# mooch443/trex

Hardware: AMD Instinct MI355X
Metric: frames/s end-to-end (segment+CNN-ID), 2048x2048 x100 individuals (higher is better)
Workload: dtype fp16x3-split

## Files before the change

### include/trexhip.h

```cpp
#ifndef TREXHIP_H
#define TREXHIP_H
#include <stddef.h>
#include <stdint.h>
#ifdef __cplusplus
extern "C" {
#endif

#define TREXHIP_ABI_VERSION 22

enum {
    TREXHIP_OK = 0,
    TREXHIP_E_INVALID = -1,
    TREXHIP_E_DEVICE = -2,
    TREXHIP_E_CAPACITY = -3,
    TREXHIP_E_UNSUPPORTED = -4,
    TREXHIP_E_NOMEM = -5
};

#define TREXHIP_FRAME_OVERFLOW_RUNS   1u
#define TREXHIP_FRAME_OVERFLOW_OUTPUT 2u
#define TREXHIP_FRAME_MALFORMED       4u

typedef struct trexhip_params {
    int32_t device;
    int32_t width, height;
    int32_t max_batch;
    int32_t max_runs;
    int32_t max_blobs;
    int32_t max_pixels;
    int32_t threshold;
    int32_t threshold_maximum;
    int32_t enable_difference;
    int32_t absolute_difference;
    int32_t image_invert;
    int32_t inclusive;
    int32_t zero_is_background;
    int32_t connectivity;
    int32_t dilation_size;
    int32_t use_closing;
    int32_t closing_size;
    int32_t n_ranges;
    double  cm_per_pixel;
    double  ranges[16];
    int32_t pixel_encoding;
    int32_t image_adjust, blur_difference, equalize_histogram, correct_luminance, use_adaptive_threshold;
    int32_t device_color_reduce;
    int32_t reserved_[1];
} trexhip_params;
enum { TREXHIP_ENC_GRAY = 0, TREXHIP_ENC_R3G3B2 = 1, TREXHIP_ENC_RGB8 = 2 };

#define TREXHIP_BLOB_IN_RANGE    0u
#define TREXHIP_BLOB_BELOW_RANGE 1u
#define TREXHIP_BLOB_BIG         2u

typedef struct trexhip_run { uint16_t x0, x1, y, pad; } trexhip_run;

typedef struct trexhip_blob {
    uint32_t run_begin, n_runs;
    uint32_t pix_begin, n_pixels;
    uint16_t x0, y0, x1, y1;
    uint32_t bid;
    uint32_t px_min_max;
    uint32_t parent;
    uint32_t flags;
    uint64_t m10, m01;
    uint64_t m20, m11, m02;
    uint64_t sp, spx, spy;
} trexhip_blob;

typedef struct trexhip_frame_info {
    uint32_t n_blobs, n_runs, n_pixels;
    uint32_t blob_begin, run_begin, pix_begin;
    uint32_t n_raw_runs, n_raw_blobs;
    uint32_t flags;
    uint32_t reserved[3];
} trexhip_frame_info;

typedef struct trexhip_batch_result {
    int32_t n_frames;
    uint32_t total_blobs, total_runs, total_pixels;
    const trexhip_frame_info* frames;
    const trexhip_blob* blobs;
    const trexhip_run* runs;
    const uint8_t* pixels;
    uint32_t pixel_channels;
    uint32_t reserved_;
} trexhip_batch_result;

typedef struct trexhip_device_view {
    const trexhip_frame_info* frames;
    const trexhip_blob* blobs;
// ... 92 lines not shown
    int32_t n_ranges;
    int32_t reserved_;
    double  size_ranges[16];
} trexhip_split_params;
typedef struct trexhip_split_info {
    int32_t threshold;
    int32_t effective_threshold;
    int32_t status;
    int32_t initial_action;
    int32_t n_result;
    int32_t n_evaluated;
    int32_t min_pixel, max_pixel;
    float   first_size;
    float   reserved_;
    double  min_size_bound;
} trexhip_split_info;
void trexhip_default_split_params(trexhip_split_params* p);
int trexhip_split_search_device(trexhip_ctx* ctx, const trexhip_split_params* sp, int32_t method, const int32_t* d_presumed_nr,
                                int32_t n_blobs, int32_t* d_thresholds, trexhip_split_info* d_info);

typedef struct trexhip_posture_params {
    float   outline_resample;
    int32_t outline_smooth_samples;
    int32_t outline_smooth_step;
    int32_t outline_approximate;
    float   outline_curvature_range_ratio;
    float   midline_walk_offset;
    int32_t max_points;
    int32_t posture_closing_steps, peak_mode, posture_direction_smoothing;
} trexhip_posture_params;
typedef struct trexhip_posture_info { int32_t status, n_outline, n_segments, tail_index, head_index, n_traced, reserved[2]; } trexhip_posture_info;
void trexhip_default_posture_params(trexhip_posture_params* p);
int trexhip_posture_device(trexhip_ctx* ctx, int32_t table, const trexhip_posture_params* pp, int32_t n_blobs,
                           float* d_outline, float* d_segments, trexhip_posture_info* d_info);

int trexhip_posture_auto_device(trexhip_ctx* ctx, const trexhip_posture_params* pp, int32_t method, int32_t track_posture_threshold,
                                int32_t n_blobs, float* d_outline, float* d_segments, trexhip_posture_info* d_info,
                                int32_t* d_threshold_used, int32_t* d_iterations);

typedef struct trexhip_midline_params {
    int32_t midline_resolution;
    float   midline_stiff_percentage;
    int32_t midline_invert;
    int32_t midline_start_with_head;
} trexhip_midline_params;
typedef struct trexhip_midline_info { int32_t status, n; float len, angle, offx, offy; int32_t reserved[2]; } trexhip_midline_info;
void trexhip_default_midline_params(trexhip_midline_params* p);
int trexhip_midline_device(trexhip_ctx* ctx, const trexhip_midline_params* mp, int32_t n_blobs, int32_t max_points,
                           const trexhip_posture_info* d_posture_info, float* d_segments, float* d_midline,
                           trexhip_midline_info* d_midline_info);
int trexhip_midline_movement_device(trexhip_ctx* ctx, const trexhip_midline_params* mp, int32_t n_blobs, int32_t max_points,
                                    const trexhip_posture_info* d_posture_info, float* d_segments, float* d_midline,
                                    trexhip_midline_info* d_midline_info, const float* d_movement_direction);

enum { TREXHIP_NORMALIZE_NONE = 0, TREXHIP_NORMALIZE_MOMENTS = 1, TREXHIP_NORMALIZE_POSTURE = 2 };
int trexhip_crops_device(trexhip_ctx* ctx, uint8_t* d_crops, int32_t n_blobs, int32_t out_w, int32_t out_h,
                         int32_t normalization, int32_t difference);

int trexhip_crops_transformed_device(trexhip_ctx* ctx, uint8_t* d_crops, int32_t n_blobs, int32_t out_w, int32_t out_h,
                                     const float* transforms, const float* midline_lengths, int32_t use_legacy,
                                     float image_scale, int32_t difference);
int trexhip_crops_posture_device(trexhip_ctx* ctx, uint8_t* d_crops, int32_t n_blobs, int32_t out_w, int32_t out_h,
                                 const trexhip_midline_info* d_midline_info, const float* midline_lengths, int32_t use_legacy,
                                 float image_scale, int32_t difference);

int trexhip_load_weights(trexhip_ctx* ctx, const void* blob, size_t bytes);
int trexhip_num_classes(trexhip_ctx* ctx);
int trexhip_network_channels(trexhip_ctx* ctx);
int trexhip_network_image_size(trexhip_ctx* ctx, int32_t* width, int32_t* height);
enum { TREXHIP_NET_V118_3 = 0, TREXHIP_NET_V100 = 1, TREXHIP_NET_V110 = 2, TREXHIP_NET_V119 = 3, TREXHIP_NET_V200 = 4 };
int trexhip_network_version(trexhip_ctx* ctx);
size_t trexhip_network_blob_bytes(int32_t version, int32_t classes, int32_t channels, int32_t width, int32_t height);
int trexhip_identify_chunk_crops(trexhip_ctx* ctx, int32_t* crops);
enum { TREXHIP_CNN_FP32 = 0, TREXHIP_CNN_BF16X6 = 1, TREXHIP_CNN_BF16X3 = 2, TREXHIP_CNN_FP16X3 = 3 };
int trexhip_set_identity_precision(trexhip_ctx* ctx, int32_t mode);
int trexhip_identify_device(trexhip_ctx* ctx, const uint8_t* d_crops, int32_t n, float* d_probs, float* d_logits);
int trexhip_identify(trexhip_ctx* ctx, const uint8_t* crops, int32_t n, float* probs);
int trexhip_identify_guard_stats(trexhip_ctx* ctx, uint32_t* rerun_crops, uint32_t* whole_batch);
int trexhip_identify_skip_stats(trexhip_ctx* ctx, uint32_t* passes, uint32_t* listed, uint64_t* bytes_filled);

int trexhip_identify_skip3_stats(trexhip_ctx* ctx, uint32_t* pairs, uint32_t* listed, uint32_t* passes, uint64_t* bytes_filled);

int trexhip_identify_skipx_stats(trexhip_ctx* ctx, uint32_t* crops_windowed, uint32_t* windowed_passes, uint32_t* full_passes);

int trexhip_identify_fc1_stats(trexhip_ctx* ctx, uint32_t* rows, uint32_t* listed);

int trexhip_export_id_table_device(trexhip_ctx* ctx, const float* d_probs, int32_t n_blobs, int32_t classes,
                                   uint32_t frame_base, void* d_table, int32_t max_rows);
int trexhip_export_id_table_ex_device(trexhip_ctx* ctx, const float* d_probs, int32_t n_blobs, int32_t classes, uint32_t frame_base,
                                      const float* d_midline, const trexhip_midline_info* d_midline_info, int32_t midline_resolution,
                                      void* d_table, int32_t max_rows);

typedef struct trexhip_comm trexhip_comm;
int trexhip_comm_unique_id(void* id128);
int trexhip_comm_create(trexhip_ctx* ctx, const void* id128, int32_t rank, int32_t world, trexhip_comm** out);
void trexhip_comm_destroy(trexhip_comm* comm);
int trexhip_comm_rank(trexhip_comm* comm);
int trexhip_comm_world(trexhip_comm* comm);
int trexhip_comm_gather_device(trexhip_comm* comm, const void* d_send, size_t bytes, void* d_recv_rank0);
int trexhip_comm_gather_device_on(trexhip_comm* comm, trexhip_ctx* stream_ctx, const void* d_send, size_t bytes, void* d_recv_rank0);
int trexhip_comm_count_ranks(trexhip_comm* comm, int32_t* ranks_seen);

enum { TREXHIP_STAGE_ROWS = 0, TREXHIP_STAGE_SEGMENT_ALL = 1, TREXHIP_STAGE_CONV2 = 2, TREXHIP_STAGE_CONV3 = 3,
       TREXHIP_STAGE_CNN_ALL = 4, TREXHIP_STAGE_CROPS = 5, TREXHIP_STAGE_POSTURE = 6,
       TREXHIP_STAGE_UPLOAD_COPY = 8, TREXHIP_STAGE_UPLOAD_DMA = 9, TREXHIP_STAGE_COUNT = 10 };
int trexhip_profile_enable(trexhip_ctx* ctx, int32_t on);
int trexhip_profile_read(trexhip_ctx* ctx, int32_t stage, double* total_ms, int64_t* launches);
int trexhip_profile_reset(trexhip_ctx* ctx);

#define TREXHIP_NET_CATEGORY 100
typedef struct trexhip_trainer trexhip_trainer;
typedef struct {
    int32_t max_batch;
    float lr;
    float beta1, beta2, eps;
    float bn_momentum;
    float dropout;
    int32_t precision;
    uint64_t seed;
} trexhip_train_params;
size_t trexhip_weight_blob_bytes(int32_t classes, int32_t channels);
int trexhip_trainer_create(trexhip_ctx* ctx, const void* blob, size_t bytes, const trexhip_train_params* params, trexhip_trainer** out);
void trexhip_trainer_destroy(trexhip_trainer* trainer);
int trexhip_trainer_set_lr(trexhip_trainer* trainer, float lr);
int64_t trexhip_trainer_steps(trexhip_trainer* trainer);
int trexhip_trainer_image_size(trexhip_trainer* trainer, int32_t* width, int32_t* height);
int trexhip_trainer_version(trexhip_trainer* trainer, int32_t* version);
size_t trexhip_trainer_keep_mask_bytes(trexhip_trainer* trainer, int32_t n);
int trexhip_train_step_device(trexhip_trainer* trainer, const float* d_inputs, const int32_t* d_targets, int32_t n, const uint8_t* d_keep_masks,
                              float* loss, int32_t* correct);
int trexhip_train_eval_device(trexhip_trainer* trainer, const float* d_inputs, const int32_t* d_targets, int32_t n, float* loss, int32_t* correct);
int trexhip_train_eval(trexhip_trainer* trainer, const float* inputs, const int32_t* targets, int32_t n, float* loss, int32_t* correct);
int trexhip_train_step(trexhip_trainer* trainer, const float* inputs, const int32_t* targets, int32_t n, const uint8_t* keep_masks, float* loss,
                       int32_t* correct);
int trexhip_train_predict_device(trexhip_trainer* trainer, const uint8_t* d_crops, int32_t n, float* d_probs);
int trexhip_trainer_read(trexhip_trainer* trainer, int32_t tensor, int32_t kind, float* out, size_t count);
int trexhip_trainer_export(trexhip_trainer* trainer, void* blob, size_t capacity, size_t* bytes);

typedef struct {
    float degrees;
    float translate_x, translate_y;
    float brightness_lo, brightness_hi;
    float contrast_lo, contrast_hi;
    float saturation_lo, saturation_hi;
    float hue_lo, hue_hi;
    uint64_t seed;
} trexhip_augment_params;
typedef struct {
    float angle; int32_t tx, ty;
    float brightness, contrast, saturation, hue;
    int32_t order;
} trexhip_augment_draw;
void trexhip_default_augment_params(trexhip_augment_params* p, int32_t width, int32_t height);
int trexhip_augment_device(trexhip_ctx* ctx, const trexhip_augment_params* ap, const uint8_t* d_pool, const int32_t* d_pool_targets,
                           int32_t pool_size, const int32_t* indices, int32_t n, int32_t width, int32_t height, int32_t channels,
                           trexhip_augment_draw* d_draws, int32_t draws_given, uint64_t counter, float* d_out, int32_t* d_targets_out);

typedef struct {
    uint32_t good_frames, bad_frames;
    float    good_ratio;
    float    mean_unique;
    float    mean_unique_raw;
} trexhip_uniqueness_result;
int trexhip_validation_metrics_device(trexhip_ctx* ctx, const float* d_probs, int32_t n, int32_t classes,
                                      const int32_t* d_targets,
                                      const int32_t* frame_ranges,
// ... 58 lines not shown
```

### trex_amd/capi.py

```python
import collections
import ctypes as C
import os
import numpy as np

_HERE = os.path.dirname(os.path.abspath(__file__))
LIB_PATH = os.environ.get("TREXHIP_LIB_PATH") or os.path.join(_HERE, "libtrexhip.so")
_LIB = None

RUN_DTYPE = np.dtype([("x0", "<u2"), ("x1", "<u2"), ("y", "<u2"), ("pad", "<u2")])
BLOB_DTYPE = np.dtype([
    ("run_begin", "<u4"), ("n_runs", "<u4"), ("pix_begin", "<u4"), ("n_pixels", "<u4"),
    ("x0", "<u2"), ("y0", "<u2"), ("x1", "<u2"), ("y1", "<u2"),
    ("bid", "<u4"), ("px_min_max", "<u4"), ("parent", "<u4"), ("flags", "<u4"),
    ("m10", "<u8"), ("m01", "<u8"), ("m20", "<u8"), ("m11", "<u8"), ("m02", "<u8"),
    ("sp", "<u8"), ("spx", "<u8"), ("spy", "<u8"),
])
INFO_DTYPE = np.dtype([
    ("n_blobs", "<u4"), ("n_runs", "<u4"), ("n_pixels", "<u4"),
    ("blob_begin", "<u4"), ("run_begin", "<u4"), ("pix_begin", "<u4"),
    ("n_raw_runs", "<u4"), ("n_raw_blobs", "<u4"), ("flags", "<u4"), ("reserved", "<u4", (3,)),
])
assert BLOB_DTYPE.itemsize == 104 and RUN_DTYPE.itemsize == 8 and INFO_DTYPE.itemsize == 48

CNN_FP32, CNN_BF16X6, CNN_BF16X3, CNN_FP16X3 = 0, 1, 2, 3
# ... 73 lines not shown
MIDLINE_INFO_DTYPE = np.dtype([("status", "<i4"), ("n", "<i4"), ("len", "<f4"), ("angle", "<f4"), ("offx", "<f4"), ("offy", "<f4"),
                               ("reserved", "<i4", (2,))])
POSTURE_INFO_DTYPE = np.dtype([("status", "<i4"), ("n_outline", "<i4"), ("n_segments", "<i4"), ("tail_index", "<i4"),
                               ("head_index", "<i4"), ("n_traced", "<i4"), ("reserved", "<i4", (2,))])


class BatchResult(C.Structure):
    _fields_ = [
        ("n_frames", C.c_int32), ("total_blobs", C.c_uint32), ("total_runs", C.c_uint32), ("total_pixels", C.c_uint32),
        ("frames", C.c_void_p), ("blobs", C.c_void_p), ("runs", C.c_void_p), ("pixels", C.c_void_p),
        ("pixel_channels", C.c_uint32), ("reserved_", C.c_uint32),
    ]


ENC_GRAY, ENC_R3G3B2, ENC_RGB8 = 0, 1, 2
FRAME_OVERFLOW_RUNS, FRAME_OVERFLOW_OUTPUT, FRAME_MALFORMED = 1, 2, 4


class DeviceView(C.Structure):
    _fields_ = [("frames", C.c_void_p), ("blobs", C.c_void_p), ("runs", C.c_void_p), ("pixels", C.c_void_p),
                ("totals", C.c_void_p), ("blob_frame", C.c_void_p)]


class TrexHipError(RuntimeError):
    def __init__(self, code, msg):
        super().__init__(f"libtrexhip error {code}: {msg}")
        self.code = code
        self.frames = None


class TrainParams(C.Structure):
    _fields_ = [("max_batch", C.c_int32), ("lr", C.c_float), ("beta1", C.c_float), ("beta2", C.c_float), ("eps", C.c_float),
                ("bn_momentum", C.c_float), ("dropout", C.c_float), ("precision", C.c_int32), ("seed", C.c_uint64)]


class AugmentParams(C.Structure):
    _fields_ = [("degrees", C.c_float), ("translate_x", C.c_float), ("translate_y", C.c_float), ("brightness_lo", C.c_float), ("brightness_hi", C.c_float),
                ("contrast_lo", C.c_float), ("contrast_hi", C.c_float), ("saturation_lo", C.c_float), ("saturation_hi", C.c_float),
                ("hue_lo", C.c_float), ("hue_hi", C.c_float), ("seed", C.c_uint64)]


AUGMENT_DRAW_DTYPE = np.dtype([("angle", "<f4"), ("tx", "<i4"), ("ty", "<i4"), ("brightness", "<f4"), ("contrast", "<f4"), ("saturation", "<f4"),
                               ("hue", "<f4"), ("order", "<i4")])
assert AUGMENT_DRAW_DTYPE.itemsize == 32
AUGMENT_IDENTITY_ORDER = 0xE4


class UniquenessResult(C.Structure):
    _fields_ = [("good_frames", C.c_uint32), ("bad_frames", C.c_uint32), ("good_ratio", C.c_float), ("mean_unique", C.c_float), ("mean_unique_raw", C.c_float)]


class ValidationMetrics:
    __slots__ = ("confusion", "per_class_accuracy", "good_frames", "bad_frames", "good_ratio", "mean_unique", "mean_unique_raw",
                 "unique_percent", "unique_percent_raw", "uniqueness_per_class")

    def __init__(self):
        for k in self.__slots__:
            setattr(self, k, None)


class ClassAverages:
    __slots__ = ("samples", "values", "max_index", "max_p")

    def __init__(self, samples, values, max_index, max_p):
        self.samples, self.values, self.max_index, self.max_p = samples, values, max_index, max_p


class VisualFieldResult:
    __slots__ = VF_OUTPUTS

    def __init__(self):
        for k in self.__slots__:
            setattr(self, k, None)


TrackletLabels = collections.namedtuple("TrackletLabels", "counts rows label share skipped")


SYMBOLS = [
    "trexhip_abi_version", "trexhip_network_channels", "trexhip_network_image_size", "trexhip_network_version", "trexhip_network_blob_bytes", "trexhip_identify_chunk_crops", "trexhip_comm_unique_id", "trexhip_comm_create", "trexhip_comm_destroy", "trexhip_comm_rank", "trexhip_comm_world", "trexhip_comm_gather_device", "trexhip_comm_gather_device_on", "trexhip_comm_count_ranks", "trexhip_last_error", "trexhip_default_params", "trexhip_create", "trexhip_destroy",
    "trexhip_set_stream", "trexhip_get_live_params", "trexhip_update_params", "trexhip_set_background", "trexhip_set_background_device", "trexhip_set_background_color", "trexhip_set_background_color_device", "trexhip_generate_average_device", "trexhip_get_background", "trexhip_segment_device",
    "trexhip_segment", "trexhip_segment_color", "trexhip_segment_color_device", "trexhip_rethreshold_device", "trexhip_rethreshold_per_blob_device", "trexhip_fetch_rethreshold", "trexhip_fetch", "trexhip_device_view_get", "trexhip_synchronize",
    "trexhip_profile_enable", "trexhip_profile_read", "trexhip_profile_reset",
    "trexhip_default_posture_params", "trexhip_posture_device", "trexhip_posture_auto_device", "trexhip_pack_frames_v6_device", "trexhip_crops_device", "trexhip_pixel_channels", "trexhip_device_alloc", "trexhip_device_free", "trexhip_copy_to_host", "trexhip_copy_to_device", "trexhip_crops_transformed_device", "trexhip_crops_posture_device", "trexhip_default_midline_params", "trexhip_midline_device", "trexhip_midline_movement_device", "trexhip_default_split_params", "trexhip_split_search_device", "trexhip_export_id_table_device", "trexhip_export_id_table_ex_device", "trexhip_load_weights", "trexhip_set_identity_precision", "trexhip_num_classes", "trexhip_identify_device", "trexhip_identify", "trexhip_identify_guard_stats", "trexhip_identify_skip_stats", "trexhip_identify_skip3_stats", "trexhip_identify_skipx_stats", "trexhip_identify_fc1_stats",
    "trexhip_weight_blob_bytes", "trexhip_trainer_create", "trexhip_trainer_destroy", "trexhip_trainer_set_lr", "trexhip_trainer_steps", "trexhip_trainer_image_size", "trexhip_trainer_version", "trexhip_trainer_keep_mask_bytes", "trexhip_train_step_device", "trexhip_train_step", "trexhip_train_eval_device", "trexhip_train_eval", "trexhip_trainer_read", "trexhip_trainer_export",
    "trexhip_default_augment_params", "trexhip_augment_device",
    "trexhip_train_predict_device", "trexhip_validation_metrics_device", "trexhip_class_averages_device",
    "trexhip_lzo1x_bound", "trexhip_lzo1x_compress", "trexhip_pv_write_frames",
    "trexhip_load_frames_v6_device", "trexhip_lzo1x_decompress", "trexhip_pv_read_frames",
    "trexhip_default_prefilter_params", "trexhip_prefilter_device",
    "trexhip_default_vf_params", "trexhip_visual_field_device",
    "trexhip_categorize_load_weights", "trexhip_categorize_info", "trexhip_categorize_blob_bytes", "trexhip_categorize_device", "trexhip_categorize",
    "trexhip_tracklet_labels_device",
]


def lib():
    global _LIB
    if _LIB is None:
        if not os.path.exists(LIB_PATH):
            raise TrexHipError(-1, f"{LIB_PATH} is missing: run __graft_entry__.build() (make -C trex_amd/csrc)")
        L = C.CDLL(LIB_PATH)
        L.trexhip_last_error.restype = C.c_char_p
        L.trexhip_default_params.argtypes = [C.POINTER(Params), C.c_int32, C.c_int32]
        L.trexhip_default_params.restype = None
        L.trexhip_create.argtypes = [C.POINTER(Params), C.POINTER(C.c_void_p)]
        L.trexhip_destroy.argtypes = [C.c_void_p]
        L.trexhip_destroy.restype = None
        L.trexhip_set_stream.argtypes = [C.c_void_p, C.c_void_p]
        L.trexhip_get_live_params.argtypes = [C.c_void_p, C.POINTER(LiveParams)]
        L.trexhip_update_params.argtypes = [C.c_void_p, C.POINTER(LiveParams)]
        L.trexhip_set_background.argtypes = [C.c_void_p, C.c_void_p, C.c_int32]
        L.trexhip_set_background_device.argtypes = [C.c_void_p, C.c_void_p]
        L.trexhip_set_background_color.argtypes = [C.c_void_p, C.c_void_p, C.c_int32, C.c_int32, C.c_int32]
        L.trexhip_set_background_color_device.argtypes = [C.c_void_p, C.c_void_p, C.c_int32, C.c_int32]
        L.trexhip_generate_average_device.argtypes = [C.c_void_p, C.c_void_p, C.c_int32, C.c_int32]
        L.trexhip_get_background.argtypes = [C.c_void_p, C.c_void_p, C.c_int32]
        L.trexhip_segment_device.argtypes = [C.c_void_p, C.c_void_p, C.c_int32]
        L.trexhip_segment.argtypes = [C.c_void_p, C.POINTER(C.c_void_p), C.c_int32, C.c_int32]
        L.trexhip_segment_color.argtypes = [C.c_void_p, C.POINTER(C.c_void_p), C.c_int32, C.c_int32, C.c_int32, C.c_int32]
        L.trexhip_segment_color_device.argtypes = [C.c_void_p, C.c_void_p, C.c_int32, C.c_int32, C.c_int32]
        L.trexhip_rethreshold_device.argtypes = [C.c_void_p, C.c_int32, C.c_int32, C.c_void_p, C.c_int32]
        L.trexhip_rethreshold_per_blob_device.argtypes = [C.c_void_p, C.c_int32, C.c_void_p, C.c_int32, C.c_void_p, C.c_int32]
        L.trexhip_fetch_rethreshold.argtypes = [C.c_void_p, C.POINTER(BatchResult)]
        L.trexhip_fetch.argtypes = [C.c_void_p, C.POINTER(BatchResult)]
        L.trexhip_device_view_get.argtypes = [C.c_void_p, C.POINTER(DeviceView)]
        L.trexhip_synchronize.argtypes = [C.c_void_p]
        L.trexhip_profile_enable.argtypes = [C.c_void_p, C.c_int32]
        L.trexhip_profile_read.argtypes = [C.c_void_p, C.c_int32, C.POINTER(C.c_double), C.POINTER(C.c_int64)]
        L.trexhip_profile_reset.argtypes = [C.c_void_p]
        L.trexhip_default_midline_params.argtypes = [C.POINTER(MidlineParams)]
        L.trexhip_default_midline_params.restype = None
        L.trexhip_midline_device.argtypes = [C.c_void_p, C.POINTER(MidlineParams), C.c_int32, C.c_int32, C.c_void_p, C.c_void_p, C.c_void_p, C.c_void_p]
        L.trexhip_midline_movement_device.argtypes = [C.c_void_p, C.POINTER(MidlineParams), C.c_int32, C.c_int32, C.c_void_p, C.c_void_p, C.c_void_p, C.c_void_p, C.c_void_p]
        L.trexhip_default_split_params.argtypes = [C.POINTER(SplitParams)]
        L.trexhip_default_split_params.restype = None
        L.trexhip_split_search_device.argtypes = [C.c_void_p, C.POINTER(SplitParams), C.c_int32, C.c_void_p, C.c_int32, C.c_void_p, C.c_void_p]
        L.trexhip_crops_posture_device.argtypes = [C.c_void_p, C.c_void_p, C.c_int32, C.c_int32, C.c_int32, C.c_void_p, C.c_void_p, C.c_int32, C.c_float, C.c_int32]
        L.trexhip_default_posture_params.argtypes = [C.POINTER(PostureParams)]
        L.trexhip_default_posture_params.restype = None
        L.trexhip_posture_device.argtypes = [C.c_void_p, C.c_int32, C.POINTER(PostureParams), C.c_int32, C.c_void_p, C.c_void_p, C.c_void_p]
        L.trexhip_posture_auto_device.argtypes = [C.c_void_p, C.POINTER(PostureParams), C.c_int32, C.c_int32, C.c_int32, C.c_void_p, C.c_void_p, C.c_void_p, C.c_void_p, C.c_void_p]
        L.trexhip_crops_transformed_device.argtypes = [C.c_void_p, C.c_void_p, C.c_int32, C.c_int32, C.c_int32, C.c_void_p, C.c_void_p, C.c_int32, C.c_float, C.c_int32]
        L.trexhip_crops_device.argtypes = [C.c_void_p, C.c_void_p] + [C.c_int32] * 5
        L.trexhip_export_id_table_device.argtypes = [C.c_void_p, C.c_void_p, C.c_int32, C.c_int32, C.c_uint32, C.c_void_p, C.c_int32]
        L.trexhip_export_id_table_ex_device.argtypes = [C.c_void_p, C.c_void_p, C.c_int32, C.c_int32, C.c_uint32, C.c_void_p, C.c_void_p, C.c_int32, C.c_void_p, C.c_int32]
        L.trexhip_load_weights.argtypes = [C.c_void_p, C.c_void_p, C.c_size_t]
        L.trexhip_num_classes.argtypes = [C.c_void_p]
        L.trexhip_network_channels.argtypes = [C.c_void_p]
        L.trexhip_network_image_size.argtypes = [C.c_void_p, C.POINTER(C.c_int32), C.POINTER(C.c_int32)]
        L.trexhip_network_version.argtypes = [C.c_void_p]
        L.trexhip_network_blob_bytes.argtypes = [C.c_int32] * 5; L.trexhip_network_blob_bytes.restype = C.c_size_t
        L.trexhip_identify_chunk_crops.argtypes = [C.c_void_p, C.POINTER(C.c_int32)]
        L.trexhip_pack_frames_v6_device.argtypes = [C.c_void_p, C.c_void_p, C.c_void_p, C.c_size_t, C.c_void_p]
        L.trexhip_lzo1x_bound.argtypes = [C.c_size_t]; L.trexhip_lzo1x_bound.restype = C.c_size_t
        L.trexhip_lzo1x_compress.argtypes = [C.c_void_p, C.c_size_t, C.c_void_p, C.c_size_t, C.POINTER(C.c_size_t)]
        L.trexhip_pv_write_frames.argtypes = [C.c_void_p, C.c_void_p, C.c_int32, C.c_int32, C.c_uint64, C.c_void_p, C.c_size_t, C.c_void_p, C.POINTER(C.c_size_t)]
        L.trexhip_load_frames_v6_device.argtypes = [C.c_void_p, C.c_void_p, C.c_void_p, C.c_int32, C.c_void_p]
        L.trexhip_lzo1x_decompress.argtypes = [C.c_void_p, C.c_size_t, C.c_void_p, C.c_size_t, C.POINTER(C.c_size_t)]
        L.trexhip_pv_read_frames.argtypes = [C.c_void_p, C.c_size_t, C.c_uint64, C.c_void_p, C.c_int32, C.c_void_p, C.c_size_t, C.c_void_p, C.POINTER(C.c_size_t)]
        L.trexhip_comm_unique_id.argtypes = [C.c_void_p]
        L.trexhip_comm_create.argtypes = [C.c_void_p, C.c_void_p, C.c_int32, C.c_int32, C.POINTER(C.c_void_p)]
        L.trexhip_comm_destroy.argtypes = [C.c_void_p]
        L.trexhip_comm_destroy.restype = None
        L.trexhip_comm_rank.argtypes = [C.c_void_p]
        L.trexhip_comm_world.argtypes = [C.c_void_p]
        L.trexhip_comm_gather_device.argtypes = [C.c_void_p, C.c_void_p, C.c_size_t, C.c_void_p]
        L.trexhip_comm_gather_device_on.argtypes = [C.c_void_p, C.c_void_p, C.c_void_p, C.c_size_t, C.c_void_p]
        L.trexhip_comm_count_ranks.argtypes = [C.c_void_p, C.POINTER(C.c_int32)]
        L.trexhip_set_identity_precision.argtypes = [C.c_void_p, C.c_int32]
        L.trexhip_identify_device.argtypes = [C.c_void_p, C.c_void_p, C.c_int32, C.c_void_p, C.c_void_p]
        L.trexhip_identify.argtypes = [C.c_void_p, C.c_void_p, C.c_int32, C.c_void_p]
        L.trexhip_identify_guard_stats.argtypes = [C.c_void_p, C.POINTER(C.c_uint32), C.POINTER(C.c_uint32)]
        L.trexhip_identify_skip_stats.argtypes = [C.c_void_p, C.POINTER(C.c_uint32), C.POINTER(C.c_uint32), C.POINTER(C.c_uint64)]
        L.trexhip_identify_skipx_stats.argtypes = [C.c_void_p, C.POINTER(C.c_uint32), C.POINTER(C.c_uint32), C.POINTER(C.c_uint32)]
        L.trexhip_identify_skip3_stats.argtypes = [C.c_void_p, C.POINTER(C.c_uint32), C.POINTER(C.c_uint32), C.POINTER(C.c_uint32), C.POINTER(C.c_uint64)]
        L.trexhip_identify_fc1_stats.argtypes = [C.c_void_p, C.POINTER(C.c_uint32), C.POINTER(C.c_uint32)]
        L.trexhip_weight_blob_bytes.argtypes = [C.c_int32, C.c_int32]
        L.trexhip_weight_blob_bytes.restype = C.c_size_t
        L.trexhip_trainer_create.argtypes = [C.c_void_p, C.c_void_p, C.c_size_t, C.POINTER(TrainParams), C.POINTER(C.c_void_p)]
        L.trexhip_trainer_destroy.argtypes = [C.c_void_p]
        L.trexhip_trainer_destroy.restype = None
        L.trexhip_trainer_set_lr.argtypes = [C.c_void_p, C.c_float]
        L.trexhip_trainer_steps.argtypes = [C.c_void_p]
        L.trexhip_trainer_steps.restype = C.c_int64
        L.trexhip_trainer_image_size.argtypes = [C.c_void_p, C.POINTER(C.c_int32), C.POINTER(C.c_int32)]
        L.trexhip_trainer_version.argtypes = [C.c_void_p, C.POINTER(C.c_int32)]
        L.trexhip_trainer_keep_mask_bytes.argtypes = [C.c_void_p, C.c_int32]
        L.trexhip_trainer_keep_mask_bytes.restype = C.c_size_t
        L.trexhip_train_step_device.argtypes = [C.c_void_p, C.c_void_p, C.c_void_p, C.c_int32, C.c_void_p, C.POINTER(C.c_float), C.POINTER(C.c_int32)]
        L.trexhip_train_step.argtypes = [C.c_void_p, C.c_void_p, C.c_void_p, C.c_int32, C.c_void_p, C.POINTER(C.c_float), C.POINTER(C.c_int32)]
        L.trexhip_train_eval_device.argtypes = [C.c_void_p, C.c_void_p, C.c_void_p, C.c_int32, C.POINTER(C.c_float), C.POINTER(C.c_int32)]
        L.trexhip_train_eval.argtypes = [C.c_void_p, C.c_void_p, C.c_void_p, C.c_int32, C.POINTER(C.c_float), C.POINTER(C.c_int32)]
        L.trexhip_trainer_read.argtypes = [C.c_void_p, C.c_int32, C.c_int32, C.c_void_p, C.c_size_t]
        L.trexhip_trainer_export.argtypes = [C.c_void_p, C.c_void_p, C.c_size_t, C.POINTER(C.c_size_t)]
        L.trexhip_default_augment_params.argtypes = [C.POINTER(AugmentParams), C.c_int32, C.c_int32]
        L.trexhip_default_augment_params.restype = None
        L.trexhip_augment_device.argtypes = [C.c_void_p, C.POINTER(AugmentParams), C.c_void_p, C.c_void_p, C.c_int32, C.c_void_p, C.c_int32, C.c_int32, C.c_int32,
                                             C.c_int32, C.c_void_p, C.c_int32, C.c_uint64, C.c_void_p, C.c_void_p]
        L.trexhip_train_predict_device.argtypes = [C.c_void_p, C.c_void_p, C.c_int32, C.c_void_p]
        L.trexhip_validation_metrics_device.argtypes = [C.c_void_p, C.c_void_p, C.c_int32, C.c_int32, C.c_void_p, C.c_void_p, C.c_int32, C.c_void_p,
                                                        C.POINTER(UniquenessResult), C.c_void_p, C.c_void_p, C.c_void_p]
        L.trexhip_class_averages_device.argtypes = [C.c_void_p, C.c_void_p, C.c_int32, C.c_int32, C.c_void_p, C.c_int32, C.c_void_p, C.c_void_p, C.c_void_p, C.c_void_p]
        L.trexhip_device_alloc.argtypes = [C.c_void_p, C.c_size_t, C.POINTER(C.c_void_p)]
        L.trexhip_device_free.argtypes = [C.c_void_p, C.c_void_p]
        L.trexhip_copy_to_host.argtypes = [C.c_void_p, C.c_void_p, C.c_void_p, C.c_size_t]
        L.trexhip_copy_to_device.argtypes = [C.c_void_p, C.c_void_p, C.c_void_p, C.c_size_t]
        L.trexhip_default_prefilter_params.argtypes = [C.POINTER(PrefilterParams)]
        L.trexhip_default_prefilter_params.restype = None
        L.trexhip_prefilter_device.argtypes = [C.c_void_p, C.POINTER(PrefilterParams), C.POINTER(PrefilterTables), C.c_void_p, C.c_void_p, C.c_void_p, C.c_void_p]
        L.trexhip_default_vf_params.argtypes = [C.c_void_p, C.POINTER(VfParams)]
        L.trexhip_default_vf_params.restype = None
        L.trexhip_visual_field_device.argtypes = [C.c_void_p, C.POINTER(VfParams), C.c_void_p, C.c_void_p, C.c_void_p, C.c_int32, C.c_void_p, C.c_int32,
                                                  C.c_void_p, C.c_int32, C.c_void_p, C.c_void_p, C.c_void_p, C.c_void_p, C.c_void_p, C.c_void_p]
        L.trexhip_categorize_load_weights.argtypes = [C.c_void_p, C.c_void_p, C.c_size_t]
        L.trexhip_categorize_info.argtypes = [C.c_void_p, C.POINTER(C.c_int32), C.POINTER(C.c_int32), C.POINTER(C.c_int32), C.POINTER(C.c_int32)]
        L.trexhip_categorize_blob_bytes.argtypes = [C.c_int32, C.c_int32, C.c_int32, C.c_int32]
        L.trexhip_categorize_blob_bytes.restype = C.c_size_t
        L.trexhip_categorize_device.argtypes = [C.c_void_p, C.c_void_p, C.c_int32, C.c_void_p, C.c_void_p, C.c_void_p]
        L.trexhip_categorize.argtypes = [C.c_void_p, C.c_void_p, C.c_int32, C.c_void_p]
        L.trexhip_tracklet_labels_device.argtypes = [C.c_void_p, C.c_void_p, C.c_void_p, C.c_int32, C.c_int32, C.c_int32, C.c_void_p, C.c_void_p, C.c_void_p,
                                                     C.c_void_p, C.POINTER(C.c_uint32)]
        _LIB = L
    return _LIB


def _check(rc):
    if rc != 0:
        raise TrexHipError(rc, lib().trexhip_last_error().decode())


def default_params(width, height, **kw):
    p = Params()
    lib().trexhip_default_params(C.byref(p), width, height)
    ranges = kw.pop("size_ranges", None)
    for k, v in kw.items():
        if not hasattr(p, k):
            raise KeyError(k)
        setattr(p, k, v)
    if ranges is not None:
        p.n_ranges = len(ranges)
        for i, (a, b) in enumerate(ranges):
            p.ranges[2 * i], p.ranges[2 * i + 1] = a, b
    return p


def default_augment_params(width, height, **kw):
    p = AugmentParams()
    lib().trexhip_default_augment_params(C.byref(p), width, height)
    for k, v in kw.items():
        if not hasattr(p, k):
            raise KeyError(k)
        setattr(p, k, v)
    return p


def _from_addr(addr, count, dtype):
    if count == 0 or not addr:
# ... 195 lines not shown

    def split_search_device(self, d_presumed_ptr, n_blobs, d_thresholds_ptr, d_info_ptr, method=1, size_ranges=(), **kw):
        sp = SplitParams()
        lib().trexhip_default_split_params(C.byref(sp))
        for k, v in kw.items():
            setattr(sp, k, v)
        sp.n_ranges = len(size_ranges)
        for i, (a, b) in enumerate(size_ranges):
            sp.size_ranges[2 * i], sp.size_ranges[2 * i + 1] = a, b
        _check(lib().trexhip_split_search_device(self._h, C.byref(sp), method, C.c_void_p(d_presumed_ptr), n_blobs, C.c_void_p(d_thresholds_ptr),
                                                 C.c_void_p(d_info_ptr)))

    def crops_posture_device(self, d_crops_ptr, n_blobs, d_midline_info_ptr, midline_lengths=None, out_w=80, out_h=80, legacy=False, scale=1.0, difference=0):
        ln = None if midline_lengths is None else np.ascontiguousarray(midline_lengths, np.float32)
        _check(lib().trexhip_crops_posture_device(self._h, C.c_void_p(d_crops_ptr), n_blobs, out_w, out_h, C.c_void_p(d_midline_info_ptr),
                                                  None if ln is None else ln.ctypes.data_as(C.c_void_p), 1 if legacy else 0, scale, difference))

    def crops_transformed_device(self, d_crops_ptr, transforms, midline_lengths, out_w=80, out_h=80, legacy=False, scale=1.0, difference=0):
        tr = np.ascontiguousarray(transforms, np.float32)
        ln = np.ascontiguousarray(midline_lengths, np.float32)
        _check(lib().trexhip_crops_transformed_device(self._h, C.c_void_p(d_crops_ptr), len(tr), out_w, out_h, tr.ctypes.data_as(C.c_void_p),
                                                      ln.ctypes.data_as(C.c_void_p), 1 if legacy else 0, scale, difference))

    def export_id_table_ex(self, d_probs_ptr, n_blobs, classes, frame_base, d_table_ptr, max_rows, d_midline_ptr=0, d_midline_info_ptr=0, midline_resolution=0):
        _check(lib().trexhip_export_id_table_ex_device(self._h, C.c_void_p(d_probs_ptr) if d_probs_ptr else None, n_blobs, classes, frame_base,
                                                       C.c_void_p(d_midline_ptr) if d_midline_ptr else None,
                                                       C.c_void_p(d_midline_info_ptr) if d_midline_info_ptr else None, midline_resolution,
                                                       C.c_void_p(d_table_ptr), max_rows))

    def export_id_table(self, d_probs_ptr, n_blobs, classes, frame_base, d_table_ptr, max_rows):
        _check(lib().trexhip_export_id_table_device(self._h, C.c_void_p(d_probs_ptr) if d_probs_ptr else None, n_blobs,
                                                    classes, frame_base, C.c_void_p(d_table_ptr), max_rows))

    def load_weights(self, blob: bytes):
        buf = (C.c_uint8 * len(blob)).from_buffer_copy(blob)
        _check(lib().trexhip_load_weights(self._h, buf, len(blob)))

    def set_identity_precision(self, mode):
        _check(lib().trexhip_set_identity_precision(self._h, mode))

    def num_classes(self):
        return lib().trexhip_num_classes(self._h)

    def network_image_size(self):
        w, h = C.c_int32(0), C.c_int32(0)
        _check(lib().trexhip_network_image_size(self._h, C.byref(w), C.byref(h)))
        return int(w.value), int(h.value)

    def network_version(self):
        return int(lib().trexhip_network_version(self._h))

    def identify_chunk_crops(self):
        c = C.c_int32(0)
        _check(lib().trexhip_identify_chunk_crops(self._h, C.byref(c)))
        return int(c.value)

    def probabilities(self, crops):
        crops = np.ascontiguousarray(crops, np.uint8)
        w, h = self.network_image_size()
        if w:
            want = (h, w, lib().trexhip_network_channels(self._h))
            if crops.ndim != 4 or tuple(crops.shape[1:]) != want:
                raise ValueError(f"crops must have shape (n, {want[0]}, {want[1]}, {want[2]}) for the loaded network, got {crops.shape}")
        n = crops.shape[0]
        out = np.empty((n, self.num_classes()), np.float32)
        _check(lib().trexhip_identify(self._h, crops.ctypes.data_as(C.c_void_p), n, out.ctypes.data_as(C.c_void_p)))
        return out

    def guard_stats(self):
        a, b = C.c_uint32(0), C.c_uint32(0)
        _check(lib().trexhip_identify_guard_stats(self._h, C.byref(a), C.byref(b)))
        return int(a.value), bool(b.value)

    def skip_stats(self):
        a, b, c = C.c_uint32(0), C.c_uint32(0), C.c_uint64(0)
        _check(lib().trexhip_identify_skip_stats(self._h, C.byref(a), C.byref(b), C.byref(c)))
        return int(a.value), int(b.value), int(c.value)

    def skipx_stats(self):
        a, b, c = C.c_uint32(0), C.c_uint32(0), C.c_uint32(0)
        _check(lib().trexhip_identify_skipx_stats(self._h, C.byref(a), C.byref(b), C.byref(c)))
        return int(a.value), int(b.value), int(c.value)

    def skip3_stats(self):
        a, b, c, d = C.c_uint32(0), C.c_uint32(0), C.c_uint32(0), C.c_uint64(0)
        _check(lib().trexhip_identify_skip3_stats(self._h, C.byref(a), C.byref(b), C.byref(c), C.byref(d)))
        return int(a.value), int(b.value), int(c.value), int(d.value)

    def fc1_stats(self):
        a, b = C.c_uint32(0), C.c_uint32(0)
        _check(lib().trexhip_identify_fc1_stats(self._h, C.byref(a), C.byref(b)))
        return int(a.value), int(b.value)

    def identify_device(self, d_crops_ptr, n, d_probs_ptr, d_logits_ptr=None):
        _check(lib().trexhip_identify_device(self._h, C.c_void_p(d_crops_ptr), n, C.c_void_p(d_probs_ptr),
                                             C.c_void_p(d_logits_ptr) if d_logits_ptr else None))

    def device_alloc(self, nbytes):
        out = C.c_void_p()
        _check(lib().trexhip_device_alloc(self._h, nbytes, C.byref(out)))
        return int(out.value)

    def device_free(self, d_ptr):
        _check(lib().trexhip_device_free(self._h, C.c_void_p(d_ptr or 0)))

    def copy_to_device(self, d_ptr, array):
        a = np.ascontiguousarray(array)
        _check(lib().trexhip_copy_to_device(self._h, C.c_void_p(d_ptr), a.ctypes.data_as(C.c_void_p), a.nbytes))

    def copy_to_host(self, d_ptr, shape, dtype):
        out = np.empty(shape, dtype)
        _check(lib().trexhip_copy_to_host(self._h, out.ctypes.data_as(C.c_void_p), C.c_void_p(d_ptr), out.nbytes))
        return out

    def augment_device(self, d_pool_ptr, pool_size, n, width, height, channels, d_out_ptr, ap=None, indices=None, d_pool_targets_ptr=0,
                       d_targets_out_ptr=0, d_draws_ptr=0, draws_given=False, counter=0):
        idx = None
        if indices is not None:
            idx = np.ascontiguousarray(indices, np.int32)
            if idx.shape != (n,):
                raise ValueError(f"indices must hold n = {n} entries, got shape {idx.shape}")
        _check(lib().trexhip_augment_device(self._h, C.byref(ap) if ap is not None else None, C.c_void_p(d_pool_ptr), C.c_void_p(d_pool_targets_ptr or 0), pool_size,
                                            idx.ctypes.data_as(C.c_void_p) if idx is not None else None, n, width, height, channels,
                                            C.c_void_p(d_draws_ptr or 0), 1 if draws_given else 0, counter, C.c_void_p(d_out_ptr), C.c_void_p(d_targets_out_ptr or 0)))

    def validation_metrics(self, d_probs_ptr, n, classes, d_targets_ptr=0, frame_ranges=None):
        out = ValidationMetrics()
        conf = np.zeros((classes, classes), np.uint32) if d_targets_ptr else None
        fr = None
        res = UniquenessResult()
        up = upr = upc = None
        if frame_ranges is not None:
            fr = np.ascontiguousarray(frame_ranges, np.int32).reshape(-1, 2)
            up, upr, upc = np.zeros(len(fr), np.float32), np.zeros(len(fr), np.float32), np.zeros(classes, np.float32)
        ptr = lambda a: a.ctypes.data_as(C.c_void_p) if a is not None else None
        _check(lib().trexhip_validation_metrics_device(self._h, C.c_void_p(d_probs_ptr or 0), n, classes, C.c_void_p(d_targets_ptr or 0), ptr(fr),
                                                       len(fr) if fr is not None else 0, ptr(conf), C.byref(res) if fr is not None else None,
                                                       ptr(up), ptr(upr), ptr(upc)))
        if conf is not None:
            rows = conf.sum(axis=1, dtype=np.int64)
            out.confusion = conf
            out.per_class_accuracy = np.zeros(classes, np.float64)
            np.divide(np.diagonal(conf), rows, out=out.per_class_accuracy, where=rows > 0)
        if fr is not None:
            out.good_frames, out.bad_frames = int(res.good_frames), int(res.bad_frames)
            out.good_ratio, out.mean_unique, out.mean_unique_raw = float(res.good_ratio), float(res.mean_unique), float(res.mean_unique_raw)
            out.unique_percent, out.unique_percent_raw, out.uniqueness_per_class = up, upr, upc
        return out

    def class_averages(self, d_probs_ptr, n, classes, d_ids_ptr, n_ids):
        samples, values = np.zeros(max(n_ids, 0), np.float32), np.zeros((max(n_ids, 0), max(classes, 0)), np.float32)
        max_index, max_p = np.zeros(max(n_ids, 0), np.int32), np.zeros(max(n_ids, 0), np.float32)
        ptr = lambda a: a.ctypes.data_as(C.c_void_p)
        _check(lib().trexhip_class_averages_device(self._h, C.c_void_p(d_probs_ptr or 0), n, classes, C.c_void_p(d_ids_ptr or 0), n_ids,
                                                   ptr(samples), ptr(values), ptr(max_index), ptr(max_p)))
        return ClassAverages(samples, values, max_index, max_p)

    def load_category_weights(self, blob):
        _check(lib().trexhip_categorize_load_weights(self._h, blob, len(blob)))

    def category_info(self):
        v = [C.c_int32(0) for _ in range(4)]
        _check(lib().trexhip_categorize_info(self._h, *[C.byref(x) for x in v]))
        return tuple(int(x.value) for x in v)

    def categorize_device(self, d_crops_ptr, n, d_labels_ptr, d_probs_ptr=None, d_logits_ptr=None):
# ... 407 lines not shown
```

### trex_amd/csrc/cnn.hip

```cpp
#include "cnn_net.h"
#include "cnn_arch.h"
#include "cnn_split.h"
#include "cnn_weights.h"
#include <algorithm>
#include <cmath>
#include <cstdio>
#include <cstdlib>
#include <cstring>
#include <vector>

namespace trexhip {

template <int CH>
__global__ __launch_bounds__(256, 2) void k_conv1(const uint8_t* __restrict__ crops, const float* __restrict__ w ,
                                                  const float* __restrict__ bias , float* __restrict__ out, int S) {
    extern __shared__ __attribute__((aligned(16))) float lds[];
    const int PW = S + 4;
    float* wl = lds;
    float* img = lds + CH * 25 * 16;
    const int crop = blockIdx.x;
    const uint8_t* src = crops + (size_t)crop * S * S * CH;
    for (int i = threadIdx.x; i < CH * PW * PW; i += 256) img[i] = 0.f;
    for (int i = threadIdx.x; i < CH * 25 * 16; i += 256) wl[i] = w[i];
    __syncthreads();
// ... 1183 lines not shown

#define TRY(x) do { if (rc == TREXHIP_OK) rc = (x); } while (0)
static int make_empty_v3(trexhip_ctx* ctx, Net* net);
int net_load(trexhip_ctx* ctx, const void* blob, size_t bytes) {
    const int arch = blob_arch_id(blob, bytes);
    if (arch >= TREXHIP_NET_V100 && arch <= TREXHIP_NET_V200) return arch_load(ctx, blob, bytes);
    WeightBlob wb;
    const int prc = parse_weight_blob(blob, bytes, "trexhip_load_weights", &wb, [](int W, int H) -> int {
        if (W < 8 || W > 256 || H < 8 || H > 256) {
            set_error("trexhip_load_weights: individual_image_size " + std::to_string(W) + "x" + std::to_string(H) + " is outside 8..256 x 8..256");
            return TREXHIP_E_UNSUPPORTED;
        }
        return TREXHIP_OK;
    });
    if (prc != TREXHIP_OK) return prc;
    const int classes = wb.classes, W = wb.W, H = wb.H, CH = wb.CH;
    const bool at80 = W == 80 && H == 80;

    TH_CHECK_HIP(hipSetDevice(ctx->p.device));
    free_net(static_cast<Net*>(ctx->net));
    ctx->net = nullptr;
    Net* net = new Net();
    net->classes = classes; net->W = W; net->H = H; net->CH = CH;
    int rc = TREXHIP_OK;
    const Folded c1 = fold_conv1(&wb.t[T_C1W], CH);
    TRY(upload(net, &net->w1, c1.w)); TRY(upload(net, &net->b1, c1.b));
    if (at80) TRY(upload(net, &net->w1h, &net->inv1h, pack_conv1_frags(c1.w, CH)));
    const Folded c2 = fold_conv(&wb.t[T_C2W], 64, 16, 16);
    TRY(upload(net, &net->w2, c2.w)); TRY(upload(net, &net->b2, c2.b));
    TRY(upload(net, &net->w2s, pack_bf16x3(c2.w, 16, 64)));
    TRY(upload(net, &net->w2h, &net->inv2h, pack_f16x2(c2.w, 16, 64)));
    if (at80) TRY(upload(net, &net->w2w, &net->inv2w, pack_wino_f16(c2.w, 16, 64)));
    const Folded c3 = fold_conv(&wb.t[T_C3W], 128, 64, 16);
    TRY(upload(net, &net->w3s, pack_bf16x3(c3.w, 64, 128)));
    TRY(upload(net, &net->w3h, &net->inv3h, pack_f16x2(c3.w, 64, 128)));
    if (at80) TRY(upload(net, &net->w3w, &net->inv3w, pack_wino_f16(c3.w, 64, 128)));
    TRY(net->weights.device_bytes(&net->d_ovf, OVF_WORDS * 4, "trexhip_load_weights"));
    if (rc == TREXHIP_OK && hipMemset(net->d_ovf, 0, OVF_WORDS * 4) != hipSuccess) rc = TREXHIP_E_DEVICE;
    const Folded c3x = fold_conv(&wb.t[T_C3W], 128, 64, 32);
    TRY(upload(net, &net->w3, c3x.w)); TRY(upload(net, &net->b3, c3x.b));
    const Folded f1 = pack_fc1(wb.t[T_F1W], wb.t[T_F1B], W, H);
    TRY(upload(net, &net->wf1, f1.w)); TRY(upload(net, &net->bf1, f1.b));
    if (at80) TRY(upload(net, &net->wf1h, &net->invf1h, pack_fc1_f16(f1.w)));
    TRY(upload(net, &net->lng, wb.t[T_LNG], 100 * sizeof(float)));
    TRY(upload(net, &net->lnb, wb.t[T_LNB], 100 * sizeof(float)));
    TRY(upload(net, &net->wf2t, pack_fc2(wb.t[T_F2W], classes)));
    TRY(upload(net, &net->bf2, wb.t[T_F2B], classes * sizeof(float)));
    if (at80 && CH == 1) TRY(make_empty_v3(ctx, net));
    if (rc != TREXHIP_OK) { free_net(net); return rc; }
    ctx->net = net;
    return TREXHIP_OK;
}

static int ensure_act(trexhip_ctx* ctx, Net* net, int n) {
    if (n <= net->max_crops) return TREXHIP_OK;
    drop_graphs(net);
    net->batch.free_all();
    net->h_probs = nullptr;
    net->max_crops = 0;
    Mem& B = net->batch;
    const char* who = "trexhip_identify_device";
    const size_t N = n;
    const size_t W = net->W, H = net->H;
    int rc = B.device_bytes(&net->d_ovfc, N, who);
    TRY(B.device_bytes(&net->act1, N * (H / 2) * (W / 2) * 16 * 4, who));
    TRY(B.device_bytes(&net->act2, N * (H / 4) * (W / 4) * 64 * 4, who));
    TRY(B.device_bytes(&net->act3, N * (H / 8) * (W / 8) * 128 * 4, who));
    TRY(B.device_bytes(&net->fc1, N * 128 * 4 * FC1_KSPLIT, who));
    TRY(B.device_bytes(&net->probs, N * net->classes * 4, who));
    TRY(B.device_bytes(&net->logits, N * net->classes * 4, who));
    if (W == 80 && H == 80) {
        TRY(B.device_bytes(&net->v2, N * 40 * V2_ROWB, who));
        const size_t img = net->v3e ? (size_t)SkipGeom::V3_ROWS * V3_ROWB : 0;
        TRY(B.device_bytes(&net->v3, N * 20 * V3_ROWB + 2 * img, who));
        if (rc == TREXHIP_OK && img) {
            TH_CHECK_HIP(hipMemcpyAsync(net->v3, net->v3e, img, hipMemcpyDeviceToDevice, ctx->stream));
            TH_CHECK_HIP(hipMemcpyAsync(net->v3 + img + N * 20 * V3_ROWB, net->v3e, img, hipMemcpyDeviceToDevice, ctx->stream));
            net->v3 += img;
        }
    }
    if (net->v3e) {
        const size_t n_pass = (N * SkipGeom::V3_ROWS + SkipGeom::RPP - 1) / SkipGeom::RPP;
        TRY(B.device_bytes(&net->skip_bands, N * sizeof(int2), who));
        TRY(B.device_bytes(&net->skip_counts, ((n_pass + SKIP_LB - 1) / SKIP_LB) * 4 * 4, who));
        TRY(B.device_bytes(&net->skip_list, (n_pass + SKIP_PAD) * 4, who));
        TRY(B.device_bytes(&net->skipx_cols, N * sizeof(int2), who));
        TRY(B.device_bytes(&net->skipx_list, (N * skipx_passes({0, SkipGeom::V3_ROWS - 1}) + SKIP_PAD) * 4, who));
        const size_t blocks3 = (N + Skip3Geom::BLOCK - 1) / Skip3Geom::BLOCK;
        TRY(B.device_bytes(&net->skip3_counts, ((blocks3 + SKIP3_TB - 1) / SKIP3_TB) * sizeof(uint2), who));
        TRY(B.device_bytes(&net->skip3_tcounts, blocks3 * 4, who));
        TRY(B.device_bytes(&net->skip3_desc, blocks3 * Skip3Geom::BLOCK_PASSES * Skip3Geom::DESC * 4, who));
        TRY(B.device_bytes(&net->skip3_rows, blocks3 * Skip3Geom::BLOCK_PASSES * Skip3Reach::WORDS * 4, who));
        TRY(B.device_bytes(&net->fc1_list, Skip3Geom::PAIRS * N * sizeof(int), who));
    }
    TRY(B.device_bytes(&net->crops, N * net->W * net->H * net->CH, who));
    TRY(B.pinned(&net->h_probs, N * net->classes, who));
    if (rc != TREXHIP_OK) return rc;
    TH_CHECK_HIP(hipMemsetAsync(net->d_ovfc, 0, N, ctx->stream));
    net->max_crops = n;
    return TREXHIP_OK;
}
#undef TRY

std::vector<LdsAttr>& lds_attrs() { static std::vector<LdsAttr> v; return v; }

static const ByChannels K_CONV1{Kern(k_conv1<1>, 256, (84 * 84 + 25 * 16) * 4, false), Kern(k_conv1<3>, 256, 3 * (84 * 84 + 25 * 16) * 4, false)};
static const ByChannels K_CONV1_MFMA{Kern(k_conv1_mfma, 256), Kern(k_conv1_mfma3, 256)};
static const ByChannels K_CONV1_WPRE{Kern(k_conv1_wpre<1>, 256), Kern(k_conv1_wpre<3>, 256)};
static const Kern K_CONV12_RS(k_conv12_rs<W12RGeom>, 512, W12RGeom::LDS_BYTES);
static const Kern K_CONV12_RSX(k_conv12_rs<W12XGeom>, 512, W12XGeom::LDS_BYTES);
static const Kern K_CONV12_WPRE(k_conv12_wpre, 256, W12Geom::LDS_BYTES);
static const Kern K_CROP_BANDS(k_crop_bands, 256);
static const Kern K_PASS_COUNT(k_pass_count, SKIP_LB);
static const Kern K_PASS_LIST(k_pass_list, SKIP_LB);
static const Kern K_V3_FILL(k_v3_fill, SKIP_FILL_TB);
static const Kern K_CONV2_WPRE2(k_conv2_wpre2, 256, W2bGeom::LDS_BYTES);
static const Kern K_CONV2_STREAM(k_conv5_stream<16, 64, 40, 8, 4>, 256, ConvGeomS<16, 64, 40, 8, 4>::LDS_BYTES);
using GW3 = WinoGeom<64, 128, 20, 2>;
static const Kern K_CONV3_WINO(k_conv5_wino<64, 128, 20, 2>, GW3::NTHR, GW3::LDS_BYTES);
static const Kern K_CONV3_WPAIR(k_conv5_wpair<false>, 256, GW3::LDS_BYTES + 1024 );
static const Kern K_CONV3_WPAIR_LIST(k_conv5_wpair<true>, 256, GW3::LDS_BYTES + 1024);
static const Kern K_PAIR_COUNT(k_pair_count, SKIP3_TB);
static const Kern K_PAIR_LIST(k_pair_list, SKIP3_TB);
static const Kern K_ACT3_FILL(k_act3_fill, 256);
template <int CI, int CO, int S, int ROWS, int NTERMS>
static auto split_kern() { return Kern(k_conv5_split<CI, CO, S, ROWS, NTERMS>, 512, ConvGeomB<CI, CO, S, ROWS, SPLIT_NP>::LDS_BYTES); }
struct ExactLayer { decltype(Kern(k_conv5<16, 64, 40, 20, 16>, 512)) f32; decltype(split_kern<16, 64, 40, 10, 6>()) x6, x3, x6_plan; };
static const auto K_CONV2_X6 = split_kern<16, 64, 40, 10, 6>();
static const ExactLayer K_CONV2{Kern(k_conv5<16, 64, 40, 20, 16>, 512, ConvGeom<16, 64, 40, 20, 16>::LDS_BYTES), K_CONV2_X6, split_kern<16, 64, 40, 10, 3>(), K_CONV2_X6};
static const ExactLayer K_CONV3{Kern(k_conv5<64, 128, 20, 20, 32>, 512, ConvGeom<64, 128, 20, 20, 32>::LDS_BYTES), split_kern<64, 128, 20, 20, 6>(),
                                split_kern<64, 128, 20, 20, 3>(), split_kern<64, 128, 20, 4, 6>()};
static const Kern K_FC1(k_fc1, 256);
static const Kern K_FC1_SPLIT1(k_fc1_split<1>, 256), K_FC1_SPLIT4(k_fc1_split<4>, 256), K_FC1_SPLIT4_LIST(k_fc1_split<4, true>, 256);
static const Kern K_FC1_LIST(k_fc1_list, FC1L_TB);
static const Kern K_HEAD(k_head, 256);
static const Kern K_HEAD_SMALL(k_head_small, 256);
static const Kern K_GUARD_PLAN(k_guard_plan, 1024);

struct Pass {
    const Net& net; const CnnPlan& p; hipStream_t s; int mode;
    const uint8_t* crops; int n; float *probs, *logits;
};

static void launch_conv1(const Pass& f, const Conv1 kind, const uint32_t* guard) {
    const Net& net = f.net;
    switch (kind) {
    case Conv1::FUSED: break;
    case Conv1::WPRE: K_CONV1_WPRE[net.CH](f.s, f.p.conv1_grid, f.crops, net.w1h, net.b1, net.v2, net.inv1h, net.ovf(OVF_RANGE)); break;
    case Conv1::MFMA: K_CONV1_MFMA[net.CH](f.s, f.p.conv1_grid, f.crops, net.w1h, net.b1, net.act1, net.inv1h, guard); break;
    case Conv1::VALU: K_CONV1[net.CH](f.s, f.p.conv1_grid, f.crops, net.w1, net.b1, net.act1, net.W); break;
    case Conv1::ANY: any_conv1(f.s, net, f.p, f.crops); break;
    }
}

static void launch_exact(const Pass& f, const int layer, const int mode, const uint32_t* guard) {
    const Net& net = f.net;
    const bool c2 = layer == 2;
    const ExactLayer& K = c2 ? K_CONV2 : K_CONV3;
    const Launch& l = guard ? (c2 ? f.p.r_conv2 : f.p.r_conv3) : (c2 ? f.p.conv2 : f.p.conv3);
    const float *in = c2 ? net.act1 : net.act2, *b = c2 ? net.b2 : net.b3;
    float* out = c2 ? net.act2 : net.act3;
    if (mode == TREXHIP_CNN_FP32) K.f32(f.s, l.grid, in, c2 ? net.w2 : net.w3, b, out);
    else (guard ? K.x6_plan : mode == TREXHIP_CNN_BF16X6 ? K.x6 : K.x3)(f.s, l.grid, in, c2 ? net.w2s : net.w3s, b, out, 1.0f, guard, l.items);
}

static void launch_tail(const Pass& f, const uint32_t* guard) {
    const Net& net = f.net;
    const CnnPlan& p = f.p;
    if (guard || p.fc1 == Fc1::EXACT)
        K_FC1(f.s, dim3(guard ? p.r_fc1_grid : p.fc1_grid, p.planes), net.act3, net.wf1, net.bf1, net.fc1, f.n, p.K, guard);
    else if (p.fc1_listed)
        K_FC1_SPLIT4_LIST(f.s, dim3(p.fc1_grid, p.planes), net.act3, net.wf1h, net.bf1, net.fc1, f.n, p.K, net.invf1h, net.ovf(OVF_RANGE), net.d_ovfc,
                          net.fc1_list, net.d_skip + SK3_FC1_LEN, net.max_crops);
    else
        (p.fc1 == Fc1::SPLIT1 ? K_FC1_SPLIT1 : K_FC1_SPLIT4)(f.s, dim3(p.fc1_grid, p.planes), net.act3, net.wf1h, net.bf1, net.fc1, f.n, p.K, net.invf1h,
                                                            net.ovf(OVF_RANGE), net.d_ovfc, nullptr, nullptr, 0);
    if (guard || p.head == Head::BIG) {
        const bool listed = !guard && p.fc1_listed;
        K_HEAD(f.s, guard ? p.r_head_grid : p.head_grid, net.fc1, net.lng, net.lnb, net.wf2t, net.bf2, f.probs, f.logits, f.n, net.classes, guard, p.planes,
               listed ? net.fc1e : nullptr, listed ? net.skip_bands : nullptr, listed ? net.d_skip : nullptr);
    }
    else
        K_HEAD_SMALL(f.s, p.head_grid, net.fc1, net.lng, net.lnb, net.wf2t, net.bf2, f.probs, f.logits, f.n, net.classes, p.planes,
                     p.head_plans ? net.ovf(OVF_RANGE) : nullptr, net.d_ovfc, p.head_plans ? net.ovf(OVF_PLAN) : nullptr);
}

static void launch_rerun(const Pass& f) {
    const uint32_t* g = f.net.ovf(OVF_PLAN);
    if (!f.p.head_plans) K_GUARD_PLAN(f.s, 1, f.net.ovf(OVF_RANGE), f.net.d_ovfc, f.n, f.net.ovf(OVF_PLAN));
    if (f.p.rerun_conv1) launch_conv1(f, Conv1::MFMA, g);
    for (const int layer : {2, 3}) {
        if (f.p.chain == Chain::ANY_SIZE) any_conv(f.s, f.net, f.p, layer, TREXHIP_CNN_BF16X6, g);
        else launch_exact(f, layer, TREXHIP_CNN_BF16X6, g);
    }
    launch_tail(f, g);
}

static int make_empty_v3(trexhip_ctx* ctx, Net* net) {
    const char* who = "trexhip_load_weights";
    uint8_t* zero = nullptr;
    int rc = net->weights.device_bytes(&net->v3e, (size_t)SkipGeom::V3_ROWS * V3_ROWB, who);
    if (rc == TREXHIP_OK) rc = net->weights.device_bytes(&net->act3e, (size_t)Skip3Geom::PAIRS * 10 * 128 * 4, who);
    if (rc == TREXHIP_OK) rc = net->weights.device_bytes(&net->fc1e, (size_t)FC1_KSPLIT * 128 * 4, who);
    if (rc == TREXHIP_OK) rc = net->weights.device_bytes(&net->d_skip, SK_WORDS * 4, who);
    if (rc == TREXHIP_OK) rc = net->weights.device_bytes(&net->act2e, (size_t)SkipGeom::V3_ROWS * 20 * 64 * 4, who);
    if (rc == TREXHIP_OK) rc = net->weights.device_bytes(&zero, SkipGeom::CROP_ROWS * 80, who);
    if (rc != TREXHIP_OK) return rc;
    const CnnPlan p = cnn_plan(80, 80, 1, TREXHIP_CNN_FP16X3, true, GEOM_ROLE_SPLIT | GEOM_NO_SKIP, 1, ctx->n_cus);
    TH_CHECK_HIP(hipFuncSetAttribute(reinterpret_cast<const void*>(K_CONV12_RS.fn), hipFuncAttributeMaxDynamicSharedMemorySize, K_CONV12_RS.lds));
    TH_CHECK_HIP(hipMemsetAsync(net->d_skip, 0, SK_WORDS * 4, ctx->stream));
    TH_CHECK_HIP(hipMemsetAsync(zero, 0, SkipGeom::CROP_ROWS * 80, ctx->stream));
    K_CONV12_RS(ctx->stream, p.conv2.grid, zero, net->w1h, net->b1, net->inv1h, net->w2w, net->b2, net->v3e, net->inv2w, net->d_skip + SK_EMPTY_RANGE, 1,
                net->d_skip + SK_EMPTY_CTR, p.pk2, nullptr, nullptr, nullptr, net->act2e);
    TH_CHECK_HIP(hipGetLastError());
    TH_CHECK_HIP(hipFuncSetAttribute(reinterpret_cast<const void*>(K_CONV3_WPAIR.fn), hipFuncAttributeMaxDynamicSharedMemorySize, K_CONV3_WPAIR.lds));
    K_CONV3_WPAIR(ctx->stream, p.conv3.grid, net->v3e, net->w3w, net->b3, net->act3e, net->inv3w, 1, net->d_skip + SK3_EMPTY_CTR, p.n_big3, nullptr, nullptr, nullptr);
    TH_CHECK_HIP(hipGetLastError());
    const CnnPlan pf = cnn_plan(80, 80, 1, TREXHIP_CNN_FP16X3, true, 0, 1, ctx->n_cus);
    K_FC1_SPLIT4(ctx->stream, dim3(1, pf.planes), net->act3e, net->wf1h, net->bf1, net->fc1e, 1, pf.K, net->invf1h, net->d_skip + SK3_FC1E_RANGE, nullptr,
                 nullptr, nullptr, 0);
    TH_CHECK_HIP(hipGetLastError());
    uint32_t range = 0;
    TH_CHECK_HIP(hipMemcpyAsync(&range, net->d_skip + SK3_FC1E_RANGE, 4, hipMemcpyDeviceToHost, ctx->stream));
    TH_CHECK_HIP(hipStreamSynchronize(ctx->stream));
    if (range) {
        const uint32_t one = 1;
        TH_CHECK_HIP(hipMemcpy(net->d_skip + SK_EMPTY_RANGE, &one, 4, hipMemcpyHostToDevice));
    }
    return TREXHIP_OK;
}

static void launch_skip_prep(const Pass& f, const bool direct) {
    const Net& net = f.net;
    const CnnPlan& p = f.p;
    const int n = f.n, lb = ceil_div(p.conv2.items, SKIP_LB);
    int2* cols = p.skipx ? net.skipx_cols : nullptr;
    K_CROP_BANDS(f.s, ceil_div(n, 4), f.crops, n, net.skip_bands, cols);
    K_PASS_COUNT(f.s, lb, net.skip_bands, cols, n, net.d_skip, net.skip_counts);
    K_PASS_LIST(f.s, lb, net.skip_bands, cols, n, net.d_skip, net.skip_counts, net.skip_list, net.skipx_list);
    if (p.skip3) {
        K_PAIR_COUNT(f.s, p.skip3_grid, net.skip_bands, n, net.d_skip, net.skip3_counts, net.skip3_tcounts);
        K_PAIR_LIST(f.s, p.skip3_grid, net.skip_bands, n, net.d_skip, net.skip3_counts, net.skip3_tcounts, net.skip3_desc);
        if (p.fc1_listed) K_FC1_LIST(f.s, Skip3Geom::PAIRS, net.skip_bands, n, net.d_skip, net.fc1_list, net.max_crops);
    }
    K_V3_FILL(f.s, ceil_div(n * SkipGeom::V3_ROWS, SKIP_FILL_TB), net.skip_bands, cols, n, net.d_skip, reinterpret_cast<const uint4*>(net.v3e),
              reinterpret_cast<uint4*>(net.v3), (int)direct);
}

static int net_forward_launch(trexhip_ctx* ctx, const uint8_t* d_crops, int n, float* d_probs, float* d_logits) {
    const Net& net = *static_cast<Net*>(ctx->net);
    if (!ctx->attr_cnn) {
        for (const LdsAttr& a : lds_attrs()) TH_CHECK_HIP(hipFuncSetAttribute(a.fn, hipFuncAttributeMaxDynamicSharedMemorySize, a.bytes));
        ctx->attr_cnn = true;
    }
    const CnnPlan p = cnn_plan(net.W, net.H, net.CH, ctx->cnn_mode, (reinterpret_cast<uintptr_t>(d_crops) & 15) == 0, ctx->tune_conv_geom, n, ctx->n_cus);
    const Pass f{net, p, ctx->stream, ctx->cnn_mode, d_crops, n, d_probs, d_logits};
    hipStream_t s = f.s;
    const long long alloc_rows = (long long)net.max_crops * SkipGeom::V3_ROWS;
    const bool direct = p.v3_direct && skip3_direct_fits(alloc_rows);
    stage_begin(ctx, TREXHIP_STAGE_CNN_ALL);
    launch_conv1(f, p.conv1, nullptr);
    if (p.chain == Chain::ANY_SIZE) {
        any_conv(s, net, p, 2, f.mode, nullptr);
        any_conv(s, net, p, 3, f.mode, nullptr);
    } else {
        const bool pre = p.chain == Chain::ROLE_SPLIT || p.chain == Chain::FUSED_2WG || p.chain == Chain::TWO_KERNEL;
        stage_begin(ctx, TREXHIP_STAGE_CONV2);
        switch (p.chain) {
        case Chain::ROLE_SPLIT:
            if (p.skip) launch_skip_prep(f, direct);
            if (p.skipx)
                K_CONV12_RSX(s, p.conv2.grid, d_crops, net.w1h, net.b1, net.inv1h, net.w2w, net.b2, net.v3, net.inv2w, net.ovf(OVF_RANGE), n, net.d_skip + SKX_CTR,
                             p.pk2, net.d_ovfc, net.skipx_list, net.d_skip + SKX_PASSES, net.act2e);
            K_CONV12_RS(s, p.conv2.grid, d_crops, net.w1h, net.b1, net.inv1h, net.w2w, net.b2, net.v3, net.inv2w, net.ovf(OVF_RANGE), n, net.ovf(OVF_PASS2),
                        p.pk2, net.d_ovfc, p.skip ? net.skip_list : nullptr, p.skip ? net.d_skip + (p.skipx ? SKX_FULL : SK_LEN) : nullptr, nullptr);
            break;
        case Chain::FUSED_2WG:
            K_CONV12_WPRE(s, p.conv2.grid, d_crops, net.w1h, net.b1, net.inv1h, net.w2w, net.b2, net.v3, net.inv2w, net.ovf(OVF_RANGE), n, net.ovf(OVF_PASS2),
                          p.pk2, net.d_ovfc);
            break;
        case Chain::TWO_KERNEL:
            K_CONV2_WPRE2(s, p.conv2.grid, net.v2, net.w2w, net.b2, net.v3, net.inv2w, net.ovf(OVF_RANGE), n, net.ovf(OVF_PASS2));
            break;
        case Chain::FP32_ACT:
            K_CONV2_STREAM(s, p.conv2.grid, net.act1, net.w2h, net.b2, net.act2, net.inv2h, net.ovf(OVF_RANGE), p.conv2.items);
            break;
        default: launch_exact(f, 2, f.mode, nullptr);
        }
        stage_end(ctx, TREXHIP_STAGE_CONV2);
        stage_begin(ctx, TREXHIP_STAGE_CONV3);
        if (pre) {
            if (p.skip3) {
                K_ACT3_FILL(s, p.act3_fill.grid, net.skip_bands, n, net.d_skip, reinterpret_cast<const uint4*>(net.act3e), reinterpret_cast<uint4*>(net.act3), net.skip3_desc,
                            net.skip3_rows, alloc_rows, (int)direct, (int)!p.fc1_listed);
                K_CONV3_WPAIR_LIST(s, p.conv3.grid, net.v3, net.w3w, net.b3, net.act3, net.inv3w, n, net.ovf(OVF_PASS3), 0, net.skip3_desc, net.skip3_rows, net.d_skip);
            }
            K_CONV3_WPAIR(s, p.conv3.grid, net.v3, net.w3w, net.b3, net.act3, net.inv3w, n, net.ovf(OVF_PASS3), p.n_big3, nullptr, nullptr, p.skip3 ? net.d_skip : nullptr);
        }
        else if (p.chain == Chain::FP32_ACT)
            K_CONV3_WINO(s, p.conv3.grid, net.act2, net.w3w, net.b3, net.act3, net.inv3w, net.ovf(OVF_RANGE), n, net.ovf(OVF_PASS3));
        else launch_exact(f, 3, f.mode, nullptr);
        stage_end(ctx, TREXHIP_STAGE_CONV3);
    }
    launch_tail(f, nullptr);
    if (p.rerun) launch_rerun(f);
    stage_end(ctx, TREXHIP_STAGE_CNN_ALL);
    TH_CHECK_HIP(hipGetLastError());
    return TREXHIP_OK;
}

static constexpr int GRAPH_MAX_CROPS = 6400;
static constexpr size_t GRAPH_CACHE = 8;
static constexpr int GRAPH_MIN_SEEN = 3;

static int net_forward_inner(trexhip_ctx* ctx, const uint8_t* d_crops, int n, float* d_probs, float* d_logits);
int net_forward(trexhip_ctx* ctx, const uint8_t* d_crops, int n, float* d_probs, float* d_logits) {
    Net* net = static_cast<Net*>(ctx->net);
    if (ctx->cnn_mode == TREXHIP_CNN_FP16X3) {
        if (!net->ovf_clean) TH_CHECK_HIP(hipMemsetAsync(net->d_ovf, 0, OVF_PLAN * 4, ctx->stream));
        net->ovf_clean = false;
    }
    const int rc = net_forward_inner(ctx, d_crops, n, d_probs, d_logits);
    if (rc == TREXHIP_OK) { net->last_mode = ctx->cnn_mode; if (ctx->cnn_mode == TREXHIP_CNN_FP16X3) net->ovf_clean = true; }
    net->last_fc1_n = rc == TREXHIP_OK && !net->arch && cnn_plan(net->W, net->H, net->CH, ctx->cnn_mode, (reinterpret_cast<uintptr_t>(d_crops) & 15) == 0,
                                                                 ctx->tune_conv_geom, n, ctx->n_cus).fc1_listed ? n : 0;
    return rc;
}

static bool capture_chain(trexhip_ctx* ctx, Net* net, Net::GraphEntry* cand, const uint8_t* d_crops, int n, float* d_probs, float* d_logits) {
    hipGraph_t graph = nullptr;
    hipGraphExec_t exec = nullptr;
    hipEvent_t ev = nullptr;
    bool ok = hipStreamBeginCapture(ctx->stream, hipStreamCaptureModeThreadLocal) == hipSuccess;
    if (ok) {
        const int rc = net_forward_launch(ctx, d_crops, n, d_probs, d_logits);
        const hipError_t e_end = hipStreamEndCapture(ctx->stream, &graph);
        ok = rc == TREXHIP_OK && e_end == hipSuccess && graph && hipGraphInstantiate(&exec, graph, nullptr, nullptr, 0) == hipSuccess &&
             hipEventCreateWithFlags(&ev, hipEventDisableTiming) == hipSuccess;
    }
    if (graph) (void)hipGraphDestroy(graph);
    if (!ok) {
        (void)hipGetLastError();
        if (exec) (void)hipGraphExecDestroy(exec);
        net->graphs_ok = false;
        return false;
    }
    cand->exec = exec; cand->last = ev;
    return true;
}

static int net_forward_inner(trexhip_ctx* ctx, const uint8_t* d_crops, int n, float* d_probs, float* d_logits) {
    Net* net = static_cast<Net*>(ctx->net);
    if (net->arch) return arch_forward(ctx, *net, d_crops, n, d_probs, d_logits);
    static const bool enabled = [] { const char* e = std::getenv("TREXHIP_GRAPHS"); return !(e && std::atoi(e) == 0); }();
    if (!enabled || !net->graphs_ok || n > GRAPH_MAX_CROPS || ctx->profiling || !ctx->attr_cnn) return net_forward_launch(ctx, d_crops, n, d_probs, d_logits);
    hipStream_t s = ctx->stream;
    const Net::GraphKey key{d_crops, n, d_probs, d_logits, ctx->cnn_mode, ctx->tune_conv_geom, s};
    ++net->tick;
// ... 27 lines not shown
    if (n == 0) return TREXHIP_OK;
    TH_CHECK_HIP(hipSetDevice(ctx->p.device));
    const int rc = loaded->arch ? arch_ensure_act(ctx, loaded, n) : ensure_act(ctx, loaded, n);
    if (rc == TREXHIP_OK) *net = loaded;
    return rc;
}

}

using namespace trexhip;

extern "C" {

int trexhip_load_weights(trexhip_ctx* ctx, const void* blob, size_t bytes) {
    if (!ctx || !blob) { set_error("trexhip_load_weights: null argument"); return TREXHIP_E_INVALID; }
    return net_load(ctx, blob, bytes);
}

int trexhip_identify_device(trexhip_ctx* ctx, const uint8_t* d_crops, int32_t n, float* d_probs, float* d_logits) {
    Net* net;
    const int rc = identify_prepare(ctx, ctx && d_crops && d_probs, "trexhip_identify_device", n, &net);
    if (rc || !net) return rc;
    return net_forward(ctx, d_crops, n, d_probs, d_logits);
}

int trexhip_identify(trexhip_ctx* ctx, const uint8_t* crops, int32_t n, float* probs) {
    Net* net;
    int rc = identify_prepare(ctx, ctx && crops && probs, "trexhip_identify", n, &net);
    if (rc || !net) return rc;
    const size_t cb = (size_t)net->W * net->H * net->CH;
    TH_CHECK_HIP(hipMemcpyAsync(net->crops, crops, cb * n, hipMemcpyHostToDevice, ctx->stream));
    rc = net_forward(ctx, net->crops, n, net->probs, nullptr);
    if (rc) return rc;
    TH_CHECK_HIP(hipMemcpyAsync(probs, net->probs, (size_t)n * net->classes * 4, hipMemcpyDeviceToHost, ctx->stream));
    TH_CHECK_HIP(hipStreamSynchronize(ctx->stream));
    return TREXHIP_OK;
}

int trexhip_identify_guard_stats(trexhip_ctx* ctx, uint32_t* rerun_crops, uint32_t* whole_batch) {
    if (!ctx || !ctx->net) { set_error("trexhip_identify_guard_stats: no context / weights not loaded"); return TREXHIP_E_INVALID; }
    Net* net = static_cast<Net*>(ctx->net);
    uint32_t plan[2] = {0, 0};
    TH_CHECK_HIP(hipStreamSynchronize(ctx->stream));
    if (net->last_mode == TREXHIP_CNN_FP16X3 && net->arch) {
        uint32_t st[2] = {0, 0};
        TH_CHECK_HIP(hipMemcpy(st, net->ovf(ARCH_STAT_RERUN), 8, hipMemcpyDeviceToHost));
        if (rerun_crops) *rerun_crops = st[0];
        if (whole_batch) *whole_batch = st[1] ? 1u : 0u;
        return TREXHIP_OK;
    }
    if (net->last_mode == TREXHIP_CNN_FP16X3) TH_CHECK_HIP(hipMemcpy(plan, net->ovf(OVF_PLAN), 8, hipMemcpyDeviceToHost));
    if (rerun_crops) *rerun_crops = plan[1] == 1u ? plan[0] : 0u;
    if (whole_batch) *whole_batch = plan[1] == 2u ? 1u : 0u;
    return TREXHIP_OK;
}

static int read_skip_words(trexhip_ctx* ctx, const char* who, uint32_t (&w)[SK_WORDS]) {
    if (!ctx || !ctx->net) { set_error(std::string(who) + ": no context / weights not loaded"); return TREXHIP_E_INVALID; }
    const Net* net = static_cast<Net*>(ctx->net);
    std::fill(w, w + SK_WORDS, 0u);
    TH_CHECK_HIP(hipStreamSynchronize(ctx->stream));
    if (net->d_skip) TH_CHECK_HIP(hipMemcpy(w, net->d_skip, sizeof w, hipMemcpyDeviceToHost));
    return TREXHIP_OK;
}

int trexhip_identify_skip_stats(trexhip_ctx* ctx, uint32_t* passes, uint32_t* listed, uint64_t* bytes_filled) {
    uint32_t w[SK_WORDS];
    if (const int rc = read_skip_words(ctx, "trexhip_identify_skip_stats", w)) return rc;
    if (passes) *passes = w[SK_NPASS];
    if (listed) *listed = w[SK_LEN];
    if (bytes_filled) *bytes_filled = (uint64_t)w[SK_FILLED] * V3_ROWB;
    return TREXHIP_OK;
}

int trexhip_identify_skipx_stats(trexhip_ctx* ctx, uint32_t* crops_windowed, uint32_t* windowed_passes, uint32_t* full_passes) {
    uint32_t w[SK_WORDS];
    if (const int rc = read_skip_words(ctx, "trexhip_identify_skipx_stats", w)) return rc;
    if (crops_windowed) *crops_windowed = w[SKX_CROPS];
    if (windowed_passes) *windowed_passes = w[SKX_PASSES];
    if (full_passes) *full_passes = w[SKX_FULL];
    return TREXHIP_OK;
}

int trexhip_identify_skip3_stats(trexhip_ctx* ctx, uint32_t* pairs, uint32_t* listed, uint32_t* passes, uint64_t* bytes_filled) {
    uint32_t w[SK_WORDS];
    if (const int rc = read_skip_words(ctx, "trexhip_identify_skip3_stats", w)) return rc;
    if (pairs) *pairs = w[SK3_PAIRS];
    if (listed) *listed = w[SK3_LISTED];
    if (passes) *passes = w[SK3_USE] ? w[SK3_PASSES] : 0u;
    if (bytes_filled) *bytes_filled = (uint64_t)w[SK3_FILLED] * (10 * 128 * 4);
    return TREXHIP_OK;
}

int trexhip_identify_fc1_stats(trexhip_ctx* ctx, uint32_t* rows, uint32_t* listed) {
    uint32_t w[SK_WORDS];
    if (const int rc = read_skip_words(ctx, "trexhip_identify_fc1_stats", w)) return rc;
    const Net* net = static_cast<Net*>(ctx->net);
    uint32_t sum = 0;
    for (int q = 0; q < Skip3Geom::PAIRS && net->last_fc1_n; ++q) sum += w[SK3_FC1_LEN + q];
    if (rows) *rows = (uint32_t)net->last_fc1_n * Skip3Geom::PAIRS;
    if (listed) *listed = sum;
    return TREXHIP_OK;
}

int trexhip_set_identity_precision(trexhip_ctx* ctx, int32_t mode) {
    if (!ctx || mode < 0 || mode > 3) { set_error("trexhip_set_identity_precision: mode must be one of TREXHIP_CNN_*"); return TREXHIP_E_INVALID; }
    ctx->cnn_mode = mode;
    return TREXHIP_OK;
}

int trexhip_num_classes(trexhip_ctx* ctx) {
    if (!ctx || !ctx->net) return 0;
    return static_cast<Net*>(ctx->net)->classes;
}

int trexhip_network_version(trexhip_ctx* ctx) {
    if (!ctx || !ctx->net) return 0;
    const Net* net = static_cast<const Net*>(ctx->net);
    return net->arch ? net->arch->plan.spec->id : TREXHIP_NET_V118_3;
}

size_t trexhip_network_blob_bytes(int32_t version, int32_t classes, int32_t channels, int32_t width, int32_t height) {
    return arch_blob_bytes(version, classes, channels, width, height);
}

int trexhip_identify_chunk_crops(trexhip_ctx* ctx, int32_t* crops) {
    if (!ctx || !crops) { set_error("trexhip_identify_chunk_crops: null argument"); return TREXHIP_E_INVALID; }
    const Net* net = static_cast<const Net*>(ctx->net);
    *crops = net && net->arch ? net->arch->plan.chunk : 0;
    return TREXHIP_OK;
}

int trexhip_network_channels(trexhip_ctx* ctx) {
    if (!ctx || !ctx->net) return 0;
    return static_cast<Net*>(ctx->net)->CH;
}

int trexhip_network_image_size(trexhip_ctx* ctx, int32_t* width, int32_t* height) {
    if (!ctx) { set_error("trexhip_network_image_size: null context"); return TREXHIP_E_INVALID; }
    const Net* net = static_cast<const Net*>(ctx->net);
    if (width) *width = net ? net->W : 0;
    if (height) *height = net ? net->H : 0;
    return TREXHIP_OK;
}

}

namespace trexhip {
void net_free(trexhip_ctx* ctx) {
    free_net(static_cast<Net*>(ctx->net)); ctx->net = nullptr;
    free_net(static_cast<Net*>(ctx->cat)); ctx->cat = nullptr;
}
}
```

### trex_amd/csrc/cnn_fused12rs.h

```cpp

__device__ __forceinline__ float rs_max3(const float a, const float b, const float c) { float r; asm("v_max3_f32 %0, %1, %2, %3" : "=v"(r) : "v"(a), "v"(b), "v"(c)); return r; }
__device__ __forceinline__ float rs_max3z(const float a, const float b) { float r; asm("v_max3_f32 %0, %1, %2, 0" : "=v"(r) : "v"(a), "v"(b)); return r; }
__device__ __forceinline__ float rs_max(const float a, const float b) { float r; asm("v_max_f32 %0, %1, %2" : "=v"(r) : "v"(a), "v"(b)); return r; }

__host__ __device__ constexpr int rs_ky(const int tau) { return ((tau % 20) % 10) / 2; }
__host__ __device__ constexpr int rs_pg(const int tau) {
    const int i = tau % 20;
    return tau / 20 == 0 ? (i / 10 == 0 ? 1 + i % 2 : (i % 2 ? 3 : 0)) : 2 * (i / 10) + i % 2;
}
__host__ __device__ constexpr int rs_pos(const int tau) { return tau / 20 == 0 ? (rs_pg(tau) == 3 ? 7 : rs_pg(tau)) : 3 + rs_pg(tau); }

struct W2xGeom {
    static constexpr int CO = 64, S = 40, TPP = 2 * SkipXGeom::WT, RPP = SkipXGeom::RPP, NR = SkipXGeom::NR;
    static constexpr int KH = 5, POOL = 2;
    static constexpr int ROWL = 4 * SkipXGeom::WT * 32;
    static constexpr int PLANE = (NR + 1) * ROWL, BUF = 2 * PLANE;
    static constexpr int PBUF_OFF = 2 * BUF;
    static constexpr int BV = 2 * 2 * CO;
    static_assert(RPP * TPP == 64 && NR == POOL * RPP + KH - 1, "64 M-slots, the V2 rows a pass reads");
};

template <class GG, int CHUNK_, int TPR_, int NW1_, int NT1_, bool WIN_>
struct W12RGeomT {
    using G = GG;
    static constexpr bool WIN = WIN_;
    static constexpr int CHUNK = CHUNK_, TPR = TPR_, NW1 = NW1_, NT1 = NT1_;
    static constexpr int SLOTS = G::RPP * G::TPP;
    static constexpr int E2_ITEMS = G::RPP * 80;
    static_assert(G::TPP == 2 * TPR && SLOTS <= 64 && CHUNK * 30 <= 256 && CHUNK * 4 * TPR <= 256, "items per stage: one per producer thread");
    static constexpr int IMG_PITCH = 88, IMG_ROWS = CHUNK * 6;
    static constexpr int PEP = 24, PPP = 48;
    static constexpr int PBE_OFF = G::PBUF_OFF, PBE_BYTES = G::RPP * PEP * 64 * 4;
    static constexpr int PBP_OFF = PBE_OFF + PBE_BYTES, PBP_BYTES = CHUNK * PPP * 16 * 4;
    static constexpr int IMG_OFF = PBP_OFF + PBP_BYTES, IMG_BYTES = IMG_ROWS * IMG_PITCH * 2;
    static constexpr int CTL_OFF = IMG_OFF + IMG_BYTES;
    static constexpr int WRES_OFF = CTL_OFF + 16, WTAP = 4096;
    static constexpr int NRES = (160 * 1024 - WRES_OFF) / WTAP;
    static constexpr int LDS_BYTES = WRES_OFF + NRES * WTAP;
    static_assert(LDS_BYTES <= 160 * 1024 && CTL_OFF % 16 == 0 && NRES >= 8 && NRES <= 40, "one workgroup per CU");
    static constexpr bool resident(const int tau) { return tau < NRES; }
};
using W12RGeom = W12RGeomT<W2bGeom, 6, 10, 20, 4, false>;
using W12XGeom = W12RGeomT<W2xGeom, SkipXGeom::CHUNK, SkipXGeom::WT, 2 * SkipXGeom::WT + 2, 3, true>;

static constexpr int RS_BD = 3, RS_TSPLIT = 20, RS_PRIO = 0x201;
template <class F>
__global__ __launch_bounds__(512) void k_conv12_rs(const uint8_t* __restrict__ crops , const uint4* __restrict__ w1tab ,
                                                   const float* __restrict__ bias1, const float inv_scale1,
                                                   const uint4* __restrict__ wp , const float* __restrict__ bias,
                                                   uint8_t* __restrict__ v3, const float out_scale, uint32_t* __restrict__ overflow,
                                                   const int n_crops, uint32_t* __restrict__ pass_ctr, const int PK ,
                                                   uint8_t* __restrict__ crop_flags ,
                                                   const int* __restrict__ list ,
                                                   const uint32_t* __restrict__ list_len, float* __restrict__ act2e) {
    using G = typename F::G;
    constexpr int CO = 64, S = 40;
    extern __shared__ __attribute__((aligned(16))) uint8_t ldsb[];
    const int tid = threadIdx.x, lane = tid & 63, wave = __builtin_amdgcn_readfirstlane(tid >> 6);
    const bool producer = wave >= 4;
    const int rt = tid & 255, rw = wave & 3;
    const int total_pairs = n_crops * (S / 2);
    const int total_rows = n_crops * S;
    const int n_pass = list ? (int)*list_len : (total_pairs + G::RPP - 1) / G::RPP;
    int slot = blockIdx.x * PK;
    if (slot >= n_pass) return;
#define RS_LIST(i_) list[(i_) < n_pass ? (i_) : n_pass]
    int pass = list ? RS_LIST(slot) : slot;
    int ahead = list ? RS_LIST(slot + 1) : 0;
    int* s_next = reinterpret_cast<int*>(ldsb + F::CTL_OFF);
    int tleft = PK;
    for (int i = tid; i < 4 * (G::ROWL / 16); i += 512) {
        const int pl = i / (G::ROWL / 16), o = i - pl * (G::ROWL / 16);
        *reinterpret_cast<uint4*>(ldsb + pl * G::PLANE + o * 16) = make_uint4(0, 0, 0, 0);
    }
    _Float16* img = reinterpret_cast<_Float16*>(ldsb + F::IMG_OFF);
    float* pbe = reinterpret_cast<float*>(ldsb + F::PBE_OFF);
    float* pbp = reinterpret_cast<float*>(ldsb + F::PBP_OFF);
    for (int i = tid; i < F::IMG_BYTES / 16; i += 512) reinterpret_cast<uint4*>(img)[i] = make_uint4(0, 0, 0, 0);
    for (int i = tid; i < (F::PBE_BYTES + F::PBP_BYTES) / 16; i += 512) reinterpret_cast<uint4*>(ldsb + F::PBE_OFF)[i] = make_uint4(0, 0, 0, 0);
    for (int i = tid; i < 40 * (F::WTAP / 16); i += 512) {
        const int tau = i / (F::WTAP / 16), u = i - tau * (F::WTAP / 16);
        if (F::resident(tau)) reinterpret_cast<uint4*>(ldsb + F::WRES_OFF + tau * F::WTAP)[u] = wp[(size_t)(rs_ky(tau) * 8 + rs_pos(tau)) * G::BV + u];
    }
    if (tid == 0) *s_next = ((int)atomicAdd(pass_ctr, 1u) + (int)gridDim.x) * PK;
    float ovfm = 0.f;
    auto flag_crops = [&](const int u_lo, const int u_hi, const int per_crop) {
        if (__any(!(ovfm < 4368.0f))) {
            if (lane == 0) { if (crop_flags) { crop_flags[u_lo / per_crop] = 1; crop_flags[u_hi / per_crop] = 1; } atomicOr(overflow, 1u); }
            ovfm = 0.f;
        }
    };
#define RS_BAR() asm volatile("s_waitcnt lgkmcnt(0)\n\ts_barrier" ::: "memory")
    auto rs_gp0 = [&](const int e) { if constexpr (F::WIN) { const SkipXPass x = skipx_unpack(e); return x.crop * (S / 2) + x.r0; } else return e * G::RPP; };
    auto rs_nrw = [&](const int e) {
        if constexpr (F::WIN) return skipx_unpack(e).rows;
        else { const int left = total_pairs - e * G::RPP; return left < G::RPP ? left : G::RPP; }
    };
    auto rs_row = [&](const int e, const int rp) {
        if constexpr (F::WIN) { const SkipXPass x = skipx_unpack(e); return x.crop * (S / 2) + x.r0 + (rp < x.rows ? rp : x.rows - 1); }
        else { const int gp = e * G::RPP + rp; return gp < total_pairs ? gp : total_pairs - 1; }
    };
    auto rs_t0 = [&](const int e) { if constexpr (F::WIN) return skipx_unpack(e).t0; else return 0; };
#define RS_ROWS(pass_, qmin_, nrows_)                                                                                            \
    do {                                                                                                                         \
        const int gp0_ = rs_gp0(pass_);                                                                                          \
        const SkipXV2 v_ = rs_v2_rows(gp0_, gp0_ + rs_nrw(pass_) - 1);                                                           \
        qmin_ = v_.qmin;                                                                                                         \
        nrows_ = v_.nrows;                                                                                                       \
    } while (0)
#define RS_NEXT(pass_, res_hi_, nslot_, next_, have_, lo_, hi_, extra_)                                                                \
    do {                                                                                                                         \
        const bool draw_ = tleft == 1;                                                                                           \
        nslot_ = draw_ ? __builtin_amdgcn_readfirstlane(*s_next) : slot + 1;                                                     \
        have_ = nslot_ < n_pass;                                                                                                 \
        next_ = nslot_;                                                                                                          \
        if (list) {                                                                                                              \
            next_ = draw_ ? RS_LIST(nslot_) : ahead;                                                                             \
            ahead = RS_LIST(nslot_ + 1);                                                                                         \
        }                                                                                                                        \
        lo_ = hi_ = 0;                                                                                                           \
        if (have_) {                                                                                                             \
            const int gn_ = rs_gp0(next_);                                                                                       \
            const bool follows_ = F::WIN ? gn_ == rs_gp0(pass_) + rs_nrw(pass_) : next_ == (pass_) + 1;                          \
            const SkipXV2 nw_ = rs_new_rows(follows_, res_hi_, gn_, gn_ + rs_nrw(next_) - 1);                                    \
            lo_ = nw_.qmin;                                                                                                      \
            hi_ = lo_ + nw_.nrows;                                                                                               \
        }                                                                                                                        \
        extra_ = rs_round_chunks(hi_ - lo_, F::CHUNK) - 1;                                                                       \
    } while (0)
    __syncthreads();

    int qmin, nrows;
    RS_ROWS(pass, qmin, nrows);
    if (producer) {
        __builtin_amdgcn_s_setprio((RS_PRIO >> 8) & 3);
        constexpr int CR = G::POOL + G::KH - 1;
        static_assert(CR == 6 && F::IMG_ROWS == F::CHUNK * CR, "the chunk's crop rows in LDS");
#define RS_ITEM(it_, c0_)                                                                                                        \
                const int vk = (it_) / 5, u = (it_) - vk * 5;                                                                    \
                const int v = vk / CR, k = vk - v * CR;                                                                          \
                int q = (c0_) + v;                                                                                               \
                q = q < total_rows ? q : total_rows - 1;                                                                         \
                const int crop = q / S, y = q - crop * S;                                                                        \
                const int iy = G::POOL * y - G::KH / 2 + k;
        auto p0_load = [&](const int c0, const int nr, uint4& px) {
            px = make_uint4(0, 0, 0, 0);
            if (rt < nr * 30) {
                RS_ITEM(rt, c0)
                if (iy >= 0 && iy < 80) px = *reinterpret_cast<const uint4*>(crops + ((size_t)crop * 80 + iy) * 80 + u * 16);
            }
        };
        auto p0_store = [&](const int nr, const uint4 px) {
            if (rt < nr * 30) {
                const int vk = rt / 5, u = rt - vk * 5;
                const uint32_t w4[4] = {px.x, px.y, px.z, px.w};
                uint32_t* d = reinterpret_cast<uint32_t*>(img + vk * F::IMG_PITCH + 2 + u * 16);
#pragma unroll
                for (int e = 0; e < 8; ++e) {
                    const uint32_t b0 = (w4[e >> 1] >> (16 * (e & 1))) & 0xffu, b1 = (w4[e >> 1] >> (16 * (e & 1) + 8)) & 0xffu;
                    d[e] = pack_h2((_Float16)(float)b0, (_Float16)(float)b1);
                }
            }
        };
        const float bz1 = bias1[lane & 15];
        uint4 bf[16];
#pragma unroll
        for (int f = 0; f < 4; ++f) {
            const uint4 b = w1tab[f * 64 + lane];
            bf[f] = b;
            bf[4 + f] = make_uint4(b.x << 16, __builtin_amdgcn_alignbit(b.y, b.x, 16), __builtin_amdgcn_alignbit(b.z, b.y, 16), __builtin_amdgcn_alignbit(b.w, b.z, 16));
            bf[8 + f] = make_uint4(0u, b.x, b.y, b.z);
            bf[12 + f] = make_uint4(0u, b.x << 16, __builtin_amdgcn_alignbit(b.y, b.x, 16), __builtin_amdgcn_alignbit(b.z, b.y, 16));
        }
        auto p1 = [&](const int nr, const int tw ) {
            const int r = lane & 15, q4 = lane >> 4;
            constexpr int NW = F::NW1;
            const int wb = F::WIN ? (2 * tw - 1 < 0 ? 0 : 2 * tw - 1 > 20 - NW ? 20 - NW : 2 * tw - 1) : 0;
            const int n_win = nr * NW, n_tiles = (n_win + 7) >> 3;
            constexpr int NT1 = F::NT1;
            for (int t0 = rw; t0 < n_tiles; t0 += 4 * NT1) {
                f16x8 a1[NT1], a2[NT1];
#pragma unroll
                for (int u = 0; u < NT1; ++u) {
                    const int tile = t0 + 4 * u < n_tiles ? t0 + 4 * u : t0;
                    int wdx = tile * 8 + (r >> 1);
                    wdx = wdx < n_win ? wdx : n_win - 1;
                    const int v = wdx / NW, x4 = (wb + wdx - v * NW) * 4;
                    const int row = v * 6 + (r & 1);
                    const _Float16* p1a = img + (row + q4) * F::IMG_PITCH + x4;
                    const _Float16* p2a = img + (row + 4) * F::IMG_PITCH + x4;
                    const uint2 l1 = *reinterpret_cast<const uint2*>(p1a), h1 = *reinterpret_cast<const uint2*>(p1a + 4);
                    const uint2 l2 = *reinterpret_cast<const uint2*>(p2a), h2 = *reinterpret_cast<const uint2*>(p2a + 4);
                    a1[u] = __builtin_bit_cast(f16x8, make_uint4(l1.x, l1.y, h1.x, h1.y));
                    a2[u] = __builtin_bit_cast(f16x8, make_uint4(l2.x, l2.y, h2.x, h2.y));
                }
                f32x4 acc[NT1][4];
#pragma unroll
                for (int u = 0; u < NT1; ++u)
#pragma unroll
                    for (int s = 0; s < 4; ++s) acc[u][s] = f32x4{0.f, 0.f, 0.f, 0.f};
#pragma unroll
                for (int m = 0; m < 4; ++m)
#pragma unroll
                    for (int u = 0; u < NT1; ++u)
#pragma unroll
                        for (int s = 0; s < 4; ++s)
                            acc[u][s] = __builtin_amdgcn_mfma_f32_16x16x32_f16((m & 1) ? a2[u] : a1[u], __builtin_bit_cast(f16x8, bf[s * 4 + (m == 0 ? 1 : m == 1 ? 3 : m == 2 ? 0 : 2)]), acc[u][s], 0, 0, 0);
#pragma unroll
                for (int u = 0; u < NT1; ++u) {
                    const int tile = t0 + 4 * u;
#pragma unroll
                    for (int pos = 0; pos < 2; ++pos) {
                        const int w = tile * 8 + 2 * q4 + pos;
                        const float t0 = acc[u][0][2 * pos] * inv_scale1 + bz1, t1 = acc[u][0][2 * pos + 1] * inv_scale1 + bz1;
                        const float t2 = acc[u][1][2 * pos] * inv_scale1 + bz1, t3 = acc[u][1][2 * pos + 1] * inv_scale1 + bz1;
                        const float t4 = acc[u][2][2 * pos] * inv_scale1 + bz1, t5 = acc[u][2][2 * pos + 1] * inv_scale1 + bz1;
                        const float t6 = acc[u][3][2 * pos] * inv_scale1 + bz1, t7 = acc[u][3][2 * pos + 1] * inv_scale1 + bz1;
                        const float v0 = rs_max3z(rs_max3(t0, t1, t2), t3), v1 = rs_max3z(rs_max3(t4, t5, t6), t7);
                        if (tile < n_tiles && w < n_win) {
                            ovfm = rs_max3(ovfm, v0, v1);
                            const int vr = w / NW, px = vr * F::PPP + 4 + 2 * (wb + w - vr * NW);
                            float* o = pbp + ((px & ~15) | ((px & 3) << 2) | ((px >> 2) & 3)) * 16 + r;
                            o[0] = v0;
                            o[64] = v1;
                        }
                    }
                }
            }
        };
        auto p2 = [&](const int c0, const int nr, const int tw) {
            if (rt < nr * (4 * F::TPR)) {
                const int v = rt / (4 * F::TPR), rem = rt - v * (4 * F::TPR), tx = rem >> 2, quad = rem & 3;
                const int q = c0 + v;
                const int slot = q % G::NR + 1, rot = w2b_rot(slot);
                float4 d[8];
#pragma unroll
                for (int k = 0; k < 8; ++k) {
                    const int px = v * F::PPP + 4 * (tw + tx) + 2 + k;
                    d[k] = *reinterpret_cast<const float4*>(pbp + ((px & ~15) | ((px & 3) << 2) | ((px >> 2) & 3)) * 16 + quad * 4);
                }
                float ua[8], ub[8], uc[8], ud[8];
                wino_bt(d[0].x, d[1].x, d[2].x, d[3].x, d[4].x, d[5].x, d[6].x, d[7].x, ua);
                wino_bt(d[0].y, d[1].y, d[2].y, d[3].y, d[4].y, d[5].y, d[6].y, d[7].y, ub);
                wino_bt(d[0].z, d[1].z, d[2].z, d[3].z, d[4].z, d[5].z, d[6].z, d[7].z, uc);
                wino_bt(d[0].w, d[1].w, d[2].w, d[3].w, d[4].w, d[5].w, d[6].w, d[7].w, ud);
                uint8_t* rowb = ldsb + slot * G::ROWL + (quad & 1) * 8;
#pragma unroll
                for (int p = 0; p < 8; ++p) {
                    const int pi = p < 3 ? p : (p == 7 ? 3 : p + 1);
                    const int w = (pi & 3) * (2 * F::TPR) + tx * 2 + (quad >> 1);
                    uint8_t* dst = rowb + (pi >> 2) * G::BUF + ((w & ~15) | ((w + rot) & 15)) * 16;
                    uint32_t l0, l1, m0, m1;
                    split2h_pair(ua[p], ub[p], l0, m0);
                    split2h_pair(uc[p], ud[p], l1, m1);
                    *reinterpret_cast<uint2*>(dst) = make_uint2(l0, l1);
                    *reinterpret_cast<uint2*>(dst + G::PLANE) = make_uint2(m0, m1);
                }
            }
        };
        auto e2 = [&](const int ep) {
            const int egp0 = rs_gp0(ep), enrw = rs_nrw(ep);
            if constexpr (!F::WIN) {
                if (act2e) {
                    for (int i = rt; i < G::RPP * 20 * 16; i += 256) {
                        const int rp = i / 320, rem = i - rp * 320, x = rem >> 4, c4 = rem & 15;
                        if (rp < enrw)
                            *reinterpret_cast<float4*>(act2e + ((size_t)(egp0 + rp) * 20 + x) * 64 + c4 * 4) =
                                *reinterpret_cast<const float4*>(pbe + (rp * F::PEP + 2 + x) * 64 + c4 * 4);
                    }
                }
            }
            auto e2_item = [&](const int it) {
                const int rp = it / 80, rem = it - rp * 80, tx = rem >> 4, quad = rem & 15;
                const int gp = egp0 + rp;
                if (rp < enrw) {
                    float4 d[8];
                    const float* src = pbe + (rp * F::PEP + 4 * tx) * 64 + quad * 4;
#pragma unroll
                    for (int k = 0; k < 8; ++k) d[k] = *reinterpret_cast<const float4*>(src + k * 64);
                    float ua[8], ub[8], uc[8], ud[8];
                    wino_bt(d[0].x, d[1].x, d[2].x, d[3].x, d[4].x, d[5].x, d[6].x, d[7].x, ua);
                    wino_bt(d[0].y, d[1].y, d[2].y, d[3].y, d[4].y, d[5].y, d[6].y, d[7].y, ub);
                    wino_bt(d[0].z, d[1].z, d[2].z, d[3].z, d[4].z, d[5].z, d[6].z, d[7].z, uc);
                    wino_bt(d[0].w, d[1].w, d[2].w, d[3].w, d[4].w, d[5].w, d[6].w, d[7].w, ud);
                    uint8_t* dst = v3 + (size_t)gp * V3_ROWB + (quad >> 2) * V3_CHUNKB + tx * 32 + (quad & 3) * 8;
#pragma unroll
                    for (int p = 0; p < 8; ++p) {
                        uint32_t l0, l1, m0, m1;
                        split2h_pair(ua[p], ub[p], l0, m0);
                        split2h_pair(uc[p], ud[p], l1, m1);
                        *reinterpret_cast<uint2*>(dst + v3_off(p, 0)) = make_uint2(l0, l1);
                        *reinterpret_cast<uint2*>(dst + v3_off(p, 1)) = make_uint2(m0, m1);
                    }
                }
            };
            static_assert(F::E2_ITEMS <= 256 || (F::WIN && F::E2_ITEMS <= 320), "items of the V3 transform");
            if (rt < (F::E2_ITEMS < 256 ? F::E2_ITEMS : 256)) e2_item(rt);
            if constexpr (F::E2_ITEMS > 256) { if (rt < F::E2_ITEMS - 256) e2_item(rt + 256); }
        };
        auto bg_load = [&](const int ps, float4& bg) {
            if constexpr (F::WIN) {
                const SkipXPass x = skipx_unpack(ps);
                const int rp = rt >> 6, k = (rt >> 4) & 3, c4 = rt & 15;
                const int px = k < 2 * x.t0 ? k : k + 2 * F::TPR;
                bg = make_float4(0.f, 0.f, 0.f, 0.f);
                if (rp < x.rows) bg = *reinterpret_cast<const float4*>(act2e + ((x.r0 + rp) * 20 + px) * 64 + c4 * 4);
            }
        };
        auto bg_store = [&](const int ps, const float4 bg) {
            if constexpr (F::WIN) {
                static_assert(!F::WIN || (G::RPP * (20 - 2 * F::TPR) * 16 == 256), "one item per producer thread");
                const int t0 = skipx_unpack(ps).t0;
                const int rp = rt >> 6, k = (rt >> 4) & 3, c4 = rt & 15;
                const int px = k < 2 * t0 ? k : k + 2 * F::TPR;
                *reinterpret_cast<float4*>(pbe + (rp * F::PEP + 2 + px) * 64 + c4 * 4) = bg;
            }
        };
        for (int c = 0, c0 = qmin; c < rs_round_chunks(nrows, F::CHUNK); ++c, c0 += F::CHUNK) {
            const int nr = qmin + nrows - c0 < F::CHUNK ? qmin + nrows - c0 : F::CHUNK;
            uint4 px;
            p0_load(c0, nr, px);
            p0_store(nr, px);
            RS_BAR();
            p1(nr, rs_t0(pass));
            flag_crops(c0, c0 + nr - 1, S);
            RS_BAR();
            p2(c0, nr, rs_t0(pass));
            RS_BAR();
        }
        int res_hi = qmin + nrows;
        int prev = -1;
        for (;;) {
            int next_slot, next_pass, lo, hi, extra;
            bool have_next;
            RS_NEXT(pass, res_hi, next_slot, next_pass, have_next, lo, hi, extra);
            const int tn = have_next ? rs_t0(next_pass) : 0;
            const int nr0 = hi - lo < F::CHUNK ? hi - lo : F::CHUNK;
            uint4 px;
            p0_load(lo, nr0, px);
            if (prev >= 0) e2(prev);
            p0_store(nr0, px);
            RS_BAR();
            float4 bg = make_float4(0.f, 0.f, 0.f, 0.f);
            bg_load(pass, bg);
            p1(nr0, tn);
            if (nr0 > 0) flag_crops(lo, lo + nr0 - 1 < total_rows ? lo + nr0 - 1 : total_rows - 1, S);
            bg_store(pass, bg);
            RS_BAR();
            p2(lo, nr0, tn);
            RS_BAR();
            for (int c = 0, c0 = lo + F::CHUNK; c < extra; ++c, c0 += F::CHUNK) {
                const int nr = hi - c0 < F::CHUNK ? hi - c0 : F::CHUNK;
                p0_load(c0, nr, px);
                p0_store(nr, px);
                RS_BAR();
                p1(nr, tn);
                flag_crops(c0, c0 + nr - 1 < total_rows ? c0 + nr - 1 : total_rows - 1, S);
                RS_BAR();
                p2(c0, nr, tn);
                RS_BAR();
            }
            prev = pass;
            if (!have_next) break;
            res_hi = hi;
            tleft = tleft == 1 ? PK : tleft - 1;
            pass = next_pass;
            slot = next_slot;
        }
        e2(prev);
#undef RS_ITEM
    } else {
        const int j = lane & 31, h = lane >> 5;
        const int n = rw & 1, mg = rw >> 1;
        const __amdgpu_buffer_rsrc_t wrs = make_rsrc(wp, (uint32_t)(40 * G::BV * 16));
        const int boff = (h * CO + n * 32 + j) * 16;
        const int co = n * 32 + j;
        const float bz = bias[co];
        for (int c = 0; c < rs_round_chunks(nrows, F::CHUNK); ++c) { RS_BAR(); RS_BAR(); RS_BAR(); }
        int res_hi = qmin + nrows;
#define W2_POS(tau_) rs_pos(tau_)
#define W2_BOFF(tau_) ((rs_ky(tau_) * 8 + W2_POS(tau_)) * G::BV * 16)
        uint4 bq[8][2];
        const uint8_t* wres = ldsb + F::WRES_OFF + boff;
#define RS_WFETCH(dst_, tau_)                                                                                                    \
        do {                                                                                                                     \
            if (F::resident(tau_)) {                                                                                             \
                dst_[0] = *reinterpret_cast<const uint4*>(wres + (tau_) * F::WTAP);                                              \
                dst_[1] = *reinterpret_cast<const uint4*>(wres + (tau_) * F::WTAP + 2 * CO * 16);                                \
            } else {                                                                                                             \
                dst_[0] = buf_load16(wrs, boff, W2_BOFF(tau_));                                                                  \
                dst_[1] = buf_load16(wrs, boff, W2_BOFF(tau_) + 2 * CO * 16);                                                    \
            }                                                                                                                    \
        } while (0)
#pragma unroll
        for (int t = 0; t < RS_BD; ++t) RS_WFETCH(bq[t], t);
        int aoff[G::KH][4], srow[G::KH], srot[G::KH];
        int wh[4], wl[4];
        {
            int s_ = mg * 32 + j;
            s_ = s_ < G::RPP * G::TPP ? s_ : G::RPP * G::TPP - 1;
            const int r2_ = s_ % G::TPP, tx_ = r2_ >> 1;
#pragma unroll
            for (int pg = 0; pg < 4; ++pg) { const int w_ = pg * (2 * F::TPR) + tx_ * 2 + h; wh[pg] = (w_ & ~15) * 16; wl[pg] = w_ & 15; }
        }
#define RS_AOFF(ps_)                                                                                                             \
        do {                                                                                                                     \
            int s_ = mg * 32 + j;                                                                                                \
            s_ = s_ < G::RPP * G::TPP ? s_ : G::RPP * G::TPP - 1;                                                                \
            const int rp_ = s_ / G::TPP, r2_ = s_ - rp_ * G::TPP;                                                                \
            const int gp_ = rs_row(ps_, rp_);                                                                                    \
            const int qo_ = 2 * gp_ + (r2_ & 1), y_ = qo_ % S;                                                                   \
            _Pragma("unroll") for (int ky = 0; ky < G::KH; ++ky) {                                                               \
                const int iy_ = y_ + ky - G::KH / 2;                                                                             \
                const int slot_ = (iy_ >= 0 && iy_ < S) ? (qo_ + ky - G::KH / 2) % G::NR + 1 : 0;                                \
                srow[ky] = slot_ * G::ROWL; srot[ky] = w2b_rot(slot_);                                                           \
            }                                                                                                                    \
        } while (0)
#define RS_AUNIT(tau_) do { if ((tau_) < 20) aoff[rs_ky(tau_)][rs_pg(tau_)] = srow[rs_ky(tau_)] + (wh[rs_pg(tau_)] | (((wl[rs_pg(tau_)] + srot[rs_ky(tau_)]) & 15) << 4)); } while (0)
        RS_AOFF(pass);
        for (;;) {
            int next_slot, next_pass, lo, hi, extra;
            bool have_next;
            RS_NEXT(pass, res_hi, next_slot, next_pass, have_next, lo, hi, extra);
            const bool draw = tleft == 1;
            uint32_t ticket = 0;
            if (draw && tid == 0) asm volatile("global_atomic_add %0, %1, %2, off sc0" : "=v"(ticket) : "v"(pass_ctr), "v"(1u) : "memory");
            f32x16 acc[8];
            const f32x16 zero16 = {0.f, 0.f, 0.f, 0.f, 0.f, 0.f, 0.f, 0.f, 0.f, 0.f, 0.f, 0.f, 0.f, 0.f, 0.f, 0.f};
            __builtin_amdgcn_s_setprio((RS_PRIO >> 4) & 3);
            uint4 af[2][2];
            auto rs_fold = [&](const int tau) {
#define RS_PIN(x_) asm volatile("" : "+v"(x_))
                if (tau >= 11 && tau < 19) {
#pragma unroll
                    for (int r = 2 * (tau - 11); r < 2 * (tau - 11) + 2; ++r) {
                        float e = acc[1][r] + acc[2][r], o = acc[1][r] - acc[2][r];
                        RS_PIN(e); RS_PIN(o); acc[1][r] = e; acc[2][r] = o;
                    }
                }
                if (tau >= 21 && tau < 29) {
#pragma unroll
                    for (int r = 2 * (tau - 21); r < 2 * (tau - 21) + 2; ++r) {
                        float a = acc[0][r] + acc[1][r], d = acc[2][r] + acc[7][r];
                        RS_PIN(a); RS_PIN(d); acc[0][r] = a; acc[7][r] = d;
                    }
                }
                if (tau >= 31 && tau < 39) {
#pragma unroll
                    for (int r = 2 * (tau - 31); r < 2 * (tau - 31) + 2; ++r) {
                        const float e2 = acc[3][r] + acc[4][r], o2 = acc[3][r] - acc[4][r];
                        float a = acc[0][r] + e2, b = acc[2][r] + 2.f * o2, c = acc[1][r] + 4.f * e2, d = acc[7][r] + 8.f * o2;
                        RS_PIN(a); RS_PIN(b); RS_PIN(c); RS_PIN(d); acc[0][r] = a; acc[2][r] = b; acc[1][r] = c; acc[7][r] = d;
                    }
                }
#undef RS_PIN
            };
#define RS_AREAD(dst_, tau_)                                                                                                     \
            do {                                                                                                                 \
                const uint8_t* an_ = ldsb + ((tau_) / 20) * G::BUF + aoff[rs_ky(tau_)][rs_pg(tau_)];                             \
                dst_[0] = *reinterpret_cast<const uint4*>(an_);                                                                  \
                dst_[1] = *reinterpret_cast<const uint4*>(an_ + G::PLANE);                                                       \
            } while (0)
#define RS_TAP(tau)                                                                                                              \
            do {                                                                                                                 \
                const int tl = (tau) % 20;                                                                                       \
                if ((tau) + 1 < 40) { RS_AUNIT((tau) + 1); RS_AREAD(af[((tau) + 1) % 2], (tau) + 1); }                           \
                RS_WFETCH(bq[((tau) + RS_BD) % 8], ((tau) + RS_BD) % 40);                                                        \
                const int p = W2_POS(tau);                                                                                       \
                const f16x8 b1 = __builtin_bit_cast(f16x8, bq[(tau) % 8][0]), b2 = __builtin_bit_cast(f16x8, bq[(tau) % 8][1]); \
                const f16x8 a1 = __builtin_bit_cast(f16x8, af[(tau) % 2][0]), a2 = __builtin_bit_cast(f16x8, af[(tau) % 2][1]); \
                acc[p] = mfma16(a2, b1, rs_ky(tau) == 0 ? zero16 : acc[p]);              \
                acc[p] = mfma16(a1, b2, acc[p]);                                                                                 \
                acc[p] = mfma16(a1, b1, acc[p]);                                                                                 \
                rs_fold(tau);                                                                                                    \
                __builtin_amdgcn_sched_group_barrier(0x100, 2, 0);                                                               \
                __builtin_amdgcn_sched_group_barrier(0x020, 2, 0);                                                               \
                _Pragma("unroll") for (int g = 0; g < 3; ++g) {                                                                  \
                    __builtin_amdgcn_sched_group_barrier(0x008, 1, 0);                                                           \
                    __builtin_amdgcn_sched_group_barrier(0x006, 6, 0);                                                           \
                }                                                                                                                \
                __builtin_amdgcn_sched_barrier(0);                                                                               \
            } while (0)
            RS_AUNIT(0);
            RS_AREAD(af[0], 0);
#pragma clang loop unroll(full)
            for (int tau = 0; tau < RS_TSPLIT; ++tau) RS_TAP(tau);
            RS_BAR();
#pragma clang loop unroll(full)
            for (int tau = RS_TSPLIT; tau < 40; ++tau) RS_TAP(tau);
            if (draw) {
                asm volatile("s_waitcnt vmcnt(0)" : "+v"(ticket) :: "memory");
                if (tid == 0) *s_next = ((int)ticket + (int)gridDim.x) * PK;
            }
            RS_BAR();
            __builtin_amdgcn_s_setprio(RS_PRIO & 3);
            const int t0c = rs_t0(pass);
            f32x16 y0 = acc[0], y1 = acc[2], y2 = acc[1], y3 = acc[7];
            {
                const f32x16 e3 = acc[5] + acc[6], o3 = acc[5] - acc[6];
                y0 += e3; y1 += 0.5f * o3; y2 += 0.25f * e3; y3 += 0.125f * o3;
            }
#pragma unroll
            for (int rr = 0; rr < 8; ++rr) {
                const int r = 2 * rr;
                const int s = mg * 32 + (r & 3) + 8 * (r >> 2) + 4 * h;
                const float v0 = rs_max(rs_max3(y0[r], y1[r], y0[r + 1]), y1[r + 1]);
                const float v1 = rs_max(rs_max3(y2[r], y3[r], y2[r + 1]), y3[r + 1]);
                if (s < G::RPP * G::TPP) {
                    const int rp = s / G::TPP, tx = (s - rp * G::TPP) >> 1;
                    const float a0 = fmaxf(v0 * out_scale + bz, 0.f), a1 = fmaxf(v1 * out_scale + bz, 0.f);
                    ovfm = rs_max3(ovfm, a0, a1);
                    float* o = pbe + (rp * F::PEP + 2 + 2 * (t0c + tx)) * 64 + co;
                    o[0] = a0;
                    o[64] = a1;
                }
            }
            { const int g0 = rs_gp0(pass); flag_crops(g0, g0 + rs_nrw(pass) - 1, S / 2); }
            if (have_next) RS_AOFF(next_pass);
            RS_BAR();
            for (int c = 0; c < extra; ++c) { RS_BAR(); RS_BAR(); RS_BAR(); }
            if (!have_next) break;
            res_hi = hi;
            tleft = tleft == 1 ? PK : tleft - 1;
            pass = next_pass;
            slot = next_slot;
        }
#undef RS_TAP
#undef RS_WFETCH
#undef RS_AOFF
#undef RS_AUNIT
#undef RS_AREAD
#undef W2_POS
#undef W2_BOFF
    }
#undef RS_NEXT
#undef RS_LIST
#undef RS_ROWS
#undef RS_BAR
    if (__any(!(ovfm < 4368.0f)) && lane == 0) atomicOr(overflow, 3u);
}
```

### trex_amd/csrc/cnn_net.h

```cpp
#pragma once
#include "internal.h"
#include "cnn_plan.h"
#include "cnn_skip.h"
#include "cnn_skip_words.h"
#include "cnn_skipx.h"
#include <tuple>

namespace trexhip {

struct ArchNet;

struct Net {
    int classes = 0, W = 0, H = 0, CH = 0, max_crops = 0;
    ArchNet* arch = nullptr;
    uint4 *w2s = nullptr, *w3s = nullptr;
    uint4 *w2h = nullptr, *w3h = nullptr;
    float inv2h = 1.f, inv3h = 1.f;
    uint4 *w2w = nullptr, *w3w = nullptr;
    float inv2w = 1.f, inv3w = 1.f;
    uint4* wf1h = nullptr;
    float invf1h = 1.f;
    uint4* w1h = nullptr;
    float inv1h = 1.f;
    uint32_t* d_ovf = nullptr;
    uint8_t* d_ovfc = nullptr;
    float *w1 = nullptr, *b1 = nullptr, *w2 = nullptr, *b2 = nullptr, *w3 = nullptr, *b3 = nullptr;
    float *wf1 = nullptr, *bf1 = nullptr, *lng = nullptr, *lnb = nullptr, *wf2t = nullptr, *bf2 = nullptr;
    float *act1 = nullptr, *act2 = nullptr, *act3 = nullptr, *fc1 = nullptr, *probs = nullptr, *logits = nullptr;
    uint8_t *v2 = nullptr, *v3 = nullptr;
    uint8_t* crops = nullptr;
    uint8_t* v3e = nullptr;
    uint32_t* d_skip = nullptr;
    int2* skip_bands = nullptr;
    uint32_t* skip_counts = nullptr;
    int* skip_list = nullptr;
    float* act2e = nullptr;
    int2* skipx_cols = nullptr;
    int* skipx_list = nullptr;
    float* act3e = nullptr;
    uint2* skip3_counts = nullptr;
    uint32_t* skip3_tcounts = nullptr;
    int* skip3_desc = nullptr;
    uint32_t* skip3_rows = nullptr;
    float* fc1e = nullptr;
    int* fc1_list = nullptr;
    int last_fc1_n = 0;
    float* h_probs = nullptr;
    Mem weights, batch;
    using GraphKey = std::tuple<const uint8_t* , int , float* , float* , int , int , hipStream_t>;
    struct GraphEntry { GraphKey key; hipGraphExec_t exec; uint64_t used; hipEvent_t last; int seen; };
    std::vector<GraphEntry> graphs;
    bool graphs_ok = true;
    uint64_t tick = 0;
    bool ovf_clean = true;
    int last_mode = -1;
    uint32_t* ovf(const int word) const { return d_ovf + word; }
};

struct LdsAttr { const void* fn; int bytes; };
std::vector<LdsAttr>& lds_attrs();
template <class... A>
struct Kern {
    void (*fn)(A...);
    int threads, lds;
    Kern(void (*f)(A...), const int threads_, const int lds_ = 0, const bool attr = true) : fn(f), threads(threads_), lds(lds_) {
        if (lds && attr) lds_attrs().push_back({reinterpret_cast<const void*>(f), lds});
    }
    template <class... B>
    void operator()(hipStream_t s, const dim3 grid, B... args) const { hipLaunchKernelGGL(fn, grid, dim3(threads), lds, s, static_cast<A>(args)...); }
};
template <class K> struct ByChannels {
    K one, three;
    const K& operator[](const int CH) const { return CH == 1 ? one : three; }
};
template <class K> ByChannels(K, K) -> ByChannels<K>;

void any_conv1(hipStream_t s, const Net& net, const CnnPlan& p, const uint8_t* d_crops);
void any_conv(hipStream_t s, const Net& net, const CnnPlan& p, int layer, int mode, const uint32_t* guard);

}
```

### trex_amd/csrc/cnn_plan.h

```cpp
#pragma once
#include <algorithm>
#include "../../include/trexhip.h"
#include "cnn_geom.h"
#include "cnn_skip_words.h"
#include "cnn_skipx.h"

namespace trexhip {

enum : int {
    GEOM_FP32_ACT = 0xfff,
    GEOM_NO_SKIPX = 1 << 23,
    GEOM_DENSE_FC1 = 1 << 24,
    GEOM_V3_COPY = 1 << 25,
    GEOM_DENSE_CONV3 = 1 << 26,
    GEOM_NO_SKIP = 1 << 27,
    GEOM_TWO_KERNEL = 1 << 28,
    GEOM_ROLE_SPLIT = 1 << 29,
    GEOM_FUSED_2WG = 1 << 30,
    GEOM_MASK = GEOM_FP32_ACT | GEOM_NO_SKIPX | GEOM_DENSE_FC1 | GEOM_V3_COPY | GEOM_DENSE_CONV3 | GEOM_NO_SKIP | GEOM_TWO_KERNEL | GEOM_ROLE_SPLIT | GEOM_FUSED_2WG
};

enum class Chain { ROLE_SPLIT, FUSED_2WG, TWO_KERNEL, FP32_ACT, EXACT, ANY_SIZE };
enum class Conv1 { FUSED , WPRE, MFMA, VALU, ANY };
enum class Fc1 { EXACT , SPLIT1 , SPLIT4  };
enum class Head { SMALL , BIG  };

struct Launch { int grid, items; };

struct CnnPlan {
    Chain chain;
    Conv1 conv1;
    int conv1_grid;
    Launch conv2, conv3;
    int pk2;
    int n_big3;
    Fc1 fc1;
    int fc1_grid, planes, K;
    Head head;
    int head_grid;
    bool rerun;
    bool head_plans;
    bool rerun_conv1;
    Launch r_conv2, r_conv3;
    int r_fc1_grid, r_head_grid;
    AnyTiles t2, t3;
    int tx1, t1;
    bool skip;
    bool skip3;
    int skip3_grid;
    Launch act3_fill;
    bool v3_direct;
    bool fc1_listed;
    bool skipx;
};

inline int ceil_div(const int a, const int b) { return (a + b - 1) / b; }
inline Launch whole(const int items) { return {items, items}; }
inline Launch guarded(const int items, const int n_cus) { return {std::min(items, 4 * n_cus), items}; }

inline CnnPlan cnn_plan(const int W, const int H, const int CH, const int mode, const bool aligned, const int geom, const int n, const int n_cus) {
    using GW = WinoGeom<64, 128, 20, 2>;
    CnnPlan p{};
    const bool h16 = mode == TREXHIP_CNN_FP16X3;
    const int P = (H / 8) * (W / 8);
    p.planes = FC1_KSPLIT;
    while (P % p.planes) --p.planes;
    p.K = 128 * P;
    p.fc1 = Fc1::EXACT;
    p.fc1_grid = p.r_fc1_grid = ceil_div(n, 32);
    p.head = Head::BIG;
    p.head_grid = p.r_head_grid = ceil_div(n, 4 * HEAD_CPW);
    p.rerun = h16;

    if (W != 80 || H != 80) {
        p.chain = Chain::ANY_SIZE;
        p.conv1 = Conv1::ANY;
        p.tx1 = ceil_div(W / 2, C1T);
        p.t1 = ceil_div(H / 2, C1T) * p.tx1;
        p.conv1_grid = n * p.t1;
        p.t2 = any_tiles(H / 4, W / 4);
        p.t3 = any_tiles(H / 8, W / 8);
        p.conv2 = whole(n * p.t2.tiles);
        p.conv3 = whole(n * p.t3.tiles);
        p.r_conv2 = guarded(p.conv2.items, n_cus);
        p.r_conv3 = guarded(p.conv3.items, n_cus);
        return p;
    }

    const bool pre = h16 && aligned && (geom & GEOM_FP32_ACT) == 0;
    const bool fused12 = pre && CH == 1 && !(geom & GEOM_TWO_KERNEL);
    const bool role_split = fused12 && !(geom & GEOM_FUSED_2WG) && ((geom & GEOM_ROLE_SPLIT) || n >= 3200);
    p.chain = role_split ? Chain::ROLE_SPLIT : fused12 ? Chain::FUSED_2WG : pre ? Chain::TWO_KERNEL : h16 ? Chain::FP32_ACT : Chain::EXACT;
    p.conv1 = fused12 ? Conv1::FUSED : pre ? Conv1::WPRE : aligned ? Conv1::MFMA : Conv1::VALU;
    p.conv1_grid = n;
    p.skip = role_split && !(geom & GEOM_NO_SKIP);
    p.skip3 = p.skip && !(geom & GEOM_DENSE_CONV3);
    p.skipx = p.skip && !(geom & GEOM_NO_SKIPX) && n < SKIPX_MAX_CROPS;
    if (p.skip3) {
        p.skip3_grid = ceil_div(ceil_div(n, 32 ), 256);
        p.act3_fill = {ceil_div(n, 16), n};
        p.v3_direct = !(geom & GEOM_V3_COPY) && skip3_direct_fits((long long)n * SkipGeom::V3_ROWS);
    }

    const int n_pass2 = ceil_div(n * 20, W2bGeom::RPP), n_pass3 = ceil_div(n * GW::TPC, GW::MB);
    if (fused12) {
        const int wgs = role_split ? n_cus : 2 * n_cus;
        p.pk2 = std::max(1, std::min(role_split ? 32 : 16, n_pass2 / (wgs * 4)));
        p.conv2 = {std::min(ceil_div(n_pass2, p.pk2), wgs), n_pass2};
    }
    else if (pre) p.conv2 = {std::min(n_pass2, 2 * n_cus), n_pass2};
    else if (h16) p.conv2 = whole(n * ConvGeomS<16, 64, 40, 8, 4>::BPC);
    else if (mode == TREXHIP_CNN_FP32) p.conv2 = whole(n * ConvGeom<16, 64, 40, 20, 16>::BPC);
    else p.conv2 = whole(n * ConvGeomB<16, 64, 40, 10, SPLIT_NP>::BPC);
    if (pre) {
        p.n_big3 = n_pass3 >= 16 * n_cus ? (int)((long long)n_pass3 * 7 / 8) / 4 : 0;
        p.conv3 = {std::min(p.n_big3 + (n_pass3 - p.n_big3 * 4), n_cus), n_pass3};
    }
    else if (h16) p.conv3 = {std::min(n_pass3, n_cus), n_pass3};
    else if (mode == TREXHIP_CNN_FP32) p.conv3 = whole(n * ConvGeom<64, 128, 20, 20, 32>::BPC);
    else p.conv3 = whole(n * ConvGeomB<64, 128, 20, 20, SPLIT_NP>::BPC);

    const bool small = n <= 1024;
    if (h16) {
        p.fc1 = small ? Fc1::SPLIT1 : Fc1::SPLIT4;
        if (!small) p.fc1_grid = ceil_div(n, 128);
    }
    if (small) { p.head = Head::SMALL; p.head_grid = ceil_div(n, 4); }
    p.fc1_listed = p.skip3 && p.fc1 == Fc1::SPLIT4 && p.head == Head::BIG && !(geom & GEOM_DENSE_FC1);
    p.head_plans = h16 && small;
    p.rerun_conv1 = pre;
    p.r_conv2 = guarded(n * ConvGeomB<16, 64, 40, 10, SPLIT_NP>::BPC, n_cus);
    p.r_conv3 = guarded(n * ConvGeomB<64, 128, 20, 4, SPLIT_NP>::BPC, n_cus);
    return p;
}

}
```

### trex_amd/csrc/cnn_skip_kernels.h

```cpp
#pragma once

static constexpr int SKIP_LB = 1024;
static constexpr int SKIP_PAD = 1;
static constexpr int SKIP_FILL_TB = 256;

__global__ __launch_bounds__(256) void k_crop_bands(const uint8_t* __restrict__ crops, const int n, int2* __restrict__ bands, int2* __restrict__ cols) {
    using G = SkipGeom;
    constexpr int UPR = 80 / 16, UNITS = G::CROP_ROWS * UPR;
    const int lane = threadIdx.x & 63, crop = blockIdx.x * 4 + (threadIdx.x >> 6);
    if (crop >= n) return;
    const uint4* src = reinterpret_cast<const uint4*>(crops + (size_t)crop * (G::CROP_ROWS * 80));
    uint4 px[(UNITS + 63) / 64];
#pragma unroll
    for (int k = 0; k < (UNITS + 63) / 64; ++k) {
        const int i = lane + 64 * k;
        px[k] = i < UNITS ? src[i] : make_uint4(0, 0, 0, 0);
    }
    int y0 = G::CROP_ROWS, y1 = -1;
#pragma unroll
    for (int k = 0; k < (UNITS + 63) / 64; ++k) {
        if (px[k].x | px[k].y | px[k].z | px[k].w) {
            const int row = (lane + 64 * k) / UPR;
            y0 = row < y0 ? row : y0;
            y1 = row > y1 ? row : y1;
        }
    }
#pragma unroll
    for (int d = 32; d >= 1; d >>= 1) {
        const int a = __shfl_xor(y0, d), b = __shfl_xor(y1, d);
        y0 = a < y0 ? a : y0;
        y1 = b > y1 ? b : y1;
    }
    if (lane == 0) bands[crop] = make_int2(y0, y1);
    if (cols) {
        int x0 = 80, x1 = -1;
#pragma unroll
        for (int k = 0; k < (UNITS + 63) / 64; ++k) {
            const int c0 = ((lane + 64 * k) % UPR) * 16;
            const uint32_t w4[4] = {px[k].x, px[k].y, px[k].z, px[k].w};
#pragma unroll
            for (int j = 0; j < 4; ++j) {
                if (w4[j]) {
                    const int a = c0 + 4 * j + ((__ffs((int)w4[j]) - 1) >> 3), b = c0 + 4 * j + ((31 - __clz((int)w4[j])) >> 3);
                    x0 = a < x0 ? a : x0;
                    x1 = b > x1 ? b : x1;
                }
            }
        }
#pragma unroll
        for (int d = 32; d >= 1; d >>= 1) {
            const int a = __shfl_xor(x0, d), b = __shfl_xor(x1, d);
            x0 = a < x0 ? a : x0;
            x1 = b > x1 ? b : x1;
        }
        if (lane == 0) cols[crop] = make_int2(x0, x1);
    }
}

struct SkipBandsOf {
    const int2* bands;
    __host__ __device__ SkipBand operator()(const int crop) const { const int2 b = bands[crop]; return {b.x, b.y}; }
};
__device__ __forceinline__ bool skip_needed(const int p, const int total_pairs, const int2* __restrict__ bands, const bool all) {
    return all || skip_pass_needed(p, total_pairs, SkipBandsOf{bands});
}
struct SkipXWinOf {
    const int2* cols; bool all;
    __host__ __device__ int operator()(const int crop) const {
        if (!cols) return -1;
        const int2 c = cols[crop];
        return skipx_window({c.x, c.y}, all);
    }
};
struct SkipXItem { bool full, need; int wpasses, t0; SkipRows rows; };
__device__ __forceinline__ SkipXItem skipx_item(const int i, const int n, const int2* __restrict__ bands, const int2* __restrict__ cols, const bool all) {
    const int total_pairs = n * SkipGeom::V3_ROWS, n_pass = (total_pairs + SkipGeom::RPP - 1) / SkipGeom::RPP;
    const bool none = all || !cols;
    SkipXItem it{false, false, 0, -1, {1, 0}};
    if (i < n_pass) {
        it.need = skip_needed(i, total_pairs, bands, all);
        it.full = it.need && (none || skipx_full_needed(i, total_pairs, SkipBandsOf{bands}, SkipXWinOf{cols, all}));
    }
    if (i < n) {
        it.t0 = SkipXWinOf{cols, all}(i);
        const int2 b = bands[i];
        it.rows = skip_rows({b.x, b.y});
        it.wpasses = it.t0 >= 0 ? skipx_passes(it.rows) : 0;
    }
    return it;
}
__global__ __launch_bounds__(SKIP_LB) void k_pass_count(const int2* __restrict__ bands, const int2* __restrict__ cols, const int n,
                                                        const uint32_t* __restrict__ words, uint32_t* __restrict__ counts) {
    __shared__ uint32_t s_cnt[4];
    if (threadIdx.x < 4) s_cnt[threadIdx.x] = 0;
    __syncthreads();
    const SkipXItem it = skipx_item(blockIdx.x * SKIP_LB + threadIdx.x, n, bands, cols, words[SK_EMPTY_RANGE] != 0);
    uint32_t v[4] = {it.full ? 1u : 0u, it.need ? 1u : 0u, (uint32_t)it.wpasses, it.wpasses ? 1u : 0u};
#pragma unroll
    for (int k = 0; k < 4; ++k) {
#pragma unroll
        for (int d = 32; d >= 1; d >>= 1) v[k] += __shfl_xor(v[k], d);
        if ((threadIdx.x & 63) == 0 && v[k]) atomicAdd(&s_cnt[k], v[k]);
    }
    __syncthreads();
    if (threadIdx.x < 4) counts[blockIdx.x * 4 + threadIdx.x] = s_cnt[threadIdx.x];
}
__global__ __launch_bounds__(SKIP_LB) void k_pass_list(const int2* __restrict__ bands, const int2* __restrict__ cols, const int n,
                                                       uint32_t* __restrict__ words, const uint32_t* __restrict__ counts, int* __restrict__ list,
                                                       int* __restrict__ wlist) {
    __shared__ uint32_t s_base[4], s_wave[2][SKIP_LB / 64];
    const int total_pairs = n * SkipGeom::V3_ROWS, n_pass = (total_pairs + SkipGeom::RPP - 1) / SkipGeom::RPP;
    const int tid = threadIdx.x, lane = tid & 63, wave = tid >> 6;
    const int i = blockIdx.x * SKIP_LB + tid;
    if (tid < 4) s_base[tid] = 0;
    __syncthreads();
    uint32_t part[4] = {0, 0, 0, 0};
    for (int b = tid; b < (int)blockIdx.x; b += SKIP_LB) {
#pragma unroll
        for (int k = 0; k < 4; ++k) part[k] += counts[b * 4 + k];
    }
#pragma unroll
    for (int k = 0; k < 4; ++k) {
#pragma unroll
        for (int d = 32; d >= 1; d >>= 1) part[k] += __shfl_xor(part[k], d);
        if (lane == 0 && part[k]) atomicAdd(&s_base[k], part[k]);
    }
    const SkipXItem it = skipx_item(i, n, bands, cols, words[SK_EMPTY_RANGE] != 0);
    uint32_t sc[2] = {it.full ? 1u : 0u, (uint32_t)it.wpasses};
#pragma unroll
    for (int k = 0; k < 2; ++k) {
#pragma unroll
        for (int d = 1; d < 64; d <<= 1) { const uint32_t v = __shfl_up(sc[k], d); if (lane >= d) sc[k] += v; }
        if (lane == 63) s_wave[k][wave] = sc[k];
    }
    __syncthreads();
#pragma unroll
    for (int k = 0; k < 2; ++k) {
        uint32_t before = 0;
        for (int w = 0; w < wave; ++w) before += s_wave[k][w];
        sc[k] += before;
    }
    if (it.full) list[s_base[0] + sc[0] - 1] = i;
    if (it.wpasses) {
        const uint32_t at = s_base[2] + sc[1] - (uint32_t)it.wpasses;
        for (int k = 0; k < it.wpasses; ++k) wlist[at + k] = skipx_pack(skipx_pass(i, it.rows, it.t0, k));
    }
    if (blockIdx.x == gridDim.x - 1 && tid == SKIP_LB - 1) {
        const uint32_t full = s_base[0] + sc[0], wp = s_base[2] + sc[1];
        uint32_t need = s_base[1], wc = s_base[3];
        for (int k = 0; k < 2; ++k) { const uint32_t c = counts[blockIdx.x * 4 + 1 + 2 * k]; if (k) wc += c; else need += c; }
        for (int k = 0; k < SKIP_PAD; ++k) list[full + k] = n_pass;
        const bool last_need = skip_needed(n_pass - 1, total_pairs, bands, words[SK_EMPTY_RANGE] != 0);
        const uint32_t listed_rows = need * SkipGeom::RPP - (last_need ? (uint32_t)(n_pass * SkipGeom::RPP - total_pairs) : 0u);
        words[SK_LEN] = need; words[SK_NPASS] = (uint32_t)n_pass; words[SK_FILLED] = (uint32_t)total_pairs - listed_rows;
        if (cols) {
            for (int k = 0; k < SKIP_PAD; ++k) wlist[wp + k] = 0;
            words[SKX_CROPS] = wc; words[SKX_PASSES] = wp; words[SKX_FULL] = full; words[SKX_CTR] = 0;
        }
    }
}
__global__ __launch_bounds__(SKIP_FILL_TB) void k_v3_fill(const int2* __restrict__ bands, const int2* __restrict__ cols, const int n, const uint32_t* __restrict__ words,
                                                          const uint4* __restrict__ v3e, uint4* __restrict__ v3, const int direct) {
    using G = SkipGeom;
    constexpr int ROWQ = V3_ROWB / 16;
    __shared__ unsigned long long s_fill[SKIP_FILL_TB / 64];
    if (direct && words[SK3_USE]) return;
    const bool all = words[SK_EMPTY_RANGE] != 0;
    const int total_pairs = n * G::V3_ROWS, tid = threadIdx.x, gp0 = blockIdx.x * SKIP_FILL_TB;
    {
        const int gp = gp0 + tid;
        bool fill = false;
        if (gp < total_pairs && !all) {
            const int crop = gp / G::V3_ROWS, r = gp - crop * G::V3_ROWS;
            if (!cols) fill = !skip_pass_needed(gp / G::RPP, total_pairs, SkipBandsOf{bands});
            else {
                const SkipXWinOf win{cols, all};
                bool computed = false;
                if (win(crop) >= 0) { const int2 b = bands[crop]; const SkipRows need = skip_rows({b.x, b.y}); computed = r >= need.lo && r <= need.hi; }
                fill = !computed && !skipx_full_needed(gp / G::RPP, total_pairs, SkipBandsOf{bands}, win);
            }
        }
        const unsigned long long m = __ballot(fill);
        if ((tid & 63) == 0) s_fill[tid >> 6] = m;
    }
    __syncthreads();
    for (int w = 0; w < SKIP_FILL_TB / 64; ++w) {
        unsigned long long m = s_fill[w];
        while (m) {
            const int gp = gp0 + w * 64 + __ffsll((long long)m) - 1;
            m &= m - 1;
            for (int q = tid; q < ROWQ; q += SKIP_FILL_TB) v3[(size_t)gp * ROWQ + q] = v3e[(gp % G::V3_ROWS) * ROWQ + q];
        }
    }
}

static constexpr int SKIP3_TB = 256;

__device__ __forceinline__ void skip3_stage_runs(const int2* __restrict__ bands, const int n, const bool all, uint16_t* s_run) {
    using G = Skip3Geom;
    const int c0 = blockIdx.x * SKIP3_TB * G::BLOCK;
    constexpr int U = 8;
    static_assert(G::BLOCK % U == 0, "whole groups of loads");
    for (int i0 = threadIdx.x; i0 < SKIP3_TB * G::BLOCK; i0 += U * SKIP3_TB) {
        int2 b[U];
#pragma unroll
        for (int u = 0; u < U; ++u) {
            const int i = i0 + u * SKIP3_TB;
            b[u] = c0 + i < n ? bands[c0 + i] : make_int2(SKIP_BAND_NONE.y0, SKIP_BAND_NONE.y1);
        }
#pragma unroll
        for (int u = 0; u < U; ++u) {
            const int i = i0 + u * SKIP3_TB;
            const SkipPairs r = all && c0 + i < n ? SkipPairs{0, G::PAIRS - 1} : skip3_pairs({b[u].x, b[u].y});
            s_run[(i % G::BLOCK) * SKIP3_TB + i / G::BLOCK] = (uint16_t)(r.lo <= r.hi ? r.lo | (r.hi - r.lo + 1) << 8 : 0);
        }
    }
    __syncthreads();
}
template <class E>
__device__ __forceinline__ int skip3_walk(const uint16_t* s_run, const int blk, int& passes, E&& emit) {
    using G = Skip3Geom;
    Skip3Pass p{};
    int listed = 0;
#pragma unroll 1
    for (int k = 0; k < G::BLOCK; ++k) {
        const int r = s_run[k * SKIP3_TB + threadIdx.x], len = r >> 8;
        if (len) {
            listed += len;
            skip3_add_run(p, passes, (blk * G::BLOCK + k) * G::PAIRS + (r & 0xff), len, emit);
        }
    }
    skip3_flush(p, passes, emit);
    return listed;
}

__global__ __launch_bounds__(SKIP3_TB) void k_pair_count(const int2* __restrict__ bands, const int n, const uint32_t* __restrict__ words,
                                                         uint2* __restrict__ counts ,
                                                         uint32_t* __restrict__ tcounts ) {
    __shared__ uint32_t s_pass, s_pair;
    __shared__ uint16_t s_run[SKIP3_TB * Skip3Geom::BLOCK];
// ... 146 lines not shown
```

### trex_amd/csrc/cnn_skip_words.h

```cpp
#pragma once
#include "cnn_skip3.h"

namespace trexhip {

enum : int {
    SK_EMPTY_RANGE = 0,
    SK_EMPTY_CTR = 1,
    SK_LEN = 2,
    SK_NPASS = 3,
    SK_FILLED = 4,
    SK3_PAIRS = 8,
    SK3_LISTED = 9,
    SK3_PASSES = 10,
    SK3_FILLED = 11,
    SK3_USE = 12,
    SK3_EMPTY_CTR = 13,
    SK3_FC1E_RANGE = 14,
    SK3_FC1_LEN = 16,
    SK3_LAST = SK3_FC1_LEN + Skip3Geom::PAIRS - 1,
    SKX_CROPS = 26,
    SKX_PASSES = 27,
    SKX_FULL = 28,
    SKX_CTR = 29,
    SK_WORDS = 32
};
static_assert(SK_FILLED < SK3_PAIRS && SK3_LAST < SKX_CROPS && SKX_CTR < SK_WORDS, "no word twice, the last one inside the table");

}
```

### trex_amd/csrc/cnn_skipx.h

```cpp
#pragma once
#include "cnn_skip.h"

namespace trexhip {

struct SkipXGeom {
    static constexpr int TILE = 4;
    static constexpr int TILES = W2bGeom::S / TILE;
    static constexpr int WT = 8, WR = 8;
    static constexpr int RPP = WR / SkipGeom::POOL;
    static constexpr int NR = WR + W2bGeom::KH - 1;
    static constexpr int CHUNK = WR;
    static constexpr int V2_LO0 = -(W2bGeom::KH / 2), V2_HI0 = TILE - 1 + W2bGeom::KH / 2;
    static constexpr int STEP = TILE * SkipGeom::POOL, LO0 = skip_layer_lo(V2_LO0), HI0 = skip_layer_hi(V2_HI0);
    static_assert(STEP == 8 && LO0 == -6 && HI0 == 13, "tile t reads crop columns 8 t - 6 .. 8 t + 13");
    static_assert(WT * WR == 64 && WT <= TILES && RPP * SkipGeom::POOL == WR, "one MFMA M block, whole pooled rows");
};

struct SkipTiles { int lo, hi; };
TREXHIP_HD constexpr SkipTiles skipx_tiles(const SkipBand b) {
    using X = SkipXGeom;
    if (b.y0 > b.y1) return {1, 0};
    const int lo = b.y0 <= X::HI0 ? 0 : (b.y0 - X::HI0 + X::STEP - 1) / X::STEP;
    const int hi = (b.y1 - X::LO0) / X::STEP;
    return {lo, hi < X::TILES - 1 ? hi : X::TILES - 1};
}

TREXHIP_HD constexpr int skipx_window(const SkipBand cols, const bool empty_out_of_range) {
    using X = SkipXGeom;
    if (empty_out_of_range) return -1;
    const SkipTiles t = skipx_tiles(cols);
    if (t.lo > t.hi) return 0;
    if (t.hi - t.lo + 1 > X::WT) return -1;
    return t.lo < X::TILES - X::WT ? t.lo : X::TILES - X::WT;
}

struct SkipXPass { int crop, r0, rows, t0; };
static constexpr int SKIPX_MAX_CROPS = 1 << 22;
TREXHIP_HD constexpr int skipx_pack(const SkipXPass p) { return p.crop << 9 | p.r0 << 4 | (p.rows - 1) << 2 | p.t0; }
TREXHIP_HD constexpr SkipXPass skipx_unpack(const int e) { return {e >> 9, (e >> 4) & 31, ((e >> 2) & 3) + 1, e & 3}; }
static_assert(SkipXGeom::RPP <= 4 && SkipXGeom::TILES - SkipXGeom::WT <= 3 && SkipGeom::V3_ROWS <= 32, "the fields of an entry");

TREXHIP_HD constexpr int skipx_passes(const SkipRows need) {
    return need.lo > need.hi ? 0 : (need.hi - need.lo + 1 + SkipXGeom::RPP - 1) / SkipXGeom::RPP;
}
TREXHIP_HD constexpr SkipXPass skipx_pass(const int crop, const SkipRows need, const int t0, const int k ) {
    const int r0 = need.lo + k * SkipXGeom::RPP, left = need.hi - r0 + 1;
    return {crop, r0, left < SkipXGeom::RPP ? left : SkipXGeom::RPP, t0};
}

template <class B, class W>
TREXHIP_HD constexpr bool skipx_full_needed(const int p, const int total_pairs, const B& band, const W& win) {
    using G = SkipGeom;
    for (int gp = p * G::RPP; gp < (p + 1) * G::RPP && gp < total_pairs; ++gp) {
        const int crop = gp / G::V3_ROWS, r = gp - crop * G::V3_ROWS;
        if (win(crop) >= 0) continue;
        const SkipRows need = skip_rows(band(crop));
        if (r >= need.lo && r <= need.hi) return true;
    }
    return false;
}

TREXHIP_HD constexpr int rs_round_chunks(const int new_rows, const int chunk) { return new_rows <= chunk ? 1 : (new_rows + chunk - 1) / chunk; }
TREXHIP_HD constexpr int rs_round_stages(const int new_rows, const int chunk) { return 3 * rs_round_chunks(new_rows, chunk); }

struct SkipXV2 { int qmin, nrows; };
TREXHIP_HD constexpr SkipXV2 rs_v2_rows(const int gp0, const int gpl) {
    constexpr int S = W2bGeom::S;
    const int y0 = (2 * gp0) % S, yl = (2 * gpl) % S + 1;
    const int qmin = 2 * gp0 - (y0 >= 2 ? 2 : 0);
    return {qmin, 2 * gpl + 1 + (yl + 2 <= S - 1 ? 2 : 0) - qmin + 1};
}
TREXHIP_HD constexpr SkipXV2 rs_new_rows(const bool follows, const int res_hi, const int gp0n, const int gpln) {
    const SkipXV2 v = rs_v2_rows(gp0n, gpln);
    const int lo = (follows && res_hi > v.qmin) ? res_hi : v.qmin;
    return {lo, v.qmin + v.nrows - lo};
}

}
```

Baseline: 42320.

## Skip computing background V2 rows in windowed conv1-2 passes using precomputed table

Adds a per-pass V2 row range (derived from each crop's column band) so the windowed fused conv1+conv2 kernel only computes the V2 rows that can hold foreground, and fills the rest from a precomputed background tile table (bgtab) built at weight-load time. The intent is to cut conv1/conv2 MFMA work on rows that are pure background. It adds a second per-pass list (skipx_rows), extra counters and stats, more LDS per plane, and more complex round scheduling, which could cost extra overhead when few rows are skipped.

```diff
diff --git a/include/trexhip.h b/include/trexhip.h
--- a/include/trexhip.h
+++ b/include/trexhip.h
@@ -6,7 +6,7 @@
 extern "C" {
 #endif
 
-#define TREXHIP_ABI_VERSION 22
+#define TREXHIP_ABI_VERSION 23
 
 enum {
     TREXHIP_OK = 0,
@@ -265,6 +265,8 @@
 int trexhip_identify_skip3_stats(trexhip_ctx* ctx, uint32_t* pairs, uint32_t* listed, uint32_t* passes, uint64_t* bytes_filled);
 
 int trexhip_identify_skipx_stats(trexhip_ctx* ctx, uint32_t* crops_windowed, uint32_t* windowed_passes, uint32_t* full_passes);
+
+int trexhip_identify_bgrow_stats(trexhip_ctx* ctx, uint32_t* rows_read, uint32_t* rows_made);
 
 int trexhip_identify_fc1_stats(trexhip_ctx* ctx, uint32_t* rows, uint32_t* listed);
 
diff --git a/trex_amd/capi.py b/trex_amd/capi.py
--- a/trex_amd/capi.py
+++ b/trex_amd/capi.py
@@ -179,7 +179,7 @@
     "trexhip_set_stream", "trexhip_get_live_params", "trexhip_update_params", "trexhip_set_background", "trexhip_set_background_device", "trexhip_set_background_color", "trexhip_set_background_color_device", "trexhip_generate_average_device", "trexhip_get_background", "trexhip_segment_device",
     "trexhip_segment", "trexhip_segment_color", "trexhip_segment_color_device", "trexhip_rethreshold_device", "trexhip_rethreshold_per_blob_device", "trexhip_fetch_rethreshold", "trexhip_fetch", "trexhip_device_view_get", "trexhip_synchronize",
     "trexhip_profile_enable", "trexhip_profile_read", "trexhip_profile_reset",
-    "trexhip_default_posture_params", "trexhip_posture_device", "trexhip_posture_auto_device", "trexhip_pack_frames_v6_device", "trexhip_crops_device", "trexhip_pixel_channels", "trexhip_device_alloc", "trexhip_device_free", "trexhip_copy_to_host", "trexhip_copy_to_device", "trexhip_crops_transformed_device", "trexhip_crops_posture_device", "trexhip_default_midline_params", "trexhip_midline_device", "trexhip_midline_movement_device", "trexhip_default_split_params", "trexhip_split_search_device", "trexhip_export_id_table_device", "trexhip_export_id_table_ex_device", "trexhip_load_weights", "trexhip_set_identity_precision", "trexhip_num_classes", "trexhip_identify_device", "trexhip_identify", "trexhip_identify_guard_stats", "trexhip_identify_skip_stats", "trexhip_identify_skip3_stats", "trexhip_identify_skipx_stats", "trexhip_identify_fc1_stats",
+    "trexhip_default_posture_params", "trexhip_posture_device", "trexhip_posture_auto_device", "trexhip_pack_frames_v6_device", "trexhip_crops_device", "trexhip_pixel_channels", "trexhip_device_alloc", "trexhip_device_free", "trexhip_copy_to_host", "trexhip_copy_to_device", "trexhip_crops_transformed_device", "trexhip_crops_posture_device", "trexhip_default_midline_params", "trexhip_midline_device", "trexhip_midline_movement_device", "trexhip_default_split_params", "trexhip_split_search_device", "trexhip_export_id_table_device", "trexhip_export_id_table_ex_device", "trexhip_load_weights", "trexhip_set_identity_precision", "trexhip_num_classes", "trexhip_identify_device", "trexhip_identify", "trexhip_identify_guard_stats", "trexhip_identify_skip_stats", "trexhip_identify_skip3_stats", "trexhip_identify_skipx_stats", "trexhip_identify_bgrow_stats", "trexhip_identify_fc1_stats",
     "trexhip_weight_blob_bytes", "trexhip_trainer_create", "trexhip_trainer_destroy", "trexhip_trainer_set_lr", "trexhip_trainer_steps", "trexhip_trainer_image_size", "trexhip_trainer_version", "trexhip_trainer_keep_mask_bytes", "trexhip_train_step_device", "trexhip_train_step", "trexhip_train_eval_device", "trexhip_train_eval", "trexhip_trainer_read", "trexhip_trainer_export",
     "trexhip_default_augment_params", "trexhip_augment_device",
     "trexhip_train_predict_device", "trexhip_validation_metrics_device", "trexhip_class_averages_device",
@@ -271,6 +271,7 @@
         L.trexhip_identify_guard_stats.argtypes = [C.c_void_p, C.POINTER(C.c_uint32), C.POINTER(C.c_uint32)]
         L.trexhip_identify_skip_stats.argtypes = [C.c_void_p, C.POINTER(C.c_uint32), C.POINTER(C.c_uint32), C.POINTER(C.c_uint64)]
         L.trexhip_identify_skipx_stats.argtypes = [C.c_void_p, C.POINTER(C.c_uint32), C.POINTER(C.c_uint32), C.POINTER(C.c_uint32)]
+        L.trexhip_identify_bgrow_stats.argtypes = [C.c_void_p, C.POINTER(C.c_uint32), C.POINTER(C.c_uint32)]
         L.trexhip_identify_skip3_stats.argtypes = [C.c_void_p, C.POINTER(C.c_uint32), C.POINTER(C.c_uint32), C.POINTER(C.c_uint32), C.POINTER(C.c_uint64)]
         L.trexhip_identify_fc1_stats.argtypes = [C.c_void_p, C.POINTER(C.c_uint32), C.POINTER(C.c_uint32)]
         L.trexhip_weight_blob_bytes.argtypes = [C.c_int32, C.c_int32]
@@ -632,6 +633,11 @@
         _check(lib().trexhip_identify_skipx_stats(self._h, C.byref(a), C.byref(b), C.byref(c)))
         return int(a.value), int(b.value), int(c.value)
 
+    def bgrow_stats(self):
+        a, b = C.c_uint32(0), C.c_uint32(0)
+        _check(lib().trexhip_identify_bgrow_stats(self._h, C.byref(a), C.byref(b)))
+        return int(a.value), int(b.value)
+
     def skip3_stats(self):
         a, b, c, d = C.c_uint32(0), C.c_uint32(0), C.c_uint32(0), C.c_uint64(0)
         _check(lib().trexhip_identify_skip3_stats(self._h, C.byref(a), C.byref(b), C.byref(c), C.byref(d)))
diff --git a/trex_amd/csrc/cnn.hip b/trex_amd/csrc/cnn.hip
--- a/trex_amd/csrc/cnn.hip
+++ b/trex_amd/csrc/cnn.hip
@@ -1289,10 +1289,11 @@
     if (net->v3e) {
         const size_t n_pass = (N * SkipGeom::V3_ROWS + SkipGeom::RPP - 1) / SkipGeom::RPP;
         TRY(B.device_bytes(&net->skip_bands, N * sizeof(int2), who));
-        TRY(B.device_bytes(&net->skip_counts, ((n_pass + SKIP_LB - 1) / SKIP_LB) * 4 * 4, who));
+        TRY(B.device_bytes(&net->skip_counts, ((n_pass + SKIP_LB - 1) / SKIP_LB) * SKIP_NCNT * 4, who));
         TRY(B.device_bytes(&net->skip_list, (n_pass + SKIP_PAD) * 4, who));
         TRY(B.device_bytes(&net->skipx_cols, N * sizeof(int2), who));
         TRY(B.device_bytes(&net->skipx_list, (N * skipx_passes({0, SkipGeom::V3_ROWS - 1}) + SKIP_PAD) * 4, who));
+        TRY(B.device_bytes(&net->skipx_rows, (N * skipx_passes({0, SkipGeom::V3_ROWS - 1}) + SKIP_PAD) * 4, who));
         const size_t blocks3 = (N + Skip3Geom::BLOCK - 1) / Skip3Geom::BLOCK;
         TRY(B.device_bytes(&net->skip3_counts, ((blocks3 + SKIP3_TB - 1) / SKIP3_TB) * sizeof(uint2), who));
         TRY(B.device_bytes(&net->skip3_tcounts, blocks3 * 4, who));
@@ -1411,6 +1412,7 @@
     if (rc == TREXHIP_OK) rc = net->weights.device_bytes(&net->fc1e, (size_t)FC1_KSPLIT * 128 * 4, who);
     if (rc == TREXHIP_OK) rc = net->weights.device_bytes(&net->d_skip, SK_WORDS * 4, who);
     if (rc == TREXHIP_OK) rc = net->weights.device_bytes(&net->act2e, (size_t)SkipGeom::V3_ROWS * 20 * 64 * 4, who);
+    if (rc == TREXHIP_OK) rc = net->weights.device_bytes(&net->bgtab, (size_t)W2xGeom::NBG * W2xGeom::BG_UNITS * sizeof(uint4), who);
     if (rc == TREXHIP_OK) rc = net->weights.device_bytes(&zero, SkipGeom::CROP_ROWS * 80, who);
     if (rc != TREXHIP_OK) return rc;
     const CnnPlan p = cnn_plan(80, 80, 1, TREXHIP_CNN_FP16X3, true, GEOM_ROLE_SPLIT | GEOM_NO_SKIP, 1, ctx->n_cus);
@@ -1418,7 +1420,11 @@
     TH_CHECK_HIP(hipMemsetAsync(net->d_skip, 0, SK_WORDS * 4, ctx->stream));
     TH_CHECK_HIP(hipMemsetAsync(zero, 0, SkipGeom::CROP_ROWS * 80, ctx->stream));
     K_CONV12_RS(ctx->stream, p.conv2.grid, zero, net->w1h, net->b1, net->inv1h, net->w2w, net->b2, net->v3e, net->inv2w, net->d_skip + SK_EMPTY_RANGE, 1,
-                net->d_skip + SK_EMPTY_CTR, p.pk2, nullptr, nullptr, nullptr, net->act2e);
+                net->d_skip + SK_EMPTY_CTR, p.pk2, nullptr, nullptr, nullptr, net->act2e, nullptr, nullptr);
+    TH_CHECK_HIP(hipGetLastError());
+    TH_CHECK_HIP(hipFuncSetAttribute(reinterpret_cast<const void*>(K_CONV12_RSX.fn), hipFuncAttributeMaxDynamicSharedMemorySize, K_CONV12_RSX.lds));
+    K_CONV12_RSX(ctx->stream, 1, zero, net->w1h, net->b1, net->inv1h, net->w2w, net->b2, net->v3e, net->inv2w, net->d_skip + SK_EMPTY_RANGE, 1,
+                 net->d_skip + SKX_CTR, 1, nullptr, nullptr, nullptr, net->act2e, nullptr, net->bgtab);
     TH_CHECK_HIP(hipGetLastError());
     TH_CHECK_HIP(hipFuncSetAttribute(reinterpret_cast<const void*>(K_CONV3_WPAIR.fn), hipFuncAttributeMaxDynamicSharedMemorySize, K_CONV3_WPAIR.lds));
     K_CONV3_WPAIR(ctx->stream, p.conv3.grid, net->v3e, net->w3w, net->b3, net->act3e, net->inv3w, 1, net->d_skip + SK3_EMPTY_CTR, p.n_big3, nullptr, nullptr, nullptr);
@@ -1443,8 +1449,8 @@
     const int n = f.n, lb = ceil_div(p.conv2.items, SKIP_LB);
     int2* cols = p.skipx ? net.skipx_cols : nullptr;
     K_CROP_BANDS(f.s, ceil_div(n, 4), f.crops, n, net.skip_bands, cols);
-    K_PASS_COUNT(f.s, lb, net.skip_bands, cols, n, net.d_skip, net.skip_counts);
-    K_PASS_LIST(f.s, lb, net.skip_bands, cols, n, net.d_skip, net.skip_counts, net.skip_list, net.skipx_list);
+    K_PASS_COUNT(f.s, lb, net.skip_bands, cols, n, net.d_skip, net.skip_counts, (int)p.bgrows);
+    K_PASS_LIST(f.s, lb, net.skip_bands, cols, n, net.d_skip, net.skip_counts, net.skip_list, net.skipx_list, net.skipx_rows, (int)p.bgrows);
     if (p.skip3) {
         K_PAIR_COUNT(f.s, p.skip3_grid, net.skip_bands, n, net.d_skip, net.skip3_counts, net.skip3_tcounts);
         K_PAIR_LIST(f.s, p.skip3_grid, net.skip_bands, n, net.d_skip, net.skip3_counts, net.skip3_tcounts, net.skip3_desc);
@@ -1478,9 +1484,9 @@
             if (p.skip) launch_skip_prep(f, direct);
             if (p.skipx)
                 K_CONV12_RSX(s, p.conv2.grid, d_crops, net.w1h, net.b1, net.inv1h, net.w2w, net.b2, net.v3, net.inv2w, net.ovf(OVF_RANGE), n, net.d_skip + SKX_CTR,
-                             p.pk2, net.d_ovfc, net.skipx_list, net.d_skip + SKX_PASSES, net.act2e);
+                             p.pk2, net.d_ovfc, net.skipx_list, net.d_skip + SKX_PASSES, net.act2e, net.skipx_rows, net.bgtab);
             K_CONV12_RS(s, p.conv2.grid, d_crops, net.w1h, net.b1, net.inv1h, net.w2w, net.b2, net.v3, net.inv2w, net.ovf(OVF_RANGE), n, net.ovf(OVF_PASS2),
-                        p.pk2, net.d_ovfc, p.skip ? net.skip_list : nullptr, p.skip ? net.d_skip + (p.skipx ? SKX_FULL : SK_LEN) : nullptr, nullptr);
+                        p.pk2, net.d_ovfc, p.skip ? net.skip_list : nullptr, p.skip ? net.d_skip + (p.skipx ? SKX_FULL : SK_LEN) : nullptr, nullptr, nullptr, nullptr);
             break;
         case Chain::FUSED_2WG:
             K_CONV12_WPRE(s, p.conv2.grid, d_crops, net.w1h, net.b1, net.inv1h, net.w2w, net.b2, net.v3, net.inv2w, net.ovf(OVF_RANGE), n, net.ovf(OVF_PASS2),
@@ -1674,6 +1680,14 @@
     return TREXHIP_OK;
 }
 
+int trexhip_identify_bgrow_stats(trexhip_ctx* ctx, uint32_t* rows_read, uint32_t* rows_made) {
+    uint32_t w[SK_WORDS];
+    if (const int rc = read_skip_words(ctx, "trexhip_identify_bgrow_stats", w)) return rc;
+    if (rows_read) *rows_read = w[SKX_V2_READ];
+    if (rows_made) *rows_made = w[SKX_V2_MADE];
+    return TREXHIP_OK;
+}
+
 int trexhip_identify_skip3_stats(trexhip_ctx* ctx, uint32_t* pairs, uint32_t* listed, uint32_t* passes, uint64_t* bytes_filled) {
     uint32_t w[SK_WORDS];
     if (const int rc = read_skip_words(ctx, "trexhip_identify_skip3_stats", w)) return rc;
diff --git a/trex_amd/csrc/cnn_fused12rs.h b/trex_amd/csrc/cnn_fused12rs.h
--- a/trex_amd/csrc/cnn_fused12rs.h
+++ b/trex_amd/csrc/cnn_fused12rs.h
@@ -14,10 +14,11 @@
     static constexpr int CO = 64, S = 40, TPP = 2 * SkipXGeom::WT, RPP = SkipXGeom::RPP, NR = SkipXGeom::NR;
     static constexpr int KH = 5, POOL = 2;
     static constexpr int ROWL = 4 * SkipXGeom::WT * 32;
-    static constexpr int PLANE = (NR + 1) * ROWL, BUF = 2 * PLANE;
+    static constexpr int NBG = SkipXGeom::TILES - SkipXGeom::WT + 1, BG_SLOT = NR + 1, BG_UNITS = 4 * ROWL / 16;
+    static constexpr int PLANE = (NR + 2) * ROWL, BUF = 2 * PLANE;
     static constexpr int PBUF_OFF = 2 * BUF;
     static constexpr int BV = 2 * 2 * CO;
-    static_assert(RPP * TPP == 64 && NR == POOL * RPP + KH - 1, "64 M-slots, the V2 rows a pass reads");
+    static_assert(RPP * TPP == 64 && NR == POOL * RPP + KH - 1 && NBG == 3 && BG_UNITS == 256, "64 M-slots, the V2 rows a pass reads, the background slot: a unit per producer thread");
 };
 
 template <class GG, int CHUNK_, int TPR_, int NW1_, int NT1_, bool WIN_>
@@ -52,7 +53,9 @@
                                                    const int n_crops, uint32_t* __restrict__ pass_ctr, const int PK ,
                                                    uint8_t* __restrict__ crop_flags ,
                                                    const int* __restrict__ list ,
-                                                   const uint32_t* __restrict__ list_len, float* __restrict__ act2e) {
+                                                   const uint32_t* __restrict__ list_len, float* __restrict__ act2e,
+                                                   const int* __restrict__ vrows ,
+                                                   uint4* __restrict__ bgtab ) {
     using G = typename F::G;
     constexpr int CO = 64, S = 40;
     extern __shared__ __attribute__((aligned(16))) uint8_t ldsb[];
@@ -67,6 +70,8 @@
 #define RS_LIST(i_) list[(i_) < n_pass ? (i_) : n_pass]
     int pass = list ? RS_LIST(slot) : slot;
     int ahead = list ? RS_LIST(slot + 1) : 0;
+    auto rs_vrows = [&](const int i) { if constexpr (F::WIN) return vrows ? vrows[i < n_pass ? i : n_pass] : 0; else return 0; };
+    int vr = rs_vrows(slot), vr_ahead = rs_vrows(slot + 1);
     int* s_next = reinterpret_cast<int*>(ldsb + F::CTL_OFF);
     int tleft = PK;
     for (int i = tid; i < 4 * (G::ROWL / 16); i += 512) {
@@ -101,37 +106,31 @@
         else { const int gp = e * G::RPP + rp; return gp < total_pairs ? gp : total_pairs - 1; }
     };
     auto rs_t0 = [&](const int e) { if constexpr (F::WIN) return skipx_unpack(e).t0; else return 0; };
-#define RS_ROWS(pass_, qmin_, nrows_)                                                                                            \
-    do {                                                                                                                         \
-        const int gp0_ = rs_gp0(pass_);                                                                                          \
-        const SkipXV2 v_ = rs_v2_rows(gp0_, gp0_ + rs_nrw(pass_) - 1);                                                           \
-        qmin_ = v_.qmin;                                                                                                         \
-        nrows_ = v_.nrows;                                                                                                       \
-    } while (0)
-#define RS_NEXT(pass_, res_hi_, nslot_, next_, have_, lo_, hi_, extra_)                                                                \
+#define RS_NEXT(pass_, res_hi_, nslot_, next_, nvr_, have_, rd_)                                                                 \
     do {                                                                                                                         \
         const bool draw_ = tleft == 1;                                                                                           \
         nslot_ = draw_ ? __builtin_amdgcn_readfirstlane(*s_next) : slot + 1;                                                     \
         have_ = nslot_ < n_pass;                                                                                                 \
         next_ = nslot_;                                                                                                          \
+        nvr_ = 0;                                                                                                                \
         if (list) {                                                                                                              \
             next_ = draw_ ? RS_LIST(nslot_) : ahead;                                                                             \
             ahead = RS_LIST(nslot_ + 1);                                                                                         \
+            nvr_ = draw_ ? rs_vrows(nslot_) : vr_ahead;                                                                          \
+            vr_ahead = rs_vrows(nslot_ + 1);                                                                                     \
         }                                                                                                                        \
-        lo_ = hi_ = 0;                                                                                                           \
+        rd_ = RS_ROUND_NONE;                                                                                                     \
         if (have_) {                                                                                                             \
             const int gn_ = rs_gp0(next_);                                                                                       \
             const bool follows_ = F::WIN ? gn_ == rs_gp0(pass_) + rs_nrw(pass_) : next_ == (pass_) + 1;                          \
-            const SkipXV2 nw_ = rs_new_rows(follows_, res_hi_, gn_, gn_ + rs_nrw(next_) - 1);                                    \
-            lo_ = nw_.qmin;                                                                                                      \
-            hi_ = lo_ + nw_.nrows;                                                                                               \
+            rd_ = rs_round(follows_, res_hi_, gn_, gn_ + rs_nrw(next_) - 1, F::WIN, skipx_v2_unpack(nvr_), F::CHUNK);            \
         }                                                                                                                        \
-        extra_ = rs_round_chunks(hi_ - lo_, F::CHUNK) - 1;                                                                       \
     } while (0)
     __syncthreads();
 
-    int qmin, nrows;
-    RS_ROWS(pass, qmin, nrows);
+    const RsRound first = rs_round(false, 0, rs_gp0(pass), rs_gp0(pass) + rs_nrw(pass) - 1, F::WIN, skipx_v2_unpack(vr), F::CHUNK);
+    const bool make_bg = F::WIN && !list;
+    auto bg_unit = [&]() { if constexpr (F::WIN) return reinterpret_cast<uint4*>(ldsb + (rt >> 6) * G::PLANE + G::BG_SLOT * G::ROWL) + (rt & 63); else return (uint4*)nullptr; };
     if (producer) {
         __builtin_amdgcn_s_setprio((RS_PRIO >> 8) & 3);
         constexpr int CR = G::POOL + G::KH - 1;
@@ -228,11 +227,11 @@
                 }
             }
         };
-        auto p2 = [&](const int c0, const int nr, const int tw) {
+        auto p2 = [&](const int c0, const int nr, const int tw, const int bgslot = -1) {
             if (rt < nr * (4 * F::TPR)) {
                 const int v = rt / (4 * F::TPR), rem = rt - v * (4 * F::TPR), tx = rem >> 2, quad = rem & 3;
                 const int q = c0 + v;
-                const int slot = q % G::NR + 1, rot = w2b_rot(slot);
+                const int slot = bgslot >= 0 ? bgslot : q % G::NR + 1, rot = w2b_rot(slot);
                 float4 d[8];
 #pragma unroll
                 for (int k = 0; k < 8; ++k) {
@@ -316,28 +315,49 @@
                 *reinterpret_cast<float4*>(pbe + (rp * F::PEP + 2 + px) * 64 + c4 * 4) = bg;
             }
         };
-        for (int c = 0, c0 = qmin; c < rs_round_chunks(nrows, F::CHUNK); ++c, c0 += F::CHUNK) {
-            const int nr = qmin + nrows - c0 < F::CHUNK ? qmin + nrows - c0 : F::CHUNK;
+        if constexpr (F::WIN) {
+            if (make_bg) {
+                for (int t = 0; t < G::NBG; ++t) {
+                    p1(1, t);
+                    RS_BAR();
+                    p2(0, 1, t, G::BG_SLOT);
+                    RS_BAR();
+                    bgtab[t * G::BG_UNITS + rt] = *bg_unit();
+                }
+                return;
+            }
+            *bg_unit() = bgtab[rs_t0(pass) * G::BG_UNITS + rt];
+        }
+        for (int c = 0, c0 = first.clo; c < first.chunks; ++c, c0 += F::CHUNK) {
+            const int nr = first.chi - c0 < F::CHUNK ? first.chi - c0 : F::CHUNK;
             uint4 px;
             p0_load(c0, nr, px);
             p0_store(nr, px);
             RS_BAR();
             p1(nr, rs_t0(pass));
-            flag_crops(c0, c0 + nr - 1, S);
+            if (nr > 0) flag_crops(c0, c0 + nr - 1, S);
             RS_BAR();
             p2(c0, nr, rs_t0(pass));
             RS_BAR();
         }
-        int res_hi = qmin + nrows;
+        int res_hi = first.hi;
         int prev = -1;
         for (;;) {
-            int next_slot, next_pass, lo, hi, extra;
+            int next_slot, next_pass, next_vr;
             bool have_next;
-            RS_NEXT(pass, res_hi, next_slot, next_pass, have_next, lo, hi, extra);
+            RsRound rd;
+            RS_NEXT(pass, res_hi, next_slot, next_pass, next_vr, have_next, rd);
+            const int lo = rd.clo, hi = rd.chi, extra = rd.chunks - 1;
             const int tn = have_next ? rs_t0(next_pass) : 0;
             const int nr0 = hi - lo < F::CHUNK ? hi - lo : F::CHUNK;
             uint4 px;
             p0_load(lo, nr0, px);
+            bool bg_swap = false;
+            uint4 bgv = make_uint4(0, 0, 0, 0);
+            if constexpr (F::WIN) {
+                bg_swap = have_next && tn != rs_t0(pass);
+                if (bg_swap) bgv = bgtab[tn * G::BG_UNITS + rt];
+            }
             if (prev >= 0) e2(prev);
             p0_store(nr0, px);
             RS_BAR();
@@ -348,6 +368,7 @@
             bg_store(pass, bg);
             RS_BAR();
             p2(lo, nr0, tn);
+            if constexpr (F::WIN) { if (bg_swap) *bg_unit() = bgv; }
             RS_BAR();
             for (int c = 0, c0 = lo + F::CHUNK; c < extra; ++c, c0 += F::CHUNK) {
                 const int nr = hi - c0 < F::CHUNK ? hi - c0 : F::CHUNK;
@@ -362,9 +383,10 @@
             }
             prev = pass;
             if (!have_next) break;
-            res_hi = hi;
+            res_hi = rd.hi;
             tleft = tleft == 1 ? PK : tleft - 1;
             pass = next_pass;
+            vr = next_vr;
             slot = next_slot;
         }
         e2(prev);
@@ -376,8 +398,11 @@
         const int boff = (h * CO + n * 32 + j) * 16;
         const int co = n * 32 + j;
         const float bz = bias[co];
-        for (int c = 0; c < rs_round_chunks(nrows, F::CHUNK); ++c) { RS_BAR(); RS_BAR(); RS_BAR(); }
-        int res_hi = qmin + nrows;
+        if constexpr (F::WIN) {
+            if (make_bg) { for (int t = 0; t < G::NBG; ++t) { RS_BAR(); RS_BAR(); } return; }
+        }
+        for (int c = 0; c < first.chunks; ++c) { RS_BAR(); RS_BAR(); RS_BAR(); }
+        int res_hi = first.hi;
 #define W2_POS(tau_) rs_pos(tau_)
 #define W2_BOFF(tau_) ((rs_ky(tau_) * 8 + W2_POS(tau_)) * G::BV * 16)
         uint4 bq[8][2];
@@ -403,8 +428,10 @@
 #pragma unroll
             for (int pg = 0; pg < 4; ++pg) { const int w_ = pg * (2 * F::TPR) + tx_ * 2 + h; wh[pg] = (w_ & ~15) * 16; wl[pg] = w_ & 15; }
         }
-#define RS_AOFF(ps_)                                                                                                             \
+#define RS_AOFF(ps_, vr_)                                                                                                        \
         do {                                                                                                                     \
+            const SkipV2 v2_ = skipx_v2_unpack(vr_);                                                                             \
+            const int bg_ = G::NR + 1;                                     \
             int s_ = mg * 32 + j;                                                                                                \
             s_ = s_ < G::RPP * G::TPP ? s_ : G::RPP * G::TPP - 1;                                                                \
             const int rp_ = s_ / G::TPP, r2_ = s_ - rp_ * G::TPP;                                                                \
@@ -412,16 +439,19 @@
             const int qo_ = 2 * gp_ + (r2_ & 1), y_ = qo_ % S;                                                                   \
             _Pragma("unroll") for (int ky = 0; ky < G::KH; ++ky) {                                                               \
                 const int iy_ = y_ + ky - G::KH / 2;                                                                             \
-                const int slot_ = (iy_ >= 0 && iy_ < S) ? (qo_ + ky - G::KH / 2) % G::NR + 1 : 0;                                \
+                const bool made_ = !F::WIN || (iy_ >= v2_.lo && iy_ <= v2_.hi);                                                  \
+                const int slot_ = (iy_ >= 0 && iy_ < S) ? (made_ ? (qo_ + ky - G::KH / 2) % G::NR + 1 : bg_) : 0;                \
                 srow[ky] = slot_ * G::ROWL; srot[ky] = w2b_rot(slot_);                                                           \
             }                                                                                                                    \
         } while (0)
 #define RS_AUNIT(tau_) do { if ((tau_) < 20) aoff[rs_ky(tau_)][rs_pg(tau_)] = srow[rs_ky(tau_)] + (wh[rs_pg(tau_)] | (((wl[rs_pg(tau_)] + srot[rs_ky(tau_)]) & 15) << 4)); } while (0)
-        RS_AOFF(pass);
+        RS_AOFF(pass, vr);
         for (;;) {
-            int next_slot, next_pass, lo, hi, extra;
+            int next_slot, next_pass, next_vr;
             bool have_next;
-            RS_NEXT(pass, res_hi, next_slot, next_pass, have_next, lo, hi, extra);
+            RsRound rd;
+            RS_NEXT(pass, res_hi, next_slot, next_pass, next_vr, have_next, rd);
+            const int extra = rd.chunks - 1;
             const bool draw = tleft == 1;
             uint32_t ticket = 0;
             if (draw && tid == 0) asm volatile("global_atomic_add %0, %1, %2, off sc0" : "=v"(ticket) : "v"(pass_ctr), "v"(1u) : "memory");
@@ -516,13 +546,14 @@
                 }
             }
             { const int g0 = rs_gp0(pass); flag_crops(g0, g0 + rs_nrw(pass) - 1, S / 2); }
-            if (have_next) RS_AOFF(next_pass);
+            if (have_next) RS_AOFF(next_pass, next_vr);
             RS_BAR();
             for (int c = 0; c < extra; ++c) { RS_BAR(); RS_BAR(); RS_BAR(); }
             if (!have_next) break;
-            res_hi = hi;
+            res_hi = rd.hi;
             tleft = tleft == 1 ? PK : tleft - 1;
             pass = next_pass;
+            vr = next_vr;
             slot = next_slot;
         }
 #undef RS_TAP
@@ -535,7 +566,6 @@
     }
 #undef RS_NEXT
 #undef RS_LIST
-#undef RS_ROWS
 #undef RS_BAR
     if (__any(!(ovfm < 4368.0f)) && lane == 0) atomicOr(overflow, 3u);
 }
diff --git a/trex_amd/csrc/cnn_net.h b/trex_amd/csrc/cnn_net.h
--- a/trex_amd/csrc/cnn_net.h
+++ b/trex_amd/csrc/cnn_net.h
@@ -37,6 +37,8 @@
     float* act2e = nullptr;
     int2* skipx_cols = nullptr;
     int* skipx_list = nullptr;
+    uint4* bgtab = nullptr;
+    int* skipx_rows = nullptr;
     float* act3e = nullptr;
     uint2* skip3_counts = nullptr;
     uint32_t* skip3_tcounts = nullptr;
diff --git a/trex_amd/csrc/cnn_plan.h b/trex_amd/csrc/cnn_plan.h
--- a/trex_amd/csrc/cnn_plan.h
+++ b/trex_amd/csrc/cnn_plan.h
@@ -9,6 +9,7 @@
 
 enum : int {
     GEOM_FP32_ACT = 0xfff,
+    GEOM_NO_BGROWS = 1 << 22,
     GEOM_NO_SKIPX = 1 << 23,
     GEOM_DENSE_FC1 = 1 << 24,
     GEOM_V3_COPY = 1 << 25,
@@ -17,7 +18,7 @@
     GEOM_TWO_KERNEL = 1 << 28,
     GEOM_ROLE_SPLIT = 1 << 29,
     GEOM_FUSED_2WG = 1 << 30,
-    GEOM_MASK = GEOM_FP32_ACT | GEOM_NO_SKIPX | GEOM_DENSE_FC1 | GEOM_V3_COPY | GEOM_DENSE_CONV3 | GEOM_NO_SKIP | GEOM_TWO_KERNEL | GEOM_ROLE_SPLIT | GEOM_FUSED_2WG
+    GEOM_MASK = GEOM_FP32_ACT | GEOM_NO_BGROWS | GEOM_NO_SKIPX | GEOM_DENSE_FC1 | GEOM_V3_COPY | GEOM_DENSE_CONV3 | GEOM_NO_SKIP | GEOM_TWO_KERNEL | GEOM_ROLE_SPLIT | GEOM_FUSED_2WG
 };
 
 enum class Chain { ROLE_SPLIT, FUSED_2WG, TWO_KERNEL, FP32_ACT, EXACT, ANY_SIZE };
@@ -52,6 +53,7 @@
     bool v3_direct;
     bool fc1_listed;
     bool skipx;
+    bool bgrows;
 };
 
 inline int ceil_div(const int a, const int b) { return (a + b - 1) / b; }
@@ -96,6 +98,7 @@
     p.skip = role_split && !(geom & GEOM_NO_SKIP);
     p.skip3 = p.skip && !(geom & GEOM_DENSE_CONV3);
     p.skipx = p.skip && !(geom & GEOM_NO_SKIPX) && n < SKIPX_MAX_CROPS;
+    p.bgrows = p.skipx && !(geom & GEOM_NO_BGROWS);
     if (p.skip3) {
         p.skip3_grid = ceil_div(ceil_div(n, 32 ), 256);
         p.act3_fill = {ceil_div(n, 16), n};
diff --git a/trex_amd/csrc/cnn_skip_kernels.h b/trex_amd/csrc/cnn_skip_kernels.h
--- a/trex_amd/csrc/cnn_skip_kernels.h
+++ b/trex_amd/csrc/cnn_skip_kernels.h
@@ -2,6 +2,7 @@
 
 static constexpr int SKIP_LB = 1024;
 static constexpr int SKIP_PAD = 1;
+static constexpr int SKIP_NCNT = 6;
 static constexpr int SKIP_FILL_TB = 256;
 
 __global__ __launch_bounds__(256) void k_crop_bands(const uint8_t* __restrict__ crops, const int n, int2* __restrict__ bands, int2* __restrict__ cols) {
@@ -72,11 +73,12 @@
         return skipx_window({c.x, c.y}, all);
     }
 };
-struct SkipXItem { bool full, need; int wpasses, t0; SkipRows rows; };
-__device__ __forceinline__ SkipXItem skipx_item(const int i, const int n, const int2* __restrict__ bands, const int2* __restrict__ cols, const bool all) {
+struct SkipXItem { bool full, need; int wpasses, t0; SkipRows rows; SkipV2 v2; int v2_read, v2_made; };
+__device__ __forceinline__ SkipXItem skipx_item(const int i, const int n, const int2* __restrict__ bands, const int2* __restrict__ cols, const bool all,
+                                                const bool bgrows) {
     const int total_pairs = n * SkipGeom::V3_ROWS, n_pass = (total_pairs + SkipGeom::RPP - 1) / SkipGeom::RPP;
     const bool none = all || !cols;
-    SkipXItem it{false, false, 0, -1, {1, 0}};
+    SkipXItem it{false, false, 0, -1, {1, 0}, SKIPX_V2_ALL, 0, 0};
     if (i < n_pass) {
         it.need = skip_needed(i, total_pairs, bands, all);
         it.full = it.need && (none || skipx_full_needed(i, total_pairs, SkipBandsOf{bands}, SkipXWinOf{cols, all}));
@@ -86,46 +88,52 @@
         const int2 b = bands[i];
         it.rows = skip_rows({b.x, b.y});
         it.wpasses = it.t0 >= 0 ? skipx_passes(it.rows) : 0;
+        if (bgrows && it.wpasses) {
+            it.v2 = skipx_v2_rows({b.x, b.y});
+            const RsRound r = rs_round(false, 0, it.rows.lo, it.rows.hi, true, it.v2, SkipXGeom::CHUNK);
+            it.v2_read = r.hi - r.lo;
+            it.v2_made = r.chi - r.clo;
+        }
     }
     return it;
 }
 __global__ __launch_bounds__(SKIP_LB) void k_pass_count(const int2* __restrict__ bands, const int2* __restrict__ cols, const int n,
-                                                        const uint32_t* __restrict__ words, uint32_t* __restrict__ counts) {
-    __shared__ uint32_t s_cnt[4];
-    if (threadIdx.x < 4) s_cnt[threadIdx.x] = 0;
-    __syncthreads();
-    const SkipXItem it = skipx_item(blockIdx.x * SKIP_LB + threadIdx.x, n, bands, cols, words[SK_EMPTY_RANGE] != 0);
-    uint32_t v[4] = {it.full ? 1u : 0u, it.need ? 1u : 0u, (uint32_t)it.wpasses, it.wpasses ? 1u : 0u};
-#pragma unroll
-    for (int k = 0; k < 4; ++k) {
+                                                        const uint32_t* __restrict__ words, uint32_t* __restrict__ counts, const int bgrows) {
+    __shared__ uint32_t s_cnt[SKIP_NCNT];
+    if (threadIdx.x < SKIP_NCNT) s_cnt[threadIdx.x] = 0;
+    __syncthreads();
+    const SkipXItem it = skipx_item(blockIdx.x * SKIP_LB + threadIdx.x, n, bands, cols, words[SK_EMPTY_RANGE] != 0, bgrows != 0);
+    uint32_t v[SKIP_NCNT] = {it.full ? 1u : 0u, it.need ? 1u : 0u, (uint32_t)it.wpasses, it.wpasses ? 1u : 0u, (uint32_t)it.v2_read, (uint32_t)it.v2_made};
+#pragma unroll
+    for (int k = 0; k < SKIP_NCNT; ++k) {
 #pragma unroll
         for (int d = 32; d >= 1; d >>= 1) v[k] += __shfl_xor(v[k], d);
         if ((threadIdx.x & 63) == 0 && v[k]) atomicAdd(&s_cnt[k], v[k]);
     }
     __syncthreads();
-    if (threadIdx.x < 4) counts[blockIdx.x * 4 + threadIdx.x] = s_cnt[threadIdx.x];
+    if (threadIdx.x < SKIP_NCNT) counts[blockIdx.x * SKIP_NCNT + threadIdx.x] = s_cnt[threadIdx.x];
 }
 __global__ __launch_bounds__(SKIP_LB) void k_pass_list(const int2* __restrict__ bands, const int2* __restrict__ cols, const int n,
                                                        uint32_t* __restrict__ words, const uint32_t* __restrict__ counts, int* __restrict__ list,
-                                                       int* __restrict__ wlist) {
-    __shared__ uint32_t s_base[4], s_wave[2][SKIP_LB / 64];
+                                                       int* __restrict__ wlist, int* __restrict__ wrows, const int bgrows) {
+    __shared__ uint32_t s_base[SKIP_NCNT], s_wave[2][SKIP_LB / 64];
     const int total_pairs = n * SkipGeom::V3_ROWS, n_pass = (total_pairs + SkipGeom::RPP - 1) / SkipGeom::RPP;
     const int tid = threadIdx.x, lane = tid & 63, wave = tid >> 6;
     const int i = blockIdx.x * SKIP_LB + tid;
-    if (tid < 4) s_base[tid] = 0;
-    __syncthreads();
-    uint32_t part[4] = {0, 0, 0, 0};
+    if (tid < SKIP_NCNT) s_base[tid] = 0;
+    __syncthreads();
+    uint32_t part[SKIP_NCNT] = {0, 0, 0, 0, 0, 0};
     for (int b = tid; b < (int)blockIdx.x; b += SKIP_LB) {
 #pragma unroll
-        for (int k = 0; k < 4; ++k) part[k] += counts[b * 4 + k];
-    }
-#pragma unroll
-    for (int k = 0; k < 4; ++k) {
+        for (int k = 0; k < SKIP_NCNT; ++k) part[k] += counts[b * SKIP_NCNT + k];
+    }
+#pragma unroll
+    for (int k = 0; k < SKIP_NCNT; ++k) {
 #pragma unroll
         for (int d = 32; d >= 1; d >>= 1) part[k] += __shfl_xor(part[k], d);
         if (lane == 0 && part[k]) atomicAdd(&s_base[k], part[k]);
     }
-    const SkipXItem it = skipx_item(i, n, bands, cols, words[SK_EMPTY_RANGE] != 0);
+    const SkipXItem it = skipx_item(i, n, bands, cols, words[SK_EMPTY_RANGE] != 0, bgrows != 0);
     uint32_t sc[2] = {it.full ? 1u : 0u, (uint32_t)it.wpasses};
 #pragma unroll
     for (int k = 0; k < 2; ++k) {
@@ -143,19 +151,20 @@
     if (it.full) list[s_base[0] + sc[0] - 1] = i;
     if (it.wpasses) {
         const uint32_t at = s_base[2] + sc[1] - (uint32_t)it.wpasses;
-        for (int k = 0; k < it.wpasses; ++k) wlist[at + k] = skipx_pack(skipx_pass(i, it.rows, it.t0, k));
+        for (int k = 0; k < it.wpasses; ++k) { wlist[at + k] = skipx_pack(skipx_pass(i, it.rows, it.t0, k)); wrows[at + k] = skipx_v2_pack(it.v2); }
     }
     if (blockIdx.x == gridDim.x - 1 && tid == SKIP_LB - 1) {
         const uint32_t full = s_base[0] + sc[0], wp = s_base[2] + sc[1];
         uint32_t need = s_base[1], wc = s_base[3];
-        for (int k = 0; k < 2; ++k) { const uint32_t c = counts[blockIdx.x * 4 + 1 + 2 * k]; if (k) wc += c; else need += c; }
+        for (int k = 0; k < 2; ++k) { const uint32_t c = counts[blockIdx.x * SKIP_NCNT + 1 + 2 * k]; if (k) wc += c; else need += c; }
         for (int k = 0; k < SKIP_PAD; ++k) list[full + k] = n_pass;
         const bool last_need = skip_needed(n_pass - 1, total_pairs, bands, words[SK_EMPTY_RANGE] != 0);
         const uint32_t listed_rows = need * SkipGeom::RPP - (last_need ? (uint32_t)(n_pass * SkipGeom::RPP - total_pairs) : 0u);
         words[SK_LEN] = need; words[SK_NPASS] = (uint32_t)n_pass; words[SK_FILLED] = (uint32_t)total_pairs - listed_rows;
         if (cols) {
-            for (int k = 0; k < SKIP_PAD; ++k) wlist[wp + k] = 0;
+            for (int k = 0; k < SKIP_PAD; ++k) { wlist[wp + k] = 0; wrows[wp + k] = skipx_v2_pack(SKIPX_V2_ALL); }
             words[SKX_CROPS] = wc; words[SKX_PASSES] = wp; words[SKX_FULL] = full; words[SKX_CTR] = 0;
+            words[SKX_V2_READ] = s_base[4] + counts[blockIdx.x * SKIP_NCNT + 4]; words[SKX_V2_MADE] = s_base[5] + counts[blockIdx.x * SKIP_NCNT + 5];
         }
     }
 }
diff --git a/trex_amd/csrc/cnn_skip_words.h b/trex_amd/csrc/cnn_skip_words.h
--- a/trex_amd/csrc/cnn_skip_words.h
+++ b/trex_amd/csrc/cnn_skip_words.h
@@ -22,8 +22,10 @@
     SKX_PASSES = 27,
     SKX_FULL = 28,
     SKX_CTR = 29,
+    SKX_V2_READ = 30,
+    SKX_V2_MADE = 31,
     SK_WORDS = 32
 };
-static_assert(SK_FILLED < SK3_PAIRS && SK3_LAST < SKX_CROPS && SKX_CTR < SK_WORDS, "no word twice, the last one inside the table");
+static_assert(SK_FILLED < SK3_PAIRS && SK3_LAST < SKX_CROPS && SKX_V2_MADE < SK_WORDS, "no word twice, the last one inside the table");
 
 }
diff --git a/trex_amd/csrc/cnn_skipx.h b/trex_amd/csrc/cnn_skipx.h
--- a/trex_amd/csrc/cnn_skipx.h
+++ b/trex_amd/csrc/cnn_skipx.h
@@ -60,8 +60,21 @@
     return false;
 }
 
-TREXHIP_HD constexpr int rs_round_chunks(const int new_rows, const int chunk) { return new_rows <= chunk ? 1 : (new_rows + chunk - 1) / chunk; }
-TREXHIP_HD constexpr int rs_round_stages(const int new_rows, const int chunk) { return 3 * rs_round_chunks(new_rows, chunk); }
+struct SkipV2 { int lo, hi; };
+static constexpr SkipV2 SKIPX_V2_ALL{0, SkipGeom::V2_ROWS - 1};
+TREXHIP_HD constexpr SkipV2 skipx_v2_rows(const SkipBand b) {
+    using G = SkipGeom;
+    if (b.y0 > b.y1) return {1, 0};
+    constexpr int HI0 = skip_layer_hi(0), LO0 = skip_layer_lo(0);
+    const int lo = b.y0 <= HI0 ? 0 : (b.y0 - HI0 + G::POOL - 1) / G::POOL;
+    const int hi = (b.y1 - LO0) / G::POOL;
+    return {lo, hi < G::V2_ROWS - 1 ? hi : G::V2_ROWS - 1};
+}
+TREXHIP_HD constexpr int skipx_v2_pack(const SkipV2 v) { return v.lo | v.hi << 8; }
+TREXHIP_HD constexpr SkipV2 skipx_v2_unpack(const int w) { return {w & 0xff, (w >> 8) & 0xff}; }
+
+TREXHIP_HD constexpr int rs_round_chunks(const int made_rows, const int chunk) { return made_rows <= chunk ? 1 : (made_rows + chunk - 1) / chunk; }
+TREXHIP_HD constexpr int rs_round_stages(const int made_rows, const int chunk) { return 3 * rs_round_chunks(made_rows, chunk); }
 
 struct SkipXV2 { int qmin, nrows; };
 TREXHIP_HD constexpr SkipXV2 rs_v2_rows(const int gp0, const int gpl) {
@@ -75,5 +88,20 @@
     const int lo = (follows && res_hi > v.qmin) ? res_hi : v.qmin;
     return {lo, v.qmin + v.nrows - lo};
 }
+struct RsRound { int lo, hi, clo, chi, chunks; };
+TREXHIP_HD constexpr RsRound rs_round(const bool follows, const int res_hi, const int gp0n, const int gpln, const bool clip, const SkipV2 v2, const int chunk) {
+    constexpr int S = W2bGeom::S;
+    const SkipXV2 nw = rs_new_rows(follows, res_hi, gp0n, gpln);
+    const int lo = nw.qmin, hi = nw.qmin + nw.nrows;
+    int clo = lo, chi = hi;
+    if (clip) {
+        const int base = (gp0n / (S / 2)) * S;
+        clo = lo > base + v2.lo ? lo : base + v2.lo;
+        chi = hi < base + v2.hi + 1 ? hi : base + v2.hi + 1;
+        if (chi < clo) chi = clo;
+    }
+    return {lo, hi, clo, chi, rs_round_chunks(chi - clo, chunk)};
+}
+static constexpr RsRound RS_ROUND_NONE{0, 0, 0, 0, 1};
 
 }
```

Result: faster. 43870 (median of 6 runs) (+3.6%).
